# osudrl/cassie-mujoco-sim

Hardware: AMD Instinct MI355X
Metric: env-steps/sec (whole node) at N envs; max |qpos_err| vs CPU ref (higher is better)
Workload: dtype f64

## Files before the change

cassie-mujoco-sim_amd/csrc/env_step_collision.inc:

```
        constexpr int chain_rounds = [] {
            if constexpr (TOPO::is_static) { int r = 0, n = 1; while (n < DofLevels<TOPO>::depth() + 1) { n *= 4; ++r; } return r < 3 ? r : 3; }
            else return 3;
        }();
        int pf_jlim, pf_jtype, pf_jqadr, danc[9], blast, kvin;
        double pf_jmargin, pf_jlo, pf_jhi;
        auto request_behind_collision = [&](int lane_now) {
            const int pf_lj = lane_now < njnt ? lane_now : 0, pf_kd = lane_now < nv ? lane_now : 0, pf_bb = lane_now < nbody ? lane_now : 0;
            pf_jlim = m->jnt_limited[pf_lj]; pf_jtype = m->jnt_type[pf_lj]; pf_jqadr = m->jnt_qposadr[pf_lj];
            pf_jmargin = m->jnt_margin[pf_lj]; pf_jlo = m->jnt_range[pf_lj][0]; pf_jhi = m->jnt_range[pf_lj][1];
#pragma unroll
            for (int r = 0; r < 3 * chain_rounds; ++r) danc[r] = m->dof_anc4[pf_kd][r];
            blast = m->body_lastdof[pf_bb]; kvin = m->dof_vinsrc[pf_kd];
        };
        constexpr bool request_early = (FEAT & FEAT_HFIELD) == 0;
        if constexpr (request_early) request_behind_collision(lane);
        const int pair_bound = m->npair_simple;
        struct PairConst { int g1, g2, tt; double margin, rb1, rb2, s10, s11, s20, s21, s22; };
        auto request_pair = [&](int pp, PairConst &c) {
            const int ps = pp < pair_bound ? pp : 0;
            c.g1 = m->pair_geom1[ps]; c.g2 = m->pair_geom2[ps]; c.tt = m->pair_type[ps];
            c.margin = m->pair_margin[ps]; c.rb1 = m->pair_rbound[ps][0]; c.rb2 = m->pair_rbound[ps][1];
            c.s10 = m->pair_size[ps][0]; c.s11 = m->pair_size[ps][1];
            c.s20 = m->pair_size[ps][3]; c.s21 = m->pair_size[ps][4]; c.s22 = m->pair_size[ps][5];
        };
// ... 145 lines not shown
                const double s10 = pc.s10, s11 = pc.s11, s20 = pc.s20, s21 = pc.s21, s22 = pc.s22;
                double dif[3] = {p2[0] - p1[0], p2[1] - p1[1], p2[2] - p1[2]};
                CK_STAMP(31);
                bool cull = false;
                if (rb1 > 0 && rb2 > 0) {
                    double bound = rb1 + rb2 + margin;
                    cull = dot3(dif, dif) > bound * bound;
                } else if (t1 == CM_GEOM_PLANE && rb2 > 0) {
                    double nn[3] = {m1[2], m1[5], m1[8]};
                    cull = dot3(dif, nn) > margin + rb2;
                }
                if (!cull) {
                    if (t1 == CM_GEOM_PLANE && t2 == CM_GEOM_SPHERE) {
                        n = plane_sphere(rc0, p1, m1, p2, s20, margin);
                    } else if (t1 == CM_GEOM_PLANE && t2 == CM_GEOM_CAPSULE) {
                        double axis[3] = {m2[2], m2[5], m2[8]};
                        RawContact tmp;
                        double e0[3] = {p2[0] + s21 * axis[0], p2[1] + s21 * axis[1], p2[2] + s21 * axis[2]};
                        if (plane_sphere(tmp, p1, m1, e0, s20, margin)) { rc0 = tmp; n = 1; }
                        double e1[3] = {p2[0] - s21 * axis[0], p2[1] - s21 * axis[1], p2[2] - s21 * axis[2]};
                        if (plane_sphere(tmp, p1, m1, e1, s20, margin)) { if (n == 0) rc0 = tmp; else rc1 = tmp; ++n; }
                        for (int i = 0; i < 3; ++i) { rc0.tangent[i] = axis[i]; rc1.tangent[i] = axis[i]; }
                    } else if (t1 == CM_GEOM_SPHERE && t2 == CM_GEOM_SPHERE) {
                        n = sphere_sphere(rc0, p1, s10, p2, s20, margin);
                    } else if (t1 == CM_GEOM_SPHERE && t2 == CM_GEOM_CAPSULE) {
                        double a2[3] = {m2[2], m2[5], m2[8]};
                        double d12[3] = {-dif[0], -dif[1], -dif[2]};
                        double x = clampd(dot3(a2, d12), -s21, s21);
                        double q2[3] = {p2[0] + a2[0] * x, p2[1] + a2[1] * x, p2[2] + a2[2] * x};
                        n = sphere_sphere(rc0, p1, s10, q2, s20, margin);
                    } else if (t1 == CM_GEOM_CAPSULE && t2 == CM_GEOM_CAPSULE) {
                        double a1[3] = {m1[2], m1[5], m1[8]}, a2[3] = {m2[2], m2[5], m2[8]};
                        double x1, x2;
                        segment_closest(p1, a1, s11, p2, a2, s21, x1, x2);
                        double q1[3] = {p1[0] + a1[0] * x1, p1[1] + a1[1] * x1, p1[2] + a1[2] * x1};
                        double q2[3] = {p2[0] + a2[0] * x2, p2[1] + a2[1] * x2, p2[2] + a2[2] * x2};
                        n = sphere_sphere(rc0, q1, s10, q2, s20, margin);
                    } else if (t1 == CM_GEOM_SPHERE && t2 == CM_GEOM_BOX) {
                        double sb[3] = {s20, s21, s22};
                        n = sphere_box(rc0, p1, s10, p2, m2, sb, margin);
                    } else if (t1 == CM_GEOM_CAPSULE && t2 == CM_GEOM_BOX) {
                        double sb[3] = {s20, s21, s22};
                        n = capsule_box(rc0, rc1, p1, m1, s10, s11, p2, m2, sb, margin);
                    } else {
                        warn |= WARN_UNSUPPORTED_PAIR;
                    }
                }
            }
            CK_STAMP(32);
            if (p0 + WV_WAVE < npass) request_pair(p + WV_WAVE, pc);
            const unsigned long long m1b = wv::ballot(n >= 1), m2b = wv::ballot(n >= 2);
            const unsigned long long below = (lane == 0) ? 0ull : (~0ull >> (64 - lane));
            int slot = ncon + wv::popc64(m1b & below) + wv::popc64(m2b & below);
            int more = 0;
            if constexpr ((FEAT & FEAT_HFIELD) != 0) {
                const unsigned long long m3b = wv::ballot(n >= 3), m4b = wv::ballot(n >= 4);
                slot += wv::popc64(m3b & below) + wv::popc64(m4b & below);
                more = wv::popc64(m3b) + wv::popc64(m4b);
                for (int extra = 2; extra < CM_HF_MAXC; ++extra)
                    if (n > extra && slot + extra < MAXC) {
                        const double *c = hfres + (size_t)hfs * HF_REC + 1 + 10 * extra;
                        RawContact rx;
                        rx.dist = c[0];
                        for (int i = 0; i < 3; ++i) { rx.pos[i] = c[1 + i]; rx.normal[i] = c[4 + i]; rx.tangent[i] = c[7 + i]; }
                        write_raw_contact(S, slot + extra, p, rx);
                    }
            }
            if (n >= 1 && slot < MAXC) write_raw_contact(S, slot, p, rc0);
            if (n >= 2 && slot + 1 < MAXC) write_raw_contact(S, slot + 1, p, rc1);
            ncon += wv::popc64(m1b) + wv::popc64(m2b) + more;
        }
        CK_STAMP(22);
        if constexpr (!request_early) request_behind_collision(lane);
        if constexpr ((FEAT & FEAT_WAVEPAIRS) != 0) for (int p = m->npair_simple; p < m->npair; ++p) {
            const int g1 = m->pair_geom1[p], g2 = m->pair_geom2[p], tt = m->pair_type[p];
            const int t1 = tt & 255, t2 = tt >> 8;
            const double margin = m->pair_margin[p];
            const double *p1 = S.x.s.geom_xpos[g1], *p2 = S.x.s.geom_xpos[g2];
            const double *m1 = S.x.s.geom_xmat[g1], *m2 = S.x.s.geom_xmat[g2];
            const double rb1 = m->pair_rbound[p][0], rb2 = m->pair_rbound[p][1];
            {
                double dif[3] = {p2[0] - p1[0], p2[1] - p1[1], p2[2] - p1[2]};
                bool cull = false;
                if (rb1 > 0 && rb2 > 0) { const double bound = rb1 + rb2 + margin; cull = dot3(dif, dif) > bound * bound; }
                else if (t1 == CM_GEOM_PLANE && rb2 > 0) { double nn[3] = {m1[2], m1[5], m1[8]}; cull = dot3(dif, nn) > margin + rb2; }
                if (cull) continue;
            }
            bool hit = false;
            int pairmax = 4;
            RawContact rc;
            if (t1 == CM_GEOM_PLANE && t2 == CM_GEOM_BOX) {
                if (lane < 8) {
                    const double sb0 = m->pair_size[p][3], sb1 = m->pair_size[p][4], sb2 = m->pair_size[p][5];
                    double nrm[3] = {m1[2], m1[5], m1[8]}, dif[3] = {p2[0] - p1[0], p2[1] - p1[1], p2[2] - p1[2]};
                    const double dist = dot3(dif, nrm);
                    double v[3] = {(lane & 1) ? sb0 : -sb0, (lane & 2) ? sb1 : -sb1, (lane & 4) ? sb2 : -sb2}, corner[3];
                    mulmatvec3(corner, m2, v);
                    const double ld = dot3(nrm, corner);
                    if (!(dist + ld > margin || ld > 0)) {
                        hit = true;
                        rc.dist = dist + ld;
                        for (int k = 0; k < 3; ++k) { rc.normal[k] = nrm[k]; rc.tangent[k] = 0; rc.pos[k] = corner[k] + p2[k] - nrm[k] * 0.5 * rc.dist; }
                    }
                }
            } else if (t1 == CM_GEOM_BOX && t2 == CM_GEOM_BOX) {
                double s1[3] = {m->pair_size[p][0], m->pair_size[p][1], m->pair_size[p][2]};
                double s2[3] = {m->pair_size[p][3], m->pair_size[p][4], m->pair_size[p][5]};
                pairmax = (m->flags & CM_FLAG_BOX8) ? 8 : 4;
                hit = box_box_lane(rc, lane, p1, m1, s1, p2, m2, s2, margin, pairmax);
            } else {
                warn |= WARN_UNSUPPORTED_PAIR;
            }
            const unsigned long long hb = wv::ballot(hit);
            const unsigned long long below = (lane == 0) ? 0ull : (~0ull >> (64 - lane));
            const int rank = wv::popc64(hb & below);
            if (hit && rank < pairmax && ncon + rank < MAXC) write_raw_contact(S, ncon + rank, p, rc);
            const int nh = wv::popc64(hb);
            ncon += nh < pairmax ? nh : pairmax;
        }
        const int ncon_found = ncon;
        if (ncon > capc) ncon = capc;
        wv::sync();
        finish_contacts(S, m, P, lane, ncon);
        unsigned long long lob, hib;
        {
            bool lo = false, hi = false;
            wv::keep(pf_jlim); wv::keep(pf_jtype);
            if (lane < njnt && pf_jlim && (pf_jtype == CM_JNT_HINGE || pf_jtype == CM_JNT_SLIDE)) {
                const double q = S.qpos[pf_jqadr];
                lo = q - pf_jlo < pf_jmargin;
                hi = pf_jhi - q < pf_jmargin;
            }
            lob = wv::ballot(lo); hib = wv::ballot(hi);
        }
        if constexpr (MAXR < WIDE_ROWS) {
            const bool may_go_down = io.down_rows > 0 && sub > sub_start;
            if (can_hand_over || may_go_down) {
                const int neq = m->neq;
                const bool eact = lane < neq && m->eq_active[lane < neq ? lane : 0] != 0;
                wv::sync();
                const int nfrictionless = wv::popc64(wv::ballot(lane < ncon && S.c_dim[lane < MAXC ? lane : 0] == 1));
                const int need = 3 * wv::popc64(wv::ballot(eact)) + wv::popc64(lob) + wv::popc64(hib) + 4 * ncon - 3 * nfrictionless;
                const bool up = can_hand_over && (need > capr || (ncon_found > capc && MAXC < m->maxcon));
                const bool down = !up && may_go_down && need <= io.down_rows;
                if (up || down) {
                    bailed = true; bailed_down = down;
                    if constexpr (NW == 2) { if (lane == 0) S.cmd[0] = 1; wv::publish(&S.cmd[4], sub + 1); }
                    break;
                }
            }
        }
        if (ncon_found > capc) warn |= WARN_CONTACT_FULL;
        if constexpr (NW == 1) if (io.drive_mode) {
            if (io.integrate) drive_level_io(io, S, m, env, lane, lastsub);
            wv::sync();
        }
        if constexpr (NW == 2) { CK_STAMP(33); wv::publish(&S.cmd[4], sub + 1); wv::wait_for(&S.cmd[3], sub + 1); }
        CK_STAMP(5);
```

cassie-mujoco-sim_amd/csrc/env_step_rows.inc:

```
        int r_ = lane;
        int rtype = -1, rid = 0, rsub = 0;
        int nefc = 0, nefc_before_contacts = 0;
        double rpos = 0, rmargin = 0, rR = 1.0, rK = 0, rB = 0, rimp = 1.0;
        const bool need_imu = lastsub || io.all_outputs_every_substep || (io.drive_mode && sub + 2 == nsub);
        const bool need_pos = lastsub || io.drive_mode || io.all_outputs_every_substep;
        const bool issens = lane < m->nsensor && need_pos;
        const int ls = issens ? lane : 0;
        SensorConsts sens_c;
        double ycol[NVP];
        double jvel = 0, jws = 0;
        const bool lastcol = !WIDE && lane == NROW - 1;
        for (int pass = 0; pass < (WIDE ? 2 : 1); ++pass) {
        if constexpr (WIDE) {
            if (pass == 1 && nefc <= NROW) break;
            r_ = NROW * pass + lane; rtype = -1; rid = 0; rsub = 0; nefc = 0; jvel = 0; jws = 0;
            rpos = 0; rmargin = 0; rR = 1.0; rK = 0; rB = 0; rimp = 1.0;
        }
        {
            const int neq = m->neq;
            const bool eact = lane < neq && m->eq_active[lane < neq ? lane : 0] != 0;
            const unsigned long long eall = neq >= 64 ? ~0ull : (1ull << neq) - 1;
            if (wv::ballot(eact) == eall && 3 * neq <= capr) {
                if (r_ < 3 * neq) { rtype = CM_CNSTR_EQUALITY; rid = r_ / 3; rsub = r_ - 3 * rid; }
                nefc = 3 * neq;
// ... 10 lines not shown
                const int j = wv::popc64((any & (0ull - any)) - 1);
                for (int side = 0; side < 2; ++side) {
                    if (!(((side == 0 ? lob : hib) >> j) & 1ull)) continue;
                    if (nefc >= capr) { warn |= WARN_CONSTRAINT_FULL; continue; }
                    if (r_ == nefc) { rtype = CM_CNSTR_LIMIT_JOINT; rid = j; rsub = side; }
                    ++nefc;
                }
            }
        }
        nefc_before_contacts = nefc;
        const bool cpyr = lane < ncon && S.c_dim[lane < ncon ? lane : 0] == 3;
        if (wv::ballot(cpyr) == (ncon >= 64 ? ~0ull : (1ull << ncon) - 1) && nefc + 4 * ncon <= capr) {
            if (r_ >= nefc && r_ < nefc + 4 * ncon) { rtype = CM_CNSTR_CONTACT_PYRAMIDAL; rid = (r_ - nefc) >> 2; rsub = (r_ - nefc) & 3; }
            nefc += 4 * ncon;
        } else
        for (int c = 0; c < ncon; ++c) {
            const int dim = S.c_dim[c];
            if (dim != 1 && dim != 3) { warn |= WARN_UNSUPPORTED_PAIR; continue; }
            const int nrow = dim == 1 ? 1 : 2 * (dim - 1);
            if (nefc + nrow > capr) { warn |= WARN_CONSTRAINT_FULL; continue; }
            if (r_ >= nefc && r_ < nefc + nrow) {
                rtype = dim == 1 ? CM_CNSTR_CONTACT_FRICTIONLESS : CM_CNSTR_CONTACT_PYRAMIDAL;
                rid = c; rsub = r_ - nefc;
            }
            nefc += nrow;
        }

        CK_STAMP(25);
        double u3[3] = {0, 0, 0}, wp[3] = {0, 0, 0}, wm[3] = {0, 0, 0};
        unsigned long long maskp = 0, maskm = 0;
        int limdof = -1;
        double limsgn = 0, rdiag = 0, imp_pos = 0, rRscale = 1.0;
        double solref0 = 0.02, solref1 = 1, solimp[5] = {0.9, 0.95, 0.001, 0.5, 2};
        if (rtype == CM_CNSTR_EQUALITY) {
            if (rid != pf_eq) {
                pf_eb1 = m->eq_body1[rid]; pf_eb2 = m->eq_body2[rid]; pf_er1 = m->eq_root[rid][0]; pf_er2 = m->eq_root[rid][1];
            }
            maskp = m->eq_dofmask[rid][0]; maskm = m->eq_dofmask[rid][1];
            rdiag = P->eq_invweight[rid];
            solref0 = m->eq_solref[rid][0]; solref1 = m->eq_solref[rid][1];
            for (int i = 0; i < 5; ++i) solimp[i] = m->eq_solimp[rid][i];
            const int b1 = pf_eb1, b2 = pf_eb2;
            double l1[3] = {m->eq_data[rid][0], m->eq_data[rid][1], m->eq_data[rid][2]};
            double l2[3] = {m->eq_data[rid][3], m->eq_data[rid][4], m->eq_data[rid][5]};
            double a1[3], a2[3];
            mulmatvec3(a1, S.x.s.xmat[b1], l1);
            mulmatvec3(a2, S.x.s.xmat[b2], l2);
            for (int i = 0; i < 3; ++i) { a1[i] += S.x.s.xpos[b1][i]; a2[i] += S.x.s.xpos[b2][i]; }
            u3[0] = rsub == 0 ? 1.0 : 0.0; u3[1] = rsub == 1 ? 1.0 : 0.0; u3[2] = rsub == 2 ? 1.0 : 0.0;
            const double *c1 = S.com[pf_er1], *c2 = S.com[pf_er2];
            double o1[3] = {a1[0] - c1[0], a1[1] - c1[1], a1[2] - c1[2]};
            double o2[3] = {a2[0] - c2[0], a2[1] - c2[1], a2[2] - c2[2]};
            cross3(wp, o1, u3);
            cross3(wm, o2, u3);

            double res[3] = {a1[0] - a2[0], a1[1] - a2[1], a1[2] - a2[2]};
            rpos = rsub == 0 ? res[0] : (rsub == 1 ? res[1] : res[2]); rmargin = 0;
            imp_pos = sqrt(dot3(res, res));

        } else if (rtype == CM_CNSTR_LIMIT_JOINT) {
            const double q = S.qpos[m->jnt_qposadr[rid]];
            rpos = rsub == 0 ? q - m->jnt_range[rid][0] : m->jnt_range[rid][1] - q;
            rmargin = m->jnt_margin[rid];
            imp_pos = rpos;
            limdof = m->jnt_dofadr[rid];
            limsgn = rsub == 0 ? 1.0 : -1.0;
            rdiag = P->jnt_liminvweight[rid];
            solref0 = m->jnt_solref[rid][0]; solref1 = m->jnt_solref[rid][1];
            for (int i = 0; i < 5; ++i) solimp[i] = m->jnt_solimp[rid][i];
        } else if (rtype >= 0) {
            const int c = rid;
            const double *fr = S.c_frame[c];
            if (rtype == CM_CNSTR_CONTACT_PYRAMIDAL) {
                const int a = 1 + rsub / 2;
                const double mu = a <= 2 ? S.c_fri[c][0] : (a == 3 ? S.c_fri[c][1] : S.c_fri[c][2]);
                const double sg = (rsub & 1) ? -mu : mu;
                for (int i = 0; i < 3; ++i) u3[i] = fr[i] + sg * fr[3 * a + i];
                const double mu0 = S.c_fri[c][0];
                rRscale = 2 * mu0 * mu0;
            } else {
                for (int i = 0; i < 3; ++i) u3[i] = fr[i];
            }
            const double *c1 = S.com[S.c_root[c][0]], *c2 = S.com[S.c_root[c][1]];
            double o1[3] = {S.c_pos[c][0] - c1[0], S.c_pos[c][1] - c1[1], S.c_pos[c][2] - c1[2]};
            double o2[3] = {S.c_pos[c][0] - c2[0], S.c_pos[c][1] - c2[1], S.c_pos[c][2] - c2[2]};
            cross3(wp, o2, u3);
            cross3(wm, o1, u3);
            maskp = S.c_dofmask[c][1];
            maskm = S.c_dofmask[c][0];
            rpos = S.c_dist[c]; rmargin = S.c_margin[c]; imp_pos = rpos;
            const double tran = S.c_tran[c];
            const double mu_first = S.c_fri[c][0];
            rdiag = rtype == CM_CNSTR_CONTACT_PYRAMIDAL ? tran + mu_first * mu_first * tran : tran;
            solref0 = S.c_solref[c][0]; solref1 = S.c_solref[c][1];
            for (int i = 0; i < 5; ++i) solimp[i] = S.c_solimp[c][i];
        }
        CK_STAMP(26);
        if (rtype >= 0) {
            rimp = impedance(solimp, imp_pos, rmargin);
            rR = fmax(CM_MINVAL, (1 - rimp) * rdiag / rimp);
            if (rtype == CM_CNSTR_CONTACT_PYRAMIDAL) rR = fmax(CM_MINVAL, rRscale * rR);
            const double dmax = solimp[1];
            if (solref0 > 0) {
                double tc = solref0;
                if ((m->flags & CM_FLAG_REFSAFE) && tc < 2 * h) tc = 2 * h;
                rK = 1.0 / fmax(CM_MINVAL, dmax * dmax * tc * tc * solref1 * solref1);
                rB = 2.0 / fmax(CM_MINVAL, dmax * tc);
            } else {
                rK = -solref0 / fmax(CM_MINVAL, dmax * dmax);
                rB = -solref1 / fmax(CM_MINVAL, dmax);
            }
        }
        CK_STAMP(27);
        if constexpr (NW == 1) sens_c = request_sensor_consts(m, ls);
#pragma unroll
        for (int k0 = 0; k0 < NVP; k0 += 4) {
            double cc[4][6], qv[4], qw[4], qs[4];
#pragma unroll
            for (int kk = 0; kk < 4; ++kk) {
#pragma unroll
                for (int t = 0; t < 6; ++t) cc[kk][t] = S.cdof[k0 + kk][t];
                qv[kk] = S.qvel[k0 + kk]; qw[kk] = S.qacc_ws[k0 + kk];
                if constexpr (NW == 1) qs[kk] = S.qfrc_smooth[k0 + kk]; else qs[kk] = 0.0;
            }
            wv::sched_fence();
#pragma unroll
            for (int kk = 0; kk < 4; ++kk) {
                const int k = k0 + kk;
                double v = 0;
                if (TOPO::is_static ? k < TOPO::nv : k < nv) {
                    if (rtype >= 0) {
                        const double ul = u3[0] * cc[kk][3] + u3[1] * cc[kk][4] + u3[2] * cc[kk][5];
                        const double sp = bitf(maskp, k), sm = bitf(maskm, k);
                        v = sp * (ul + wp[0] * cc[kk][0] + wp[1] * cc[kk][1] + wp[2] * cc[kk][2]) -
                            sm * (ul + wm[0] * cc[kk][0] + wm[1] * cc[kk][1] + wm[2] * cc[kk][2]);
                        if (k == limdof) v = limsgn;
                        jvel += v * qv[kk];
                        jws += v * qw[kk];
                    } else if (lastcol) {
                        v = qs[kk];
                    }
                }
                ycol[k] = v;
            }
        }
        if constexpr (WIDE) {
            if (r_ < MAXR) {
#pragma unroll
                for (int k = 0; k < NVP; ++k) S.x.Yr[r_][k] = ycol[k];
                double *rt = S.x.rowt[r_];
                rt[0] = rR; rt[1] = rtype >= 0 ? -rB * jvel - rK * rimp * (rpos - rmargin) : 0.0; rt[2] = jws;
                rt[3] = rtype < 0 ? -1.0 : (rtype == CM_CNSTR_EQUALITY ? 0.0 : 1.0);
            }
            if (io.ext && pass == 0 && rtype == CM_CNSTR_EQUALITY && r_ < CM_MAXEQROW) {
                cm_ext_t *ex = io.ext + env;
                ex->eq_pos[r_] = rpos; ex->eq_id[r_] = rid;
#pragma unroll
                for (int k = 0; k < NVP; ++k) if (k < nv) ex->eq_J[r_][k] = ycol[k];
            }
        }
        }
        const int sb = NW == 1 ? sens_c.sb : 0;
        CK_STAMP(28);
        if constexpr (NW == 2) {
            if constexpr (WIDE) { if (lane == 0) S.x.turn[0] = nefc; }
            CK_STAMP(34); wv::block_barrier();
            if (lastcol) {
#pragma unroll
                for (int k = 0; k < NVP; ++k) ycol[k] = (TOPO::is_static ? k < TOPO::nv : k < nv) ? S.qfrc_smooth[k] : 0.0;
            }
        }
        const double raref = rtype >= 0 ? -rB * jvel - rK * rimp * (rpos - rmargin) : 0.0;

        int aslot = -1;
        if constexpr (NW == 1) aslot = sensors_before_solve(io, S, m, env, issens, ls, sens_c, need_imu, lastsub);
        CK_STAMP(29);
        if (io.xpos_out && isbody && lastsub) {
            for (int i = 0; i < 3; ++i) io.xpos_out[((size_t)env * io.sb + b) * 3 + i] = S.x.s.xpos[b][i];
            if (io.xquat_out) for (int i = 0; i < 4; ++i) io.xquat_out[((size_t)env * io.sb + b) * 4 + i] = S.x.s.xquat[b][i];
        }
        if (io.ext) {
            cm_ext_t *ex = io.ext + env;
            if (isbody) for (int i = 0; i < 6; ++i) ex->cvel[b][i] = S.x.s.cvel[b][i];
            if (isbody) for (int i = 0; i < 3; ++i) { ex->subtree_com[b][i] = S.com[broot > 0 ? broot : 0][i]; ex->xipos[b][i] = S.x.s.xipos[b][i]; }
            if (lane < m->nsite) {
                const int sb = m->site_bodyid[lane];
                double sp[3] = {m->site_pos[lane][0], m->site_pos[lane][1], m->site_pos[lane][2]};
                double sq[4] = {m->site_quat[lane][0], m->site_quat[lane][1], m->site_quat[lane][2], m->site_quat[lane][3]};
                double t[3], q[4], mm[9];
                mulmatvec3(t, S.x.s.xmat[sb], sp);
                for (int i = 0; i < 3; ++i) ex->site_xpos[lane][i] = t[i] + S.x.s.xpos[sb][i];
                mulquat(q, S.x.s.xquat[sb], sq);
                quat2mat(mm, q);
                for (int i = 0; i < 9; ++i) ex->site_xmat[lane][i] = mm[i];
            }
            if (isdof) for (int i = 0; i < 6; ++i) { ex->cdof[k_][i] = S.cdof[k_][i]; ex->cdof_dot[k_][i] = S.x.s.cdof_dot[k_][i]; }
            if (!WIDE && rtype == CM_CNSTR_EQUALITY && r_ < CM_MAXEQROW) {
                ex->eq_pos[r_] = rpos; ex->eq_id[r_] = rid;
#pragma unroll
                for (int k = 0; k < NVP; ++k) if (k < nv) ex->eq_J[r_][k] = ycol[k];
            }
            if (lane == 0) { int ne = 0; for (int e = 0; e < m->neq; ++e) if (m->eq_active[e] && ne + 3 <= capr) ne += 3; ex->ne = ne; }
            if (lane < ncon) {
                ex->con_geom1[lane] = m->geom_fullid[S.c_g1[lane]]; ex->con_geom2[lane] = m->geom_fullid[S.c_g2[lane]];
                ex->con_body1[lane] = m->geom_bodyid[S.c_g1[lane]]; ex->con_body2[lane] = m->geom_bodyid[S.c_g2[lane]];
                ex->con_dim[lane] = S.c_dim[lane]; ex->con_dist[lane] = S.c_dist[lane];
                for (int i = 0; i < 3; ++i) ex->con_pos[lane][i] = S.c_pos[lane][i];
                for (int i = 0; i < 9; ++i) ex->con_frame[lane][i] = S.c_frame[lane][i];
            }
        }
        int caddr = -1;
        const bool want_cfrc = io.body_cfrc && (sub == nsub - 1 || !io.integrate);
        if (io.ext || want_cfrc) {
            int acc = nefc_before_contacts;
            for (int c = 0; c < ncon; ++c) {
                const int dim = S.c_dim[c];
                if (dim != 1 && dim != 3) continue;
                const int nrow = dim == 1 ? 1 : 2 * (dim - 1);
                if (acc + nrow > capr) continue;
                if (c == lane) caddr = acc;
                acc += nrow;
            }
        }
        wv::sync();
        CK_STAMP(8);
```

cassie-mujoco-sim_amd/csrc/env_step_solve.inc:

```
        if constexpr (WIDE) {
            int iters = 0, nguarded = 0;
            const double f = wide_solve<NVP, TOPO>(S, m, P, 0, nefc, sub, iters, nguarded);
            CK_STAMP(11);

            static_assert(sizeof(S.c_solimp) >= (2 * NROW + 4) * sizeof(double), "the row forces are handed over through the contacts' solimp slots");
            double *const fbuf = &S.c_solimp[0][0];
            fbuf[lane] = f;
            if (lane == 0) { fbuf[2 * NROW] = (double)ncon; fbuf[2 * NROW + 1] = (double)nefc; fbuf[2 * NROW + 2] = (double)iters; fbuf[2 * NROW + 3] = (double)nguarded; }
            wv::block_barrier();
#ifdef CK_WIDE_PROFILE
            if (io.prof && lane < 12) io.prof[(size_t)env * NSTAMP + (lane < 6 ? 16 + lane : 22 + lane)] = (long long)S.x.stepv[lane / 6][lane % 6];
#endif
            if (io.ext || want_cfrc) {
                const int a0 = caddr >= 0 ? caddr : 0;
                double fn = 0, ft1 = 0, ft2 = 0;
                if (lane < ncon && caddr >= 0) {
                    const double f0 = fbuf[a0];
                    if (S.c_dim[lane] == 1) fn = f0;
                    else { const double f1 = fbuf[a0 + 1], f2 = fbuf[a0 + 2], f3 = fbuf[a0 + 3], mu = S.c_fri[lane][0]; fn = f0 + f1 + f2 + f3; ft1 = mu * (f0 - f1); ft2 = mu * (f2 - f3); }
                }
                if (io.ext) {
                    cm_ext_t *ex = io.ext + env;
                    if (lane < ncon) { ex->con_force[lane][0] = fn; ex->con_force[lane][1] = ft1; ex->con_force[lane][2] = ft2; }
                    if (lane == 0) { ex->ncon = ncon; ex->nefc = nefc; ex->solver_iter = iters; }
                }
                if (want_cfrc) {
                    if (lane < ncon) {
                        const double *fr = S.c_frame[lane];
                        double fw[3];
                        for (int j = 0; j < 3; ++j) fw[j] = fr[j] * fn + fr[3 + j] * ft1 + fr[6 + j] * ft2;
                        for (int j = 0; j < 3; ++j) S.c_pos[lane][j] = fw[j];
                    }
                    wv::sync();
                    if (isbody) {
                        double acc[3] = {0, 0, 0};
                        for (int c = 0; c < ncon; ++c) {
                            const int b1 = m->geom_bodyid[S.c_g1[c]], b2 = m->geom_bodyid[S.c_g2[c]];
                            const double sg = (b2 == b ? 1.0 : 0.0) - (b1 == b ? 1.0 : 0.0);
                            for (int j = 0; j < 3; ++j) acc[j] += sg * S.c_pos[c][j];
                        }
                        for (int j = 0; j < 3; ++j) io.body_cfrc[((size_t)env * io.sb + b) * 3 + j] = acc[j];
                    }
                    wv::sync();
                }
            }
            wv::block_barrier();
            CK_STAMP(37);
            if (wv::opaque(S.cmd[0])) { warn |= WARN_DIVERGED; break; }
            if (!io.integrate) break;
            time += h;
            continue;
        }
        if constexpr (TOPO::is_static) {
            double ta[NVP], tb[NVP], ra = 0, rb = 0;
            auto fetch = [&](int k, double (&t)[NVP], double &rs) {
#pragma unroll
                for (int i = k - 1; i >= 0; --i) if ((TOPO::table[k] >> i) & 1ull) t[i] = S.Lp[LPack<TOPO, NVP>::idx(k, i)];
                rs = S.rsd[k];
            };
            fetch(TOPO::nv - 1, ((TOPO::nv - 1) & 1) ? ta : tb, ((TOPO::nv - 1) & 1) ? ra : rb);
#pragma unroll
            for (int k = NVP - 1; k >= 0; --k) {
                if (k >= TOPO::nv) continue;
                if (k > 0) fetch(k - 1, ((k - 1) & 1) ? ta : tb, ((k - 1) & 1) ? ra : rb);
                wv::sched_fence();
                const double (&t)[NVP] = (k & 1) ? ta : tb;
                const double xk = ycol[k];
#pragma unroll
                for (int i = k - 1; i >= 0; --i) if ((TOPO::table[k] >> i) & 1ull) ycol[i] -= t[i] * xk;
                ycol[k] = xk * ((k & 1) ? ra : rb);
                wv::sched_fence();
            }
        } else {
#pragma unroll
            for (int k = NVP - 1; k >= 0; --k) {
                if (k >= nv) continue;
                const unsigned long long anc = m->dof_ancmask[k];
                const double xk = ycol[k];
#pragma unroll
                for (int i = k - 1; i >= 0; --i) {
                    if (!((anc >> i) & 1ull)) continue;
                    ycol[i] -= S.Lp[CK_TRI(k, i)] * xk;
                }
                ycol[k] = xk * S.rsd[k];
            }
        }
        if (r_ < MAXR || lastcol) {
            const int yrow = lastcol ? MAXR : r_;
#pragma unroll
            for (int k = 0; k < NVP; ++k) S.x.Yr[yrow][k] = ycol[k];
        }
        wv::sync();
        if constexpr (NW == 2) wv::publish(&S.cmd[2], sub + 1);
        CK_STAMP(9);

        double arow[MAXR];
        double diag_yy = 0;
        double rb = 0;
        constexpr bool gram_on_matrix_core = MAXR == 31 && NVP % 4 == 0;
        constexpr bool gram_in_place = MAXR == 47 && NVP == 40;
        if constexpr (gram_on_matrix_core) {
            constexpr int YP = EnvShared<NVP, LPack<TOPO, NVP>::count, MAXR>::YP;
            static_assert(2 * (MAXR + 1) * YP * sizeof(double) <= sizeof(S.x), "the Gram matrix is parked behind the staged tile");
            double (*Am)[YP] = (double (*)[YP])(&S.x.Yr[0][0] + (MAXR + 1) * YP);
            const int mi = lane & 15, mk = lane >> 4;
            double y0[NVP / 4], y1[NVP / 4];
#pragma unroll
            for (int kb = 0; kb < NVP / 4; ++kb) { y0[kb] = S.x.Yr[mi][4 * kb + mk]; y1[kb] = S.x.Yr[16 + mi][4 * kb + mk]; }
            wv::mfma_acc t00 = {{0, 0, 0, 0}}, t01 = {{0, 0, 0, 0}}, t11 = {{0, 0, 0, 0}};
#pragma unroll
            for (int kb = 0; kb < NVP / 4; ++kb) wv::mfma_f64_16x16x4_x3(y0[kb], y0[kb], t00, y0[kb], y1[kb], t01, y1[kb], y1[kb], t11);
            wv::mfma_f64_drain(t00, t01, t11);
#pragma unroll
            for (int v = 0; v < 4; ++v) {
                const int row = mk + 4 * v;
                Am[row][mi] = t00.c[v];
                Am[row][16 + mi] = t01.c[v];
                Am[16 + mi][row] = t01.c[v];
                Am[16 + row][16 + mi] = t11.c[v];
            }
            wv::sync();
            const int myrow = lane & 31;
#pragma unroll
            for (int t = 0; t < MAXR; ++t) arow[t] = Am[myrow][t];
            rb = Am[myrow][MAXR] - raref;
#pragma unroll
            for (int k = 0; k < NVP; ++k) wv::touch(ycol[k]);
            diag_yy = Am[myrow][myrow];
        } else if constexpr (gram_in_place) {
            constexpr int AP = 49, AR = MAXR + 1;
            static_assert(AR == 48, "three blocks of sixteen staged rows");
            static_assert(AR * AP * sizeof(double) <= sizeof(S.x), "the matrix fits the region of the staged tile");
            double (*Am)[AP] = (double (*)[AP])&S.x.Yr[0][0];
            const int mi = lane & 15, mk = lane >> 4;
            double y0[NVP / 4], y1[NVP / 4], y2[NVP / 4];
#pragma unroll
            for (int kb = 0; kb < NVP / 4; ++kb) { y0[kb] = S.x.Yr[mi][4 * kb + mk]; y1[kb] = S.x.Yr[16 + mi][4 * kb + mk]; y2[kb] = S.x.Yr[32 + mi][4 * kb + mk]; }
            wv::mfma_acc t00 = {{0, 0, 0, 0}}, t01 = {{0, 0, 0, 0}}, t11 = {{0, 0, 0, 0}}, t02 = {{0, 0, 0, 0}}, t12 = {{0, 0, 0, 0}}, t22 = {{0, 0, 0, 0}};
#pragma unroll
            for (int kb = 0; kb < NVP / 4; ++kb) wv::mfma_f64_16x16x4_x3(y0[kb], y2[kb], t02, y1[kb], y2[kb], t12, y2[kb], y2[kb], t22);
#pragma unroll
            for (int kb = 0; kb < NVP / 4; ++kb) wv::mfma_f64_16x16x4_x3(y0[kb], y0[kb], t00, y0[kb], y1[kb], t01, y1[kb], y1[kb], t11);
            wv::mfma_f64_drain(t00, t01, t11);
            wv::mfma_f64_drain(t02, t12, t22);
            wv::sync();
#pragma unroll
            for (int v = 0; v < 4; ++v) {
                const int row = mk + 4 * v;
                Am[row][mi] = t00.c[v];
                Am[row][16 + mi] = t01.c[v]; Am[16 + mi][row] = t01.c[v];
                Am[16 + row][16 + mi] = t11.c[v];
                Am[row][32 + mi] = t02.c[v]; Am[32 + mi][row] = t02.c[v];
                Am[16 + row][32 + mi] = t12.c[v]; Am[32 + mi][16 + row] = t12.c[v];
                Am[32 + row][32 + mi] = t22.c[v];
            }
            wv::sync();
            const int myrow = lane < AR ? lane : AR - 1;
            rb = Am[myrow][MAXR] - raref;
            diag_yy = Am[myrow][myrow];
#pragma unroll
            for (int t = 0; t < MAXR; ++t) arow[t] = Am[myrow][t];
            wv::sync();
            if (r_ < MAXR || lastcol) {
                const int yrow = lastcol ? MAXR : r_;
#pragma unroll
                for (int k = 0; k < NVP; ++k) S.x.Yr[yrow][k] = ycol[k];
            }
            wv::sync();
        }
        else if constexpr (NW == 2 && NVP > 32) {
#pragma unroll
            for (int r = 0; r < MAXR; ++r) {
                double acc = 0;
                if (r < nefc) {
#pragma unroll
                    for (int k0 = 0; k0 < NVP; k0 += NVP / 2) {
                        double ya[NVP / 2];
#pragma unroll
                        for (int k = 0; k < NVP / 2; ++k) ya[k] = S.x.Yr[r][k0 + k];
#pragma unroll
                        for (int k = 0; k < NVP / 2; ++k) acc = fma(ya[k], ycol[k0 + k], acc);
                    }
                }
                arow[r] = acc;
            }
            {
                double acc = 0;
#pragma unroll
                for (int k = 0; k < NVP; ++k) acc = fma(S.x.Yr[MAXR][k], ycol[k], acc);
                rb = acc - raref;
            }
        } else {
#pragma unroll
        for (int r = 0; r < MAXR; r += 2) {
            double acc0 = 0, acc1 = 0;
            if (r < nefc) {
                constexpr int YB1 = NVP > 32 ? NVP / 2 : NVP;
                double ya[NVP], yb[NVP];
#pragma unroll
                for (int k = 0; k < NVP; ++k) ya[k] = S.x.Yr[r][k];
#pragma unroll
                for (int k = 0; k < YB1; ++k) yb[k] = S.x.Yr[r + 1 < MAXR ? r + 1 : r][k];
                wv::sched_fence();
                if constexpr (NVP == 32) {
#pragma unroll
                    for (int k = 0; k < NVP; ++k) { acc0 = fma(ya[k], ycol[k], acc0); if (r + 1 < MAXR) acc1 = fma(yb[k], ycol[k], acc1); }
                } else if constexpr (NVP == 40) {
#pragma unroll
                    for (int k = 0; k < YB1; ++k) { acc0 = fma(ya[k], ycol[k], acc0); if (r + 1 < MAXR) acc1 = fma(yb[k], ycol[k], acc1); }
                    wv::sched_fence();
#pragma unroll
                    for (int k = YB1; k < NVP; ++k) yb[k] = S.x.Yr[r + 1 < MAXR ? r + 1 : r][k];
#pragma unroll
                    for (int k = YB1; k < NVP; ++k) { acc0 = fma(ya[k], ycol[k], acc0); if (r + 1 < MAXR) acc1 = fma(yb[k], ycol[k], acc1); }
                } else {
                double a0 = 0, a1 = 0, a2 = 0, a3 = 0;
#pragma unroll
                for (int k = 0; k < NVP; k += 4) {
                    a0 += ya[k] * ycol[k]; a1 += ya[k + 1] * ycol[k + 1];
                    a2 += ya[k + 2] * ycol[k + 2]; a3 += ya[k + 3] * ycol[k + 3];
                }
                acc0 = (a0 + a1) + (a2 + a3);
                if constexpr (YB1 < NVP) {
                    wv::sched_fence();
#pragma unroll
                    for (int k = YB1; k < NVP; ++k) yb[k] = S.x.Yr[r + 1 < MAXR ? r + 1 : r][k];
                }
                if (r + 1 < MAXR) {
                    double b0 = 0, b1 = 0, b2 = 0, b3 = 0;
#pragma unroll
                    for (int k = 0; k < NVP; k += 4) {
                        b0 += yb[k] * ycol[k]; b1 += yb[k + 1] * ycol[k + 1];
                        b2 += yb[k + 2] * ycol[k + 2]; b3 += yb[k + 3] * ycol[k + 3];
                    }
                    acc1 = (b0 + b1) + (b2 + b3);
                }
                }
            }
            arow[r] = acc0;
            if (r + 1 < MAXR) arow[r + 1] = acc1;
        }
        {
            double acc = 0;
#pragma unroll
            for (int k = 0; k < NVP; ++k) acc = fma(S.x.Yr[MAXR][k], ycol[k], acc);
            rb = acc - raref;
        }
        }
        CK_STAMP(10);

        const bool isrow = rtype >= 0;
        const bool clampf = isrow && rtype != CM_CNSTR_EQUALITY;
        double Aii = 1.0;
        if constexpr (gram_on_matrix_core || gram_in_place) { if (isrow) Aii = diag_yy + rR; }
        else if (isrow) {
            if constexpr (NVP == 32 || NVP == 40) {
                double d = 0;
#pragma unroll
                for (int k = 0; k < NVP; ++k) d = fma(ycol[k], ycol[k], d);
                Aii = d + rR;
            } else {
                double d0 = 0, d1 = 0, d2 = 0, d3 = 0;
#pragma unroll
                for (int k = 0; k < NVP; k += 4) {
                    d0 += ycol[k] * ycol[k]; d1 += ycol[k + 1] * ycol[k + 1];
                    d2 += ycol[k + 2] * ycol[k + 2]; d3 += ycol[k + 3] * ycol[k + 3];
                }
                Aii = ((d0 + d1) + (d2 + d3)) + rR;
            }
        }
        const double invAii = 1.0 / Aii;
        double f = 0, res = isrow ? rb : 0.0;
        int iters = 0, nguarded = 0;
        if (nefc > 0) {
            if (m->flags & CM_FLAG_WARMSTART) {
                if (isrow) {
                    f = -(jws - raref) / rR;
                    if (clampf && f < 0) f = 0;
                }
                double af0 = 0, af1 = 0, af2 = 0, af3 = 0;
#pragma unroll
                for (int t = 0; t < MAXR; t += 4) {
                    if (t < nefc) {
                        af0 += arow[t] * wv::readlane(f, t);
                        if (t + 1 < MAXR) af1 += arow[t + 1] * wv::readlane(f, t + 1);
                        if (t + 2 < MAXR) af2 += arow[t + 2] * wv::readlane(f, t + 2);
                        if (t + 3 < MAXR) af3 += arow[t + 3] * wv::readlane(f, t + 3);
                    }
                }
                const double af = ((af0 + af1) + (af2 + af3)) + (isrow ? rR * f : 0.0);
                double cost = wv::wave_sum(isrow ? f * (rb + 0.5 * af) : 0.0);
                if (cost > 0) f = 0;
                else if (isrow) res = rb + af;
            }
        CK_STAMP(30);
            const double scale = 1.0 / (P->meaninertia * (nv > 1 ? nv : 1));
            const double halfAii = 0.5 * Aii;
            const double flo = clampf ? 0.0 : -1e300;
            const double ninvAii = -invAii;
            double sres = res * ninvAii;
#pragma unroll
            for (int t = 0; t < MAXR; ++t) arow[t] *= ninvAii;
            const double cdiag = isrow ? rR * ninvAii : 0.0;
            const int maxiter = m->iterations;
            const double tolerance = m->tolerance;
            const bool shortcut_ok = 0.5 * tolerance > (double)MAXR * 1e-10 * scale;
            if constexpr (NW == 2 && CK_PRIO_W0_PGS != CK_PRIO_W0) wv::set_priority<CK_PRIO_W0_PGS>();
            while (iters < maxiter) {
                const int nrows = wv::opaque(nefc);
                bool converged;
                {
                    const double f0 = f, s0 = sres;
                    double mys = 0;
                    const double lo_f = flo - f;
                    pgs_rows_fast<0, MAXR>(arow, nrows, r_, lo_f, sres, mys);
                    const double mydelta = wv::max_raw(mys, lo_f);
                    const double change = (r_ < nrows) ? mydelta * (halfAii * mydelta - Aii * mys) : 0.0;
                    const float tol = (float)tolerance;
                    const bool one_row_decides = shortcut_ok && wv::ballot(-(float)change * (float)scale > 2.5f * tol) != 0ull;
                    const float est = one_row_decides ? 4.0f * tol : -wv::wave_sum_f32((float)change) * (float)scale;
                    if (wv::ballot(change > 1e-10) != 0ull || wv::debug_force_guarded()) {
                        double improvement = 0;
                        f = f0; sres = s0; ++nguarded;
                        pgs_rows<0, MAXR>(arow, nrows, r_, Aii, halfAii, flo, f, sres, improvement);
                        sres = fma(cdiag, f - f0, sres);
                        converged = improvement * scale < tolerance;
                    } else {
                        if (r_ < nrows) { f += mydelta; sres = fma(cdiag, mydelta, sres); }
                        if (est < 0.5f * tol) converged = true;
                        else if (est > 2.0f * tol) converged = false;
                        else {
                            const double tree = -wv::wave_sum(change) * scale, tolv = tolerance;
                            if (fabs(tree - tolv) > 1e-9 * tolv) converged = tree < tolv;
                            else
                            {
                                double improvement = 0;
                                for (int t = 0; t < nrows; ++t) improvement -= wv::readlane(change, t);
                                converged = improvement * scale < tolerance;
                            }
                        }
                    }
                }
                ++iters;
                if (converged) break;
            }
        }
        if constexpr (NW == 2 && CK_PRIO_W0_PGS != CK_PRIO_W0) wv::set_priority<CK_PRIO_W0>();
        CK_STAMP(11);
        if (io.ext || want_cfrc) {
            const int a0 = caddr >= 0 ? caddr : 0;
            const double f0 = wv::shfl(f, a0), f1 = wv::shfl(f, (a0 + 1) & 63), f2 = wv::shfl(f, (a0 + 2) & 63), f3 = wv::shfl(f, (a0 + 3) & 63);
            double fn = 0, ft1 = 0, ft2 = 0;
            if (lane < ncon && caddr >= 0) {
                if (S.c_dim[lane] == 1) fn = f0;
                else { const double mu = S.c_fri[lane][0]; fn = f0 + f1 + f2 + f3; ft1 = mu * (f0 - f1); ft2 = mu * (f2 - f3); }
            }
            if (io.ext) {
                cm_ext_t *ex = io.ext + env;
                if (lane < ncon) { ex->con_force[lane][0] = fn; ex->con_force[lane][1] = ft1; ex->con_force[lane][2] = ft2; }
                if (lane == 0) { ex->ncon = ncon; ex->nefc = nefc; ex->solver_iter = iters; }
            }
            if (want_cfrc) {
                if (lane < ncon) {
                    const double *fr = S.c_frame[lane];
                    double fw[3];
                    for (int j = 0; j < 3; ++j) fw[j] = fr[j] * fn + fr[3 + j] * ft1 + fr[6 + j] * ft2;
                    for (int j = 0; j < 3; ++j) S.c_pos[lane][j] = fw[j];
                }
                wv::sync();
                if (isbody) {
                    double acc[3] = {0, 0, 0};
                    for (int c = 0; c < ncon; ++c) {
                        const int b1 = m->geom_bodyid[S.c_g1[c]], b2 = m->geom_bodyid[S.c_g2[c]];
                        const double sg = (b2 == b ? 1.0 : 0.0) - (b1 == b ? 1.0 : 0.0);
                        for (int j = 0; j < 3; ++j) acc[j] += sg * S.c_pos[c][j];
                    }
                    for (int j = 0; j < 3; ++j) io.body_cfrc[((size_t)env * io.sb + b) * 3 + j] = acc[j];
                }
                wv::sync();
            }
        }

        if constexpr (NW == 2) {
            static_assert(sizeof(S.c_solimp) >= 68 * sizeof(double), "the row forces are handed over through the contacts' solimp slots");
            double *const fbuf = &S.c_solimp[0][0];
            fbuf[lane] = f;
            if (lane == 0) { fbuf[64] = (double)ncon; fbuf[65] = (double)nefc; fbuf[66] = (double)iters; fbuf[67] = (double)nguarded; }
            wv::block_barrier();
            wv::block_barrier();
            CK_STAMP(37);
            if (wv::opaque(S.cmd[0])) { warn |= WARN_DIVERGED; break; }
            if (!io.integrate) break;
            time += h;
            continue;
        }
        const int pf_u = lane < nu ? lane : 0, pf_ej = lane < njnt ? lane : 0;
        const double pf_agear = m->act_gear[pf_u], pf_kdamp = P->dof_damping[isdof ? k_ : 0];
        const int pf_adof = m->act_dofid[pf_u], pf_ejt = m->jnt_type[pf_ej], pf_eqa = m->jnt_qposadr[pf_ej], pf_eda = m->jnt_dofadr[pf_ej];
        double qacc;
        {
            double z = isdof ? S.x.Yr[MAXR][k_] : 0.0;
            {
                double z1 = 0, z2 = 0, z3 = 0;
                const int kk = isdof ? k_ : 0;
                int r = 0;
                for (; r + 4 <= nefc; r += 4) {
                    const double y0 = S.x.Yr[r][kk], y1 = S.x.Yr[r + 1][kk], y2 = S.x.Yr[r + 2][kk], y3 = S.x.Yr[r + 3][kk];
                    z += y0 * wv::readlane(f, r); z1 += y1 * wv::readlane(f, r + 1);
                    z2 += y2 * wv::readlane(f, r + 2); z3 += y3 * wv::readlane(f, r + 3);
                }
                for (; r < nefc; ++r) z += S.x.Yr[r][kk] * wv::readlane(f, r);
                z = (z + z1) + (z2 + z3);
                if (!isdof) z = 0.0;
            }
            if (isdof) z *= S.rsd[k_];
            double lrow[NVP];
            stage_factor_row<NVP, TOPO>(S, k_, isdof, lrow);
            qacc = solve_forward<NVP, TOPO>(z, lrow, lane, nv);
        }
        {
            const bool badv = isdof && (!(qacc == qacc) || fabs(qacc) > 1e10);
            if (wv::ballot(badv) != 0ull) { warn |= WARN_DIVERGED; break; }
        }
        if (isdof) S.qacc[k_] = qacc;
        wv::sync();
        CK_STAMP(12);

        outputs_after_qacc(io, S, m, env, lane, isdof, k_, nu, qacc, aslot, sb, need_imu, lastsub, pf_agear * S.qvel[pf_adof], ncon, nefc, iters, nguarded);
        if (!io.integrate) break;
        CK_STAMP(13);

        {
            double lcol[NVP], lrowh[NVP];
            stage_factor_h<NVP, TOPO>(S, k_, isdof, nv, lcol, lrowh);
            const double dih = isdof ? S.dinvH[k_] : 0.0;
            euler_step<NVP, TOPO>(S, m, lane, isdof, k_, nv, njnt, h, qacc, lcol, lrowh, dih, pf_kdamp, pf_ejt, pf_eqa, pf_eda);
        }
        time += h;
        CK_STAMP(14);
    }
```

cassie-mujoco-sim_amd/csrc/env_step_wave1.inc:

```
    if constexpr (NW == 2) {
        if (wid == 1) {
            for (int sub1 = sub_start;;) {
                const int pb = isbody ? b : 0;
                const double mass = P->body_mass[pb];
                double iner[3], imat[9];
                for (int i = 0; i < 3; ++i) iner[i] = P->body_inertia[pb][i];
                for (int i = 0; i < 9; ++i) imat[i] = m->body_imat[pb][i];
                CK_STAMP(35);
                wv::block_barrier();
                if (wv::opaque(S.cmd[0])) return -1;
                wv::set_priority<(FEAT & FEAT_HFIELD) != 0 ? CK_PRIO_W1_FJ_HFIELD : CK_PRIO_W1_FJ>();
                CK_STAMP(36);
                double ximat[9] = {1, 0, 0, 0, 1, 0, 0, 0, 1};
                if (isbody && b > 0) {
                    double xm[9];
                    for (int i = 0; i < 9; ++i) xm[i] = S.x.s.xmat[b][i];
                    for (int i = 0; i < 3; ++i)
                        for (int c = 0; c < 3; ++c) ximat[3 * i + c] = xm[3 * i] * imat[c] + xm[3 * i + 1] * imat[3 + c] + xm[3 * i + 2] * imat[6 + c];
                }
                double col[NVP], colh[NVP];
                mass_matrix_columns<NVP, TOPO, FEAT, NW>(io, S, m, env, ids, mass, iner, ximat, col, colh);
                wv::publish(&S.cmd[3], sub1 + 1);
                CK_STAMP(38);
                factor_pair_by_height<NVP, TOPO, 0>(m, P, h, S, col, colh, lane);
                constexpr bool park_colh = NVP > 32;
                if constexpr (park_colh) {
                    if (isdof) {
#pragma unroll
                        for (int i = 0; i < NVP; ++i) {
                            if (i >= TOPO::nv) continue;
                            if (i == k_) S.dinvH[k_] = colh[i];
                            else if (i > k_ && LP::col_has(i, k_)) S.LHp[LP::col_idx(i, k_)] = colh[i];
                        }
                    }
                    wv::sync();
                }
                wv::wait_for(&S.cmd[4], sub1 + 1);
                if (wv::opaque(S.cmd[0])) return -1;
                if (io.drive_mode) {
                    if (io.integrate) drive_level_io(io, S, m, env, lane, sub1 == nsub - 1);
                    wv::sync();
                }
                CK_STAMP(4);
                {
                    const int kd = isdof ? k_ : 0;
                    const double kdamp = P->dof_damping[kd], kstiff = PS->dof_stiffness[kd], kref = PS->dof_springref[kd];
                    const double kgear = m->dof_gear[kd], klo = m->dof_ctrl_lo[kd], khi = m->dof_ctrl_hi[kd];
                    const int kq = m->dof_qadr[kd], ka = m->dof_act[kd];
                    wv::wait_for(&S.cmd[1], sub1 + 1);
                    bias_forces_and_qfrc_smooth<NVP, (NVP > 32)>(io, S, m, env, ids, kdamp, kstiff, kref, kgear, klo, khi, kq, ka);
                }
                const bool lastsub1 = sub1 == nsub - 1 || !io.integrate;
                const bool need_imu1 = lastsub1 || io.all_outputs_every_substep || (io.drive_mode && sub1 + 2 == nsub);
                const bool issens1 = lane < m->nsensor && (lastsub1 || io.drive_mode || io.all_outputs_every_substep);
                const int ls1 = issens1 ? lane : 0;
                const SensorConsts sens_c1 = request_sensor_consts(m, ls1);
                const int aslot1 = sensors_before_solve(io, S, m, env, issens1, ls1, sens_c1, need_imu1, lastsub1);
                CK_STAMP(47);
                wv::block_barrier();
                wv::set_priority<CK_PRIO_W1_JP>();
                CK_STAMP(39);
                if constexpr (WIDE) {
                    int it1 = 0, ng1 = 0;
                    const double f1 = wide_solve<NVP, TOPO>(S, m, P, 1, wv::opaque(S.x.turn[0]), sub1, it1, ng1);
                    (&S.c_solimp[0][0])[NROW + lane] = f1;
                }
                if constexpr (park_colh) {
#pragma unroll
                    for (int i = 0; i < NVP; ++i) {
                        double v = 0.0;
                        if (i < TOPO::nv && isdof) {
                            if (i == k_) v = S.dinvH[k_];
                            else if (i > k_ && LP::col_has(i, k_)) v = S.LHp[LP::col_idx(i, k_)];
                        }
                        colh[i] = v;
                    }
                    wv::sync();
                }
                factor_pair_by_height<NVP, TOPO, 1>(m, P, h, S, col, colh, lane);
                {
                    const bool lastsub = lastsub1, need_imu = need_imu1;
                    const int sb = sens_c1.sb, aslot = aslot1;
                    const int pf_u = lane < nu ? lane : 0, pf_ej = lane < njnt ? lane : 0;
                    const double pf_agear = m->act_gear[pf_u], pf_kdamp = P->dof_damping[isdof ? k_ : 0];
                    const int pf_adof = m->act_dofid[pf_u], pf_ejt = m->jnt_type[pf_ej], pf_eqa = m->jnt_qposadr[pf_ej], pf_eda = m->jnt_dofadr[pf_ej];
                    const double *const fbuf = &S.c_solimp[0][0];
                    double lrow[NVP];
                    constexpr bool stage_h_early = NVP <= 32;
                    if constexpr (stage_h_early) stage_factor_row<NVP, TOPO>(S, k_, isdof, lrow);
                    double lcol[NVP], lrowh[NVP];
                    if constexpr (stage_h_early) stage_factor_h<NVP, TOPO, 0>(S, k_, isdof, nv, lcol, lrowh);
                    const double rsdk = isdof ? S.rsd[k_] : 0.0;
                    const int kk = isdof ? k_ : 0;
                    constexpr bool stage_y = MAXR <= 31;
                    double ycolk[stage_y ? MAXR + 1 : 1];
                    if constexpr (stage_y) {
                        wv::wait_for(&S.cmd[2], sub1 + 1);
#pragma unroll
                        for (int r = 0; r <= MAXR; ++r) ycolk[r] = S.x.Yr[r][kk];
                    }
                    wv::block_barrier();
                    wv::set_priority<CK_PRIO_W1_PE>();
                    const double f = fbuf[lane], f_hi = WIDE ? fbuf[NROW + lane] : 0.0;
                    constexpr int FB = WIDE ? 2 * NROW : NROW;
                    const int ncon = (int)fbuf[FB], nefc = (int)fbuf[FB + 1], iters = (int)fbuf[FB + 2], nguarded = (int)fbuf[FB + 3];
                    double z, z1 = 0, z2 = 0, z3 = 0;
                    if constexpr (stage_y) {
                        z = isdof ? ycolk[MAXR] : 0.0;
#pragma unroll
                        for (int r = 0; r < MAXR; r += 4) {
                            if (r + 4 <= nefc) {
                                z += ycolk[r] * wv::readlane(f, r); z1 += ycolk[r + 1 < MAXR ? r + 1 : r] * wv::readlane(f, r + 1);
                                z2 += ycolk[r + 2 < MAXR ? r + 2 : r] * wv::readlane(f, r + 2); z3 += ycolk[r + 3 < MAXR ? r + 3 : r] * wv::readlane(f, r + 3);
                            } else {
#pragma unroll
                                for (int j = 0; j < 4; ++j) if (r + j < nefc && r + j < MAXR) z += ycolk[r + j < MAXR ? r + j : r] * wv::readlane(f, r + j);
                            }
                        }
                    } else {
                        z = isdof ? S.x.Yr[MAXR][k_] : 0.0;
                        auto frow = [&](int r) { if constexpr (WIDE) return r < NROW ? wv::readlane(f, r) : wv::readlane(f_hi, r - NROW); else return wv::readlane(f, r); };
                        int r = 0;
                        for (; r + 4 <= nefc; r += 4) {
                            const double y0 = S.x.Yr[r][kk], y1 = S.x.Yr[r + 1][kk], y2 = S.x.Yr[r + 2][kk], y3 = S.x.Yr[r + 3][kk];
                            z += y0 * frow(r); z1 += y1 * frow(r + 1);
                            z2 += y2 * frow(r + 2); z3 += y3 * frow(r + 3);
                        }
                        for (; r < nefc; ++r) z += S.x.Yr[r][kk] * frow(r);
                    }
                    z = (z + z1) + (z2 + z3);
                    if (!isdof) z = 0.0;
                    if (isdof) z *= rsdk;
                    if constexpr (stage_h_early) stage_factor_h<NVP, TOPO, 1>(S, k_, isdof, nv, lcol, lrowh);
                    const double dih = isdof ? S.dinvH[k_] : 0.0;
                    if constexpr (!stage_h_early) stage_factor_row<NVP, TOPO>(S, k_, isdof, lrow);
                    wv::sched_fence();
                    const double qacc = solve_forward<NVP, TOPO>(z, lrow, lane, nv);
                    {
                        const bool badv = isdof && (!(qacc == qacc) || fabs(qacc) > 1e10);
                        if (wv::ballot(badv) != 0ull) {
                            if (lane == 0) S.cmd[0] = 2;
                            wv::block_barrier();
                            return -1;
                        }
                    }
                    if (isdof) S.qacc[k_] = qacc;
                    const double av = pf_agear * S.qvel[pf_adof];
                    wv::sync();
                    CK_STAMP(12);
                    if (io.integrate) {
                        if constexpr (!stage_h_early) stage_factor_h<NVP, TOPO>(S, k_, isdof, nv, lcol, lrowh);
                        euler_step<NVP, TOPO>(S, m, lane, isdof, k_, nv, njnt, h, qacc, lcol, lrowh, dih, pf_kdamp, pf_ejt, pf_eqa, pf_eda);
                    }
                    CK_STAMP(13);
                    wv::block_barrier();
                    wv::set_priority<CK_PRIO_W1_EF>();
                    outputs_after_qacc(io, S, m, env, lane, isdof, k_, nu, qacc, aslot, sb, need_imu, lastsub, av, ncon, nefc, iters, nguarded);
                    CK_STAMP(14);
                }
                if (!io.integrate || ++sub1 >= nsub) return -1;
            }
        }
    }
```

cassie-mujoco-sim_amd/csrc/kernels_cassie.hip:

```cpp
#include "step_kernels.h"
namespace ck {
template void launch_step<32, TopoCassie32, 0>(unsigned, hipStream_t, const PhysIO &);
template void launch_step<32, TopoCassie32, 0, FAST_ROWS>(unsigned, hipStream_t, const PhysIO &);
}
```

cassie-mujoco-sim_amd/csrc/kernels_cassie_2w.hip:

```cpp
#include "step_kernels.h"
namespace ck {
template void launch_step<32, TopoCassie32, 0, FAST_ROWS, 2>(unsigned, hipStream_t, const PhysIO &);
}
```

cassie-mujoco-sim_amd/csrc/kernels_cassie_2w_inplace.hip:

```cpp
#include "step_kernels.h"
namespace ck {
template void launch_step<32, TopoCassie32, 0, FAST_ROWS, 2, false, 2, MID_ROWS>(unsigned, hipStream_t, const PhysIO &);
}
```

cassie-mujoco-sim_amd/csrc/kernels_hfield.hip:

```cpp
#include "step_kernels.h"
namespace ck {
template void launch_step<32, TopoCassie32, FEAT_HFIELD>(unsigned, hipStream_t, const PhysIO &);
template void launch_step<32, TopoCassie32, FEAT_HFIELD, FAST_ROWS>(unsigned, hipStream_t, const PhysIO &);
}
```

cassie-mujoco-sim_amd/csrc/kernels_hfield_2w.hip:

```cpp
#include "step_kernels.h"
namespace ck {
template void launch_step<32, TopoCassie32, FEAT_HFIELD, FAST_ROWS, 2>(unsigned, hipStream_t, const PhysIO &);
}
```

cassie-mujoco-sim_amd/csrc/kernels_hfield_2w_inplace.hip:

```cpp
#include "step_kernels.h"
namespace ck {
template void launch_step<32, TopoCassie32, FEAT_HFIELD, FAST_ROWS, 2, false, 2, MID_ROWS>(unsigned, hipStream_t, const PhysIO &);
}
```

cassie-mujoco-sim_amd/csrc/kernels_tray_2w.hip:

```cpp
#include "step_kernels.h"
namespace ck {
template void launch_step<40, TopoCassieTray38, FEAT_WAVEPAIRS, FAST_ROWS_TRAY, 2>(unsigned, hipStream_t, const PhysIO &);
}
```

cassie-mujoco-sim_amd/csrc/kernels_tray_fast.hip:

```cpp
#include "step_kernels.h"
namespace ck {
template void launch_step<40, TopoCassieTray38, FEAT_WAVEPAIRS, FAST_ROWS_TRAY>(unsigned, hipStream_t, const PhysIO &);
template void launch_step<40, TopoCassieTray38, FEAT_WAVEPAIRS, MID_ROWS, 1, true>(unsigned, hipStream_t, const PhysIO &);
}
```

cassie-mujoco-sim_amd/csrc/phys_batch.hip:

```cpp
#include <hip/hip_runtime.h>

#include <cstddef>
#include <cstdio>
#include <cstdlib>
#include <cstring>
#include <string>
#include <utility>
#include <vector>

#include "cassie_phys.h"
#include "device_mem.h"
#include "small_launch.h"
#include "step_launch.h"
#include "step_policy.h"

void phys_set_last_error(const char *s);

constexpr int DEFAULT_TRAY_WAVES = 2;

struct phys_batch {
    int nenv = 0, device = 0;
    cm_model_t host_model;
    DevBuf<cm_model_t> d_models;
    DevBuf<cm_envparams_t> d_envparams;
// ... 9 lines not shown
    DevBuf<int> d_terrain_index;
    ck::ScanCfg scan = {};
    DevBuf<double> d_scan_offsets;
    ck::DepthCfg depth = {};
    long long depth_launches[2] = {0, 0};
    ck::RayCfg rays = {};
    DevBuf<ck::RayDef> d_rays;
    long long ray_launches = 0;
    hipStream_t stream = nullptr;
    hipStream_t recent_streams[4] = {nullptr, nullptr, nullptr, nullptr};
    int recent_next = 0;
    hipEvent_t ev0 = nullptr, ev1 = nullptr, ev_mark = nullptr;
    bool use_applied = false;
    bool pd_mode = false;
    int drive_mode = CM_DRIVE_OFF;
    DevBuf<cm_drive_state_t> d_drive;
    bool use_pd_dtarget = false, use_pd_torque = false;
    DevBuf<long long> d_prof;
    bool all_outputs = false;
    DevBuf<cm_ext_t> d_ext;

    bool fast_rows = true;
    int waves_per_env = 2;
    int waves_per_env_tray = DEFAULT_TRAY_WAVES;
    int inplace_mode = 2;
    long long form_launches[2] = {0, 0};
    bool balance = true;
    DevBuf<unsigned> d_cost, d_cost_wall;
    DevBuf<int> d_order;
    std::vector<int> order_ident;
    ck::RangeTable ranges;
    DevBuf<int> d_progress;
    int chunks = ck::DEFAULT_CHUNKS_WHOLE, chunks_range = ck::DEFAULT_CHUNKS_RANGE;
    bool chunks_default = true;
    DevBuf<int> d_chunk_flag;
    int chunk_seq = 0;
    bool chunks_allowed = true;
    std::vector<std::pair<hipStream_t, bool>> probed_streams;
    HostWords chunk_fault;
    bool chunk_fault_reported = false;
    DevBuf<int> d_handover_list, d_handover_count, d_handover_list2, d_handover_count2;
    HostWords handover_seen, handover_seen2;
    bool timing = false;
    std::vector<std::pair<hipEvent_t, hipEvent_t>> ev_pool;
    size_t ev_used = 0;

    DevBuf<double> d_scratch_out;
    bool episodes = false;
    ck::EpisodeCfg ep = {};
    DevBuf<char> d_ep[PHYS_EP_ARRAYS];
    DevBuf<const double> d_ep_bank;
    ck::PlaceCfg place = {};
    DevBuf<ck::PlaceTable> d_place_table;
    DevBuf<double> d_place_offsets, d_place_pose, d_place_ground;
};

static bool hip_ok(hipError_t e, const char *what) {
    if (e == hipSuccess) return true;
    std::string msg = std::string("HIP error in ") + what + ": " + hipGetErrorString(e);
    phys_set_last_error(msg.c_str());
    fprintf(stderr, "cassie_phys: %s\n", msg.c_str());
    return false;
}

static ck::PhysIO make_io(phys_batch *b, int nsub, int integrate) {
    ck::PhysIO io;
    memset(&io, 0, sizeof io);
    io.models = b->d_models;
    io.model_stride = b->model_stride;
    io.envparams = b->d_envparams;
    io.nenv = b->nenv; io.nsub = nsub; io.integrate = integrate;
    io.sq = b->stride[PHYS_F_QPOS]; io.sqv = b->stride[PHYS_F_QVEL]; io.sv = b->host_model.nv; io.su = b->host_model.nu;
    io.ssd = b->stride[PHYS_F_SENSORDATA]; io.sb = b->host_model.nbody;
    io.qpos = b->d_field[PHYS_F_QPOS]; io.qvel = b->d_field[PHYS_F_QVEL];
    io.qacc_warmstart = b->d_field[PHYS_F_QACC_WARMSTART]; io.time = b->d_field[PHYS_F_TIME];
    io.ctrl = b->d_field[PHYS_F_CTRL];
    io.qfrc_applied = b->use_applied ? b->d_field[PHYS_F_QFRC_APPLIED] : nullptr;
    io.xfrc_applied = b->use_applied ? b->d_field[PHYS_F_XFRC_APPLIED] : nullptr;
    io.qacc = b->d_field[PHYS_F_QACC]; io.sensordata = b->d_field[PHYS_F_SENSORDATA];
    io.actuator_velocity = b->d_field[PHYS_F_ACTUATOR_VELOCITY];
    io.warn = b->d_warn; io.info = b->d_info;
    io.xpos_out = b->d_field[PHYS_F_XPOS]; io.xquat_out = b->d_field[PHYS_F_XQUAT];
    io.body_cfrc = b->d_field[PHYS_F_BODY_CFRC];
    io.hfield = b->d_hfield;
    io.hfield_stride = b->hfield_stride;
    if (b->nterrain > 0) { io.hfield_index = b->d_terrain_index; io.hfield_nterrain = b->nterrain; }
    if (b->pd_mode) {
        io.pd_ptarget = b->d_field[PHYS_F_PD_PTARGET]; io.pd_kp = b->d_field[PHYS_F_PD_KP]; io.pd_kd = b->d_field[PHYS_F_PD_KD];
    }
    io.drive_mode = b->d_drive ? b->drive_mode : CM_DRIVE_OFF;
    if (io.drive_mode != CM_DRIVE_OFF) {
        io.drive_state = b->d_drive;
        io.drive_cmd = b->d_field[PHYS_F_DRIVE_CMD];
        io.meas = b->d_field[PHYS_F_MEAS];
        if (io.drive_mode == CM_DRIVE_PD || io.drive_mode == CM_DRIVE_PD_SAFE) {
            io.pd_ptarget = b->d_field[PHYS_F_PD_PTARGET]; io.pd_kp = b->d_field[PHYS_F_PD_KP]; io.pd_kd = b->d_field[PHYS_F_PD_KD];
            io.pd_dtarget = b->use_pd_dtarget ? b->d_field[PHYS_F_PD_DTARGET] : nullptr;
            io.pd_torque = b->use_pd_torque ? b->d_field[PHYS_F_PD_TORQUE] : nullptr;
        }
    }
    io.all_outputs_every_substep = b->all_outputs ? 1 : 0;
    io.prof = b->d_prof;
    io.ext = b->d_ext;
    if (b->balance && b->d_order) { io.order = b->d_order; io.cost = b->d_cost; io.cost_wall = b->d_cost_wall; }
    return io;
}

static bool quiesce(phys_batch *b) {
    bool ok = hip_ok(hipStreamSynchronize(b->stream), "hipStreamSynchronize");
    for (hipStream_t r : b->recent_streams)
        if (r && r != b->stream) ok = hip_ok(hipStreamSynchronize(r), "hipStreamSynchronize(caller stream)") && ok;
    return ok;
}

static void note_stream(phys_batch *b, hipStream_t s) {
    for (hipStream_t r : b->recent_streams) if (r == s) return;
    b->recent_streams[b->recent_next] = s;
    b->recent_next = (b->recent_next + 1) % 4;
}

static hipStream_t launch_stream(phys_batch *b, void *stream) {
    const hipStream_t s = stream ? (hipStream_t)stream : b->stream;
    note_stream(b, s);
    return s;
}

static bool range_ok(const phys_batch *b, int env0, int n) {
    return env0 >= 0 && n >= 0 && (size_t)env0 + (size_t)n <= (size_t)b->nenv;
}
static bool strided_ok(const phys_batch *b, int first, int stride, int count) {
    return first >= 0 && stride >= 1 && count >= 0 && (count == 0 || (size_t)first + (size_t)(count - 1) * (size_t)stride < (size_t)b->nenv);
}

static ck::BatchView view_of(const phys_batch *b) {
    ck::BatchView v = {b->d_models, b->model_stride, b->d_envparams, b->d_hfield, b->hfield_stride, b->d_terrain_index, b->nterrain};
    ck::view_sizes(v, b->host_model);
    v.sq = b->stride[PHYS_F_QPOS]; v.sqv = b->stride[PHYS_F_QVEL]; v.ssd = b->stride[PHYS_F_SENSORDATA];
    v.qpos = b->d_field[PHYS_F_QPOS]; v.qvel = b->d_field[PHYS_F_QVEL]; v.warm = b->d_field[PHYS_F_QACC_WARMSTART];
    v.ctrl = b->d_field[PHYS_F_CTRL]; v.qacc = b->d_field[PHYS_F_QACC]; v.time = b->d_field[PHYS_F_TIME];
    v.sens = b->d_field[PHYS_F_SENSORDATA]; v.actvel = b->d_field[PHYS_F_ACTUATOR_VELOCITY];
    v.meas = b->d_drive ? b->d_field[PHYS_F_MEAS].get() : nullptr;
    v.drive = b->d_drive; v.warn = b->d_warn;
    v.xpos = b->d_field[PHYS_F_XPOS]; v.xquat = b->d_field[PHYS_F_XQUAT];
    return v;
}
static int refuse(const char *entry, const char *why) {
    phys_set_last_error((std::string(entry) + ": " + why).c_str());
    return -1;
}

using ck::launch_step;
using ck::FAST_ROWS; using ck::FAST_ROWS_TRAY; using ck::MID_ROWS; using ck::WIDE_ROWS;
using ck::TopoCassie32; using ck::TopoCassieTray38; using ck::TopoRuntime;
template <int FEAT>
static const ck::StepLauncher CASSIE_FORMS[ck::FORM_COUNT] = {
    launch_step<32, TopoCassie32, FEAT>,
    launch_step<32, TopoCassie32, FEAT, MID_ROWS, 2, false, 1>,
    launch_step<32, TopoCassie32, FEAT, WIDE_ROWS, 2, false, 1>,
    launch_step<32, TopoCassie32, FEAT, FAST_ROWS>,
    launch_step<32, TopoCassie32, FEAT, FAST_ROWS, 2>,
    launch_step<32, TopoCassie32, FEAT, FAST_ROWS, 2, false, 2, MID_ROWS>,
    nullptr,
    launch_step<32, TopoCassie32, FEAT, MID_ROWS, 2, true>,
    launch_step<32, TopoCassie32, FEAT, WIDE_ROWS, 2, true, 1>,
};
static const ck::StepLauncher TRAY_FORMS[ck::FORM_COUNT] = {
    launch_step<40, TopoCassieTray38, ck::FEAT_WAVEPAIRS>,
    launch_step<40, TopoCassieTray38, ck::FEAT_WAVEPAIRS, MID_ROWS, 2>,
    nullptr,
    launch_step<40, TopoCassieTray38, ck::FEAT_WAVEPAIRS, FAST_ROWS_TRAY>,
    launch_step<40, TopoCassieTray38, ck::FEAT_WAVEPAIRS, FAST_ROWS_TRAY, 2>,
    nullptr,
    launch_step<40, TopoCassieTray38, ck::FEAT_WAVEPAIRS, MID_ROWS, 1, true>,
    launch_step<40, TopoCassieTray38, ck::FEAT_WAVEPAIRS, MID_ROWS, 2, true>,
    nullptr,
};
static const ck::StepLauncher CASSIE_ALL_FORMS[ck::FORM_COUNT] = {launch_step<32, TopoCassie32, ck::FEAT_ALL>};
static const ck::StepLauncher TRAY_HFIELD_FORMS[ck::FORM_COUNT] = {launch_step<40, TopoCassieTray38, ck::FEAT_ALL>};
static const ck::StepLauncher GENERIC32_FORMS[ck::FORM_COUNT] = {launch_step<32, TopoRuntime, ck::FEAT_ALL>};
static const ck::StepLauncher GENERIC40_FORMS[ck::FORM_COUNT] = {launch_step<40, TopoRuntime, ck::FEAT_ALL>};
static const ck::StepLauncher *const FAMILY_FORMS[ck::FAMILY_COUNT] = {
    CASSIE_FORMS<0>, CASSIE_FORMS<ck::FEAT_HFIELD>, CASSIE_ALL_FORMS, TRAY_FORMS, TRAY_HFIELD_FORMS, GENERIC32_FORMS, GENERIC40_FORMS,
};

extern "C" __global__ void __launch_bounds__(128) cassie_xcd_probe_kernel(int *xcc) {
    if (threadIdx.x == 0) xcc[blockIdx.x] = (int)(wv::hw_id() >> 32) & 7;
}
static bool workgroups_go_round_the_xcds(hipStream_t s) {
    constexpr int NWG = 1024;
    DevBuf<int> d;
    int h[NWG];
    bool ok = d.alloc(NWG, false, "XCD probe");
    if (ok) {
        hipLaunchKernelGGL(cassie_xcd_probe_kernel, dim3(NWG), dim3(128), 0, s, d.get());
        ok = hipGetLastError() == hipSuccess && hipMemcpyAsync(h, d, sizeof h, hipMemcpyDeviceToHost, s) == hipSuccess && hipStreamSynchronize(s) == hipSuccess;
        for (int w = 8; ok && w < NWG; ++w) ok = h[w] == h[w % 8];
    }
    return ok;
}
static bool stream_may_chunk(phys_batch *b, hipStream_t s) {
    if (!b->chunks_allowed) return false;
    if (b->chunk_fault.host() && *(volatile int *)b->chunk_fault.host()) {
        b->chunks_allowed = false;
        if (!b->chunk_fault_reported) {
            b->chunk_fault_reported = true;
            fprintf(stderr, "cassie_phys: a chunk of a stepping launch ran on another XCD than the chunk before it (a CU-masked stream or a partition mode that "
                            "breaks the round-robin placement): the envs concerned carry warning bit 16, launches go in one piece from now on\n");
        }
        return false;
    }
    for (const auto &ps : b->probed_streams) if (ps.first == s) return ps.second;
    const bool ok = workgroups_go_round_the_xcds(s);
    if (b->probed_streams.size() < 64) b->probed_streams.emplace_back(s, ok);
    return ok;
}

static void set_chunks(phys_batch *b, ck::PhysIO &io, int n, int nsub, hipStream_t s) {
    const int nchunk = b->chunks_allowed ? ck::launch_chunks(n, b->nenv, nsub, b->chunks, b->chunks_range, b->chunks_default) : 1;
    io.nchunk = 1;
    if (nchunk <= 1 || !stream_may_chunk(b, s)) return;
    io.nchunk = nchunk;
    if (b->chunk_seq >= (1 << 24)) {
        (void)hipDeviceSynchronize();
        (void)hipMemsetAsync(b->d_chunk_flag, 0, sizeof(int) * (size_t)b->nenv, s);
        (void)hipStreamSynchronize(s);
        b->chunk_seq = 0;
    }
    io.chunk_seq = ++b->chunk_seq;
    io.chunk_flag = b->d_chunk_flag;
    io.chunk_fault = b->chunk_fault.dev();
}

static void reset_range_words(phys_batch *b, int env0, hipStream_t s) {
    (void)hipMemsetAsync(b->d_handover_count + 2 * (size_t)env0, 0, 2 * sizeof(int), s);
    b->handover_seen.host()[env0] = 0;
}

static ck::LaunchRange *claim_range(phys_batch *b, int env0, int n, hipStream_t s) {
    std::vector<ck::LaunchRange> retired;
    ck::LaunchRange *range = b->ranges.claim(env0, n, retired);
    for (const ck::LaunchRange &g : retired) {
        if (b->d_order && !hip_ok(hipMemcpyAsync(b->d_order + g.env0, b->order_ident.data() + g.env0, sizeof(int) * (size_t)g.n, hipMemcpyHostToDevice, s), "hipMemcpy(order reset)")) return nullptr;
        if (g.inplace) reset_range_words(b, g.env0, s);
    }
    return range;
}

static hipEvent_t timing_begin(phys_batch *b, hipStream_t s) {
    if (b->ev_used == b->ev_pool.size() && b->ev_pool.size() < 65536) {
        hipEvent_t a = nullptr, c = nullptr;
        if (hipEventCreate(&a) == hipSuccess && hipEventCreate(&c) == hipSuccess) b->ev_pool.emplace_back(a, c);
    }
    if (b->ev_used == b->ev_pool.size()) return nullptr;
    (void)hipEventRecord(b->ev_pool[b->ev_used].first, s);
    return b->ev_pool[b->ev_used++].second;
}

static int launch(phys_batch *b, int nsub, int integrate, hipStream_t s, bool scratch_outputs = false, int env0 = 0, int n = -1) {
    ck::PhysIO io = make_io(b, nsub, integrate);
    if (n < 0) n = b->nenv;
    io.env0 = env0; io.nenv = n;
    if (!integrate) { io.order = nullptr; io.cost = nullptr; io.cost_wall = nullptr; }
    if (scratch_outputs) {
        const cm_model_t &m = b->host_model;
        io.qacc = b->d_scratch_out; io.sv = m.nv;
        io.sensordata = b->d_scratch_out + (size_t)b->nenv * m.nv; io.ssd = m.nsensordata;
        io.actuator_velocity = io.sensordata + (size_t)b->nenv * m.nsensordata;
    }
    note_stream(b, s);
    const cm_model_t &hm = b->host_model;
    const ck::StepFamily fam = ck::pick_family(hm, b->generic_kernel);
    const ck::StepLauncher *family = FAMILY_FORMS[fam];
    const bool has_inplace = family[ck::FORM_FAST_INPLACE] != nullptr;
    auto forms_if = [&](bool inplace) {
        return ck::launch_forms(fam, has_inplace, hm.maxefc, integrate, io.ext != nullptr, n, nsub, b->fast_rows, b->waves_per_env, b->waves_per_env_tray, inplace);
    };
    ck::StepForms forms = forms_if(false);
    const bool fast = ck::is_fast_form(forms.first);
    ck::LaunchRange *range = nullptr;
    if (integrate && (io.order || fast) && !(range = claim_range(b, env0, n, s))) return -1;
    const hipEvent_t ev_after = b->timing && integrate ? timing_begin(b, s) : nullptr;
    ck::HandoverLists hl = {nullptr, nullptr, nullptr, nullptr, nullptr, nullptr};
    ck::StepGrids grids = {(unsigned)n, (unsigned)n, (unsigned)n};
    if (fast) {
        io.progress = b->d_progress;
        set_chunks(b, io, n, nsub, s);
        hl.list1 = b->d_handover_list; hl.count1 = b->d_handover_count + 2 * (size_t)env0; hl.seen1 = b->handover_seen.dev() + env0;
        if (forms.wide) { hl.list2 = b->d_handover_list2; hl.count2 = b->d_handover_count2 + 2 * (size_t)env0; hl.seen2 = b->handover_seen2.dev() + env0; }
        const int seen = *(volatile int *)(b->handover_seen.host() + env0);
        grids = ck::pass_grids(n, seen, forms.wide ? b->handover_seen2.host()[env0] : 0, forms.wide);
        if (forms.first == ck::FORM_FAST_2W && has_inplace) {
            const bool was = range->inplace;
            range->inplace = ck::next_inplace(was, seen, b->inplace_mode, io.order != nullptr);
            if (was != range->inplace) reset_range_words(b, env0, s);
            ++b->form_launches[range->inplace ? 1 : 0];
            forms = forms_if(range->inplace);
        }
    }
    const ck::StepPlan plan = ck::plan_step(io, forms, hl, grids);
    for (int i = 0; i < plan.n; ++i) {
        const ck::StepPass &p = plan.pass[i];
        if (!family[p.form]) { (void)hip_ok(hipErrorInvalidDeviceFunction, "cassie_step_kernel launch (no instantiation of this form)"); return -1; }
        family[p.form](p.grid, s, p.io);
        if (!hip_ok(hipGetLastError(), "cassie_step_kernel launch")) return -1;
        if (i == 0 && ev_after) (void)hipEventRecord(ev_after, s);
    }
    if (io.order && ck::order_kernel_due(nsub, ++range->launches_since_sort)) {
        range->launches_since_sort = 0;
        const bool inplace = forms.first == ck::FORM_FAST_INPLACE;
        hipLaunchKernelGGL(ck::cassie_order_kernel, dim3(1), dim3(ck::ORDER_THREADS), 0, s, b->d_cost, b->d_order, n, env0,
                           inplace ? hl.count1 : (int *)nullptr, inplace ? hl.seen1 : (volatile int *)nullptr);
        if (!hip_ok(hipGetLastError(), "cassie_order_kernel launch")) return -1;
    }
    return 0;
}

static void note_field_in_use(phys_batch *b, int field) {
    if (field == PHYS_F_QFRC_APPLIED || field == PHYS_F_XFRC_APPLIED) b->use_applied = true;
    if (field == PHYS_F_PD_DTARGET) b->use_pd_dtarget = true;
    if (field == PHYS_F_PD_TORQUE) b->use_pd_torque = true;
}

static bool copy_rows(phys_batch *b, int field, void *host, int env0, int n, bool to_device, const char *what) {
    if (!b->d_field[field]) { phys_set_last_error("this field is allocated by phys_batch_derive (PHYS_F_HEIGHT_SCAN: phys_batch_scan_configure, PHYS_F_DEPTH: phys_batch_depth_configure, PHYS_F_RAYS: phys_batch_rays_configure); call it first"); return false; }
    const size_t row = (size_t)b->dim[field], st = (size_t)b->stride[field];
    double *dev = b->d_field[field] + st * env0;
    if (n == 0) return true;
    if (st == row)
        return hip_ok(to_device ? hipMemcpyAsync(dev, host, sizeof(double) * row * n, hipMemcpyHostToDevice, b->stream)
                                : hipMemcpyAsync(host, dev, sizeof(double) * row * n, hipMemcpyDeviceToHost, b->stream), what);
    return hip_ok(to_device ? hipMemcpy2DAsync(dev, sizeof(double) * st, host, sizeof(double) * row, sizeof(double) * row, n, hipMemcpyHostToDevice, b->stream)
                            : hipMemcpy2DAsync(host, sizeof(double) * row, dev, sizeof(double) * st, sizeof(double) * row, n, hipMemcpyDeviceToHost, b->stream), what);
}

extern "C" {

phys_batch_t *phys_batch_create(const cm_model_t *model, int nenv, int device) {
    if (!model || nenv <= 0) { phys_set_last_error("phys_batch_create: bad arguments"); return nullptr; }
    int ndev = 0;
    if (hipGetDeviceCount(&ndev) != hipSuccess || ndev <= 0) {
        const char *msg = "phys_batch_create: no HIP device available -- this library has no CPU fallback";
        phys_set_last_error(msg);
        fprintf(stderr, "cassie_phys: %s\n", msg);
        return nullptr;
    }
    if (device < 0 || device >= ndev) { phys_set_last_error("phys_batch_create: bad device index"); return nullptr; }
    if (!hip_ok(hipSetDevice(device), "hipSetDevice")) return nullptr;
    phys_batch *b = new phys_batch;
    b->nenv = nenv; b->device = device;
    if (const char *tw = getenv("CASSIE_TRAY_TWO_WAVES")) b->waves_per_env_tray = atoi(tw) ? 2 : 1;
    b->host_model = *model;
    cm_model_sync_params(&b->host_model);
    b->host_model.env_geom = 0; b->host_model.env_springs = 0;
    model = &b->host_model;
    const int d[PHYS_F_COUNT] = {model->nq, model->nv, model->nv, 1, model->nu, model->nv, model->nbody * 6,
                                 model->nv, model->nsensordata, model->nu, model->nbody * 3, model->nbody * 4,
                                 model->nu, model->nu, model->nu, model->nbody * 3,
                                 model->nu + 1, CM_MEAS_DIM, model->nu, model->nu, CM_DRV_DIM, model->nv * model->nv, 0, 0, 0};
    const size_t n = (size_t)nenv;
    bool ok = true;
    for (int f = 0; f < PHYS_F_COUNT; ++f) {
        b->dim[f] = d[f]; b->stride[f] = d[f];
        if (f == PHYS_F_DERIVED || f == PHYS_F_QM) continue;
        if (f == PHYS_F_HEIGHT_SCAN) continue;
        if (f == PHYS_F_DEPTH) continue;
        if (f == PHYS_F_RAYS) continue;
        ok = ok && b->d_field[f].alloc(n * (d[f] > 0 ? d[f] : 1), true, "field");
    }
    ok = ok && b->d_models.alloc(1, false, "model");
    ok = ok && hip_ok(hipMemcpy(b->d_models, model, sizeof(cm_model_t), hipMemcpyHostToDevice), "hipMemcpy(model)");
    ok = ok && b->d_warn.alloc(n, true, "warn") && b->d_info.alloc(4 * n, true, "info");
    if (nenv >= 2048) {
        b->order_ident.resize(n);
        for (int e = 0; e < nenv; ++e) b->order_ident[(size_t)e] = e;
        ok = ok && b->d_order.alloc(n, false, "order");
        ok = ok && hip_ok(hipMemcpy(b->d_order, b->order_ident.data(), sizeof(int) * n, hipMemcpyHostToDevice), "hipMemcpy(order)");
        ok = ok && b->d_cost.alloc(n, true, "cost") && b->d_cost_wall.alloc(n, true, "cost, wall clock");
    }
    ok = ok && b->d_progress.alloc(n, true, "progress") && b->d_chunk_flag.alloc(n, true, "chunk words");
    if (const char *ck = getenv("CASSIE_CHUNKS")) { b->chunks = b->chunks_range = atoi(ck) > 1 ? (atoi(ck) < 7 ? atoi(ck) : 7) : 1; b->chunks_default = false; }
    ok = ok && b->chunk_fault.alloc(1, "chunk fault word");
    ok = ok && b->d_handover_list.alloc(n, false, "hand-over list") && b->d_handover_count.alloc(2 * n, true, "hand-over counts");
    ok = ok && b->handover_seen.alloc(n, "hand-over seen");
    ok = ok && b->d_handover_list2.alloc(n, false, "second hand-over list") && b->d_handover_count2.alloc(2 * n, true, "second hand-over counts");
    ok = ok && b->handover_seen2.alloc(n, "second hand-over seen");
    ok = ok && hip_ok(hipStreamCreateWithFlags(&b->stream, hipStreamNonBlocking), "hipStreamCreate");
    ok = ok && hip_ok(hipEventCreate(&b->ev0), "hipEventCreate") && hip_ok(hipEventCreate(&b->ev1), "hipEventCreate");
    ok = ok && hip_ok(hipEventCreateWithFlags(&b->ev_mark, hipEventDisableTiming), "hipEventCreate");
    if (ok) {
        std::vector<double> q0((size_t)nenv * model->nq);
        for (int e = 0; e < nenv; ++e) memcpy(&q0[(size_t)e * model->nq], model->qpos0, sizeof(double) * model->nq);
        ok = hip_ok(hipMemcpy(b->d_field[PHYS_F_QPOS], q0.data(), q0.size() * sizeof(double), hipMemcpyHostToDevice),
                    "hipMemcpy(qpos0)");
    }
    if (!ok) { phys_batch_free(b); return nullptr; }
    return b;
}

void phys_batch_free(phys_batch_t *b) {
    if (!b) return;
    (void)hipSetDevice(b->device);
    for (auto &e : b->ev_pool) { (void)hipEventDestroy(e.first); (void)hipEventDestroy(e.second); }
    if (b->ev0) (void)hipEventDestroy(b->ev0);
    if (b->ev1) (void)hipEventDestroy(b->ev1);
    if (b->ev_mark) (void)hipEventDestroy(b->ev_mark);
    if (b->stream) (void)hipStreamDestroy(b->stream);
    delete b;
}

int phys_batch_nenv(const phys_batch_t *b) { return b ? b->nenv : 0; }
int phys_batch_field_dim(const phys_batch_t *b, int field) {
    return (b && field >= 0 && field < PHYS_F_COUNT) ? b->dim[field] : 0;
}

int phys_batch_set_model(phys_batch_t *b, const cm_model_t *model, int env) {
    if (!b || !model) return -1;
    if (model->nq != b->host_model.nq || model->nv != b->host_model.nv || model->nbody != b->host_model.nbody ||
        model->nu != b->host_model.nu || model->nsensordata != b->host_model.nsensordata) {
        phys_set_last_error("phys_batch_set_model: model dimensions differ from the batch's");
        return -1;
    }
    (void)hipSetDevice(b->device);
    if (!quiesce(b)) return -1;
    cm_model_t synced = *model;
    cm_model_sync_params(&synced);
    synced.env_geom = 0; synced.env_springs = 0;
    model = &synced;
    if (env < 0) {
        b->d_envparams.reset();
        if (b->model_stride == 1) {
            if (!b->d_models.alloc(1, false, "model")) return -1;
            b->model_stride = 0;
        }
        b->host_model = *model;
        return hip_ok(hipMemcpy(b->d_models, model, sizeof(cm_model_t), hipMemcpyHostToDevice), "hipMemcpy(model)") ? 0 : -1;
    }
    if (env >= b->nenv) return -1;
    if (b->d_envparams) { phys_set_last_error("phys_batch_set_model: per-env models and per-env parameter blocks (phys_batch_randomize) do not mix"); return -1; }
    if (memcmp(model->dof_ancmask, b->host_model.dof_ancmask, sizeof(model->dof_ancmask[0]) * (size_t)model->nv) != 0 ||
        model->kin_simple != b->host_model.kin_simple || model->maxdepth != b->host_model.maxdepth ||
        (model->nhfpair > 0) != (b->host_model.nhfpair > 0) || (model->hfield_geom >= 0) != (b->host_model.hfield_geom >= 0) ||
        (model->npair > model->npair_simple) != (b->host_model.npair > b->host_model.npair_simple) ||
        model->maxefc != b->host_model.maxefc || model->maxcon != b->host_model.maxcon ||
        ((model->flags ^ b->host_model.flags) & (CM_FLAG_HFPRISM | CM_FLAG_HFMULTI | CM_FLAG_HFDENSE | CM_FLAG_BOX8)) != 0) {
        phys_set_last_error("phys_batch_set_model: a per-env model must keep the shared model's dof tree, collision pair kinds, contact / row caps and height-field contact option");
        return -1;
    }
    if (b->model_stride == 0) {
        DevBuf<cm_model_t> all;
        if (!all.alloc((size_t)b->nenv, false, "models")) return -1;
        std::vector<cm_model_t> tmp((size_t)b->nenv, b->host_model);
        if (!hip_ok(hipMemcpy(all, tmp.data(), sizeof(cm_model_t) * tmp.size(), hipMemcpyHostToDevice), "hipMemcpy(models)")) return -1;
        b->d_models = std::move(all);
        b->model_stride = 1;
    }
// ... 884 lines not shown
```

cassie-mujoco-sim_amd/csrc/physics_kernel.h:

```cpp
#ifndef CASSIE_PHYSICS_KERNEL_H
#define CASSIE_PHYSICS_KERNEL_H

#include <wave.h>

#include "cm_model.h"
#include "topo_static.h"

#include "pk_types.h"
#include "pk_math.h"
#include "pk_safety.h"
#include "pk_collision.h"
#include "pk_factor_solve.h"
#include "pk_stages.h"
#include "pk_wide_solve.h"

namespace ck {


constexpr int ENV_STEP_WENT_DOWN = 1 << 20;

template <int NVP, class TOPO, int FEAT, int MAXR, int NW>
WV_DEVICE int env_step(const PhysIO &io, EnvShared<NVP, LPack<TOPO, NVP>::count, MAXR> &S, int env, int sub_start, int nsub) {
    typedef LPack<TOPO, NVP> LP;
    static_assert(NW == 1 || NW == 2, "one or two wavefronts per env");
    static_assert(NW == 1 || TOPO::is_static, "the two-wave form exists for the compile-time topologies");
    const int wid = NW == 2 ? wv::wave_id() : 0;
    if constexpr (NW == 2) { if (wid == 0) wv::set_priority<CK_PRIO_W0>(); }
    constexpr int prio_kin = (FEAT & FEAT_HFIELD) != 0 ? CK_PRIO_W0 : CK_PRIO_W0_KIN;

    static_assert(LP::covers() && LP::distinct(), "packed factor rows must hold every ancestor pair, each in its own slot");
    typedef EnvShared<NVP, LPack<TOPO, NVP>::count, MAXR> SH_T;
    constexpr int MAXC = SH_T::MAXC;
    constexpr bool WIDE = SH_T::WIDE;
    static_assert(!WIDE || (NW == 2 && MAXR == WIDE_ROWS), "the 127-row instantiation spreads its solve over the two wavefronts of an env");
    const ModelPtr m_launch = (ModelPtr)(io.models + (size_t)env * io.model_stride);
    ModelPtr m = m_launch;
    const ParamPtr P = io.envparams ? (ParamPtr)(io.envparams + (size_t)env) : (ParamPtr)&m_launch->params;
    const ParamPtr PG = m_launch->env_geom ? P : (ParamPtr)&m_launch->params, PS = m_launch->env_springs ? P : (ParamPtr)&m_launch->params;
    int lane = wv::lane();
    const int nq = m->nq, nv = m->nv, nu = m->nu, nbody = m->nbody, njnt = m->njnt;
    const int capr = m->maxefc < MAXR ? m->maxefc : MAXR, capc = m->maxcon < MAXC ? m->maxcon : MAXC;
    const bool can_hand_over = MAXR < WIDE_ROWS && io.has_next != 0 && io.progress != nullptr && (MAXR < m->maxefc || MAXC < m->maxcon);
    const double h = m->timestep;
    int warn = 0;

    if (NW == 1 || wid == 0) {
    if (lane == 0) { S.cmd[0] = 0; S.cmd[1] = 0; S.cmd[2] = 0; S.cmd[3] = 0; S.cmd[4] = 0; }
    if constexpr (WIDE) { if (lane == 0) { S.x.turn[0] = 0; S.x.turn[1] = 0; S.x.turn[2] = 0; S.x.turn[3] = 0; } }
    if (lane < nq) S.qpos[lane] = io.qpos[(size_t)env * io.sq + lane];
    if (lane < nv) {
        S.qvel[lane] = io.qvel[(size_t)env * io.sqv + lane];
        S.qacc_ws[lane] = io.qacc_warmstart[(size_t)env * io.sv + lane];
    }
    if (lane < nu) S.ctrl[lane] = io.ctrl[(size_t)env * io.su + lane];
    if (lane < NB && !wv::test_skip_com_init()) { S.com[lane][0] = 0.0; S.com[lane][1] = 0.0; S.com[lane][2] = 0.0; }
    if (io.drive_mode) {
        if (lane < m->nsensordata) S.sens[lane] = io.sensordata[(size_t)env * io.ssd + lane];
        if (lane < nu) S.actvel[lane] = io.actuator_velocity[(size_t)env * io.su + lane];
        drive_state_load(io, S, env, lane);
        drive_consts_load(io, S, m, env, lane);
    }
    }
    double time = io.time[env];

    int b = lane;
    bool isbody = b < nbody;
    const int depth = isbody ? m->body_depth[b] : -1;
    const int bparent = isbody ? m->body_parentid[b] : 0;
    const int broot = isbody ? m->body_rootid[b] : -1;
    const int bjn = isbody ? m->body_jntnum[b] : 0;
    const int bj0 = (isbody && bjn > 0) ? m->body_jntadr[b] : 0;
    const int bend = isbody ? m->body_subtreeend[b] : 0;
    const unsigned long long bdofmask = isbody ? m->body_dofmask[b] : 0ull;
    const int bjt = (isbody && bjn > 0) ? m->jnt_type[bj0] : -1;
    const int bjq = (isbody && bjn > 0) ? m->jnt_qposadr[bj0] : 0;
    int k_ = lane;
    bool isdof = k_ < nv;
    const int kjnt = isdof ? m->dof_jntid[k_] : 0;
    const int kbody = isdof ? m->dof_bodyid[k_] : 0;
    const int kjt = isdof ? m->jnt_type[kjnt] : -1;
    const int kda = isdof ? m->jnt_dofadr[kjnt] : 0;
    const int kqa = isdof ? m->jnt_qposadr[kjnt] : 0;
    const int kroot = isdof ? m->body_rootid[kbody] : 0;
    const int kbend = isdof ? m->body_subtreeend[kbody] : 0;
    const unsigned long long kdesc = isdof ? m->dof_descmask[k_] : 0ull;
    const unsigned long long kvelmask = isdof ? m->dof_velmask[k_] : 0ull;
    int kact = -1;
    for (int u = 0; u < nu; ++u) if (isdof && m->act_dofid[u] == k_) kact = u;
    const LaneIds ids = {nbody, nv, broot, bend, kjnt, kbody, kjt, kda, kroot, kbend, kdesc};
    wv::sync();

#include "env_step_wave1.inc"

    const float *env_hfield = nullptr;
    if constexpr ((FEAT & FEAT_HFIELD) != 0) {
        bool clamped;
        env_hfield = terrain_grid(io.hfield, io.hfield_stride, io.hfield_index, io.hfield_nterrain, env, &clamped);
        if (clamped && lane == 0 && wid == 0) wv::atomic_or(io.warn + env, WARN_TERRAIN_INDEX);
    }

    bool bailed = false, bailed_down = false;
    int sub = sub_start;
    for (; sub < nsub; ++sub) {
        const bool lastsub = sub == nsub - 1 || !io.integrate;
        const bool need_quat = lastsub || io.ext != nullptr || io.all_outputs_every_substep || (io.drive_mode && sub + 2 == nsub);
        {
            bool badv = false;
            if (lane < nq) { double v = S.qpos[lane]; badv |= !(v == v) || fabs(v) > 1e10; }
            if (lane < nv) { double v = S.qvel[lane]; badv |= !(v == v) || fabs(v) > 1e10; }
            if (wv::ballot(badv) != 0ull) {
                warn |= WARN_DIVERGED;
                if constexpr (NW == 2) { if (lane == 0) S.cmd[0] = 1; wv::block_barrier(); }
                break;
            }
        }
        if (io.drive_mode) {
        } else if (io.pd_ptarget) {
            if (lane < nu) {
                const size_t o = (size_t)env * io.su + lane;
                const double ratio = m->act_gear[lane], tmax = m->act_ctrlrange[lane][1];
                const double q = S.qpos[m->act_qposadr[lane]], qd = S.qvel[m->act_dofid[lane]];
                const double tau = io.pd_kp[o] * (io.pd_ptarget[o] - q) - io.pd_kd[o] * qd;
                const double wmax = m->act_maxrpm[lane] * (2.0 * 3.14159265358979323846 / 60.0);
                const double tlim = clampd(2 * tmax * (1 - fabs(ratio * qd) / wmax), 0.0, tmax);
                S.ctrl[lane] = copysign(fmin(fabs(tau / ratio), tlim), tau);
            }
            wv::sync();
        }
        CK_STAMP(0);
        if constexpr (NW == 2 && prio_kin != CK_PRIO_W0) wv::set_priority<prio_kin>();

        double Rl[9] = {1, 0, 0, 0, 1, 0, 0, 0, 1}, pl[3] = {0, 0, 0}, qlq[4] = {1, 0, 0, 0};
        constexpr int kin_rounds = [] {
            if constexpr (TOPO::is_static) { int r = 0, n = 1; while (n < TOPO::body_levels) { n *= 3; ++r; } return r < 1 ? 1 : r; }
            else return 3;
        }();
        int kanc[2 * kin_rounds];
#pragma unroll
        for (int r = 0; r < 2 * kin_rounds; ++r) kanc[r] = isbody ? m->body_anc3[b][r] : 0;
        const bool isfree = bjt == CM_JNT_FREE;
        if constexpr (TOPO::is_static) {
            {
                const auto *kr = &m->body_kin[isbody ? b : 0];
                const int nsl = kr->nslide, j0 = kr->jnt0, jr = kr->rot_jnt, jt = kr->rot_type, qa = kr->rot_qadr;
                int sqa[CM_MAXSLIDE];
                double sref[CM_MAXSLIDE], sax[CM_MAXSLIDE][3], spo[CM_MAXSLIDE][3];
#pragma unroll
                for (int sl = 0; sl < CM_MAXSLIDE; ++sl) {
                    sqa[sl] = kr->slide_qadr[sl]; sref[sl] = kr->slide_ref[sl];
                    for (int i = 0; i < 3; ++i) { sax[sl][i] = kr->slide_axis_p[sl][i]; spo[sl][i] = kr->slide_pos_p[sl][i]; }
                }
                const double jref = kr->rot_ref;
                double jp[3], ja[3], jpp[3], xl[3], q0[4];
                for (int i = 0; i < 3; ++i) { jp[i] = kr->rot_pos[i]; ja[i] = kr->rot_axis[i]; jpp[i] = kr->rot_pos_p[i]; xl[i] = kr->rot_axis_p[i]; }
                for (int i = 0; i < 9; ++i) Rl[i] = kr->mat[i];
                for (int i = 0; i < 3; ++i) pl[i] = kr->pos[i];
                for (int i = 0; i < 4; ++i) q0[i] = kr->quat[i];
#pragma unroll
                for (int sl = 0; sl < CM_MAXSLIDE; ++sl) {
                    const double d = S.qpos[sqa[sl]] - sref[sl];
                    if (sl < nsl) for (int i = 0; i < 3; ++i) { S.x.s.xanchor[j0 + sl][i] = pl[i] + spo[sl][i]; S.x.s.xaxis[j0 + sl][i] = sax[sl][i]; }
                    for (int i = 0; i < 3; ++i) pl[i] += sax[sl][i] * d;
                }
                for (int i = 0; i < 4; ++i) qlq[i] = q0[i];
                double sn, cs;
                sincos_bounded(jt == CM_JNT_HINGE ? 0.5 * (S.qpos[qa] - jref) : 0.0, sn, cs);
                if (jr >= 0) {
                    double qj[4];
                    if (jt == CM_JNT_HINGE) {
                        qj[0] = cs; qj[1] = ja[0] * sn; qj[2] = ja[1] * sn; qj[3] = ja[2] * sn;
                    } else {
                        const int qo = jt == CM_JNT_FREE ? qa + 3 : qa;
                        for (int i = 0; i < 4; ++i) qj[i] = S.qpos[qo + i];
                        normalize4_fast(qj);
                        if (jt == CM_JNT_FREE) for (int i = 0; i < 3; ++i) pl[i] = S.qpos[qa + i];
                    }
                    double al[3], Rq[9], Rn[9], r[3];
                    for (int i = 0; i < 3; ++i) { al[i] = pl[i] + jpp[i]; S.x.s.xanchor[jr][i] = al[i]; S.x.s.xaxis[jr][i] = xl[i]; }
                    quat2mat(Rq, qj);
                    for (int i = 0; i < 3; ++i)
                        for (int c = 0; c < 3; ++c) Rn[3 * i + c] = Rl[3 * i] * Rq[c] + Rl[3 * i + 1] * Rq[3 + c] + Rl[3 * i + 2] * Rq[6 + c];
                    for (int i = 0; i < 9; ++i) Rl[i] = Rn[i];
                    if (need_quat) mulquat(qlq, q0, qj);
                    mulmatvec3(r, Rl, jp);
                    for (int i = 0; i < 3; ++i) pl[i] = al[i] - r[i];
                }
            }
        } else
        if (isbody && b > 0) {
            double bpos[3], bq[4];
            for (int i = 0; i < 3; ++i) bpos[i] = m->body_pos[b][i];
            for (int i = 0; i < 4; ++i) bq[i] = m->body_quat[b][i];
            if (isfree) {
                for (int i = 0; i < 3; ++i) pl[i] = S.qpos[bjq + i];
                for (int i = 0; i < 4; ++i) qlq[i] = S.qpos[bjq + 3 + i];
                normalize4(qlq);
                quat2mat(Rl, qlq);
                for (int i = 0; i < 3; ++i) { S.x.s.xanchor[bj0][i] = pl[i]; S.x.s.xaxis[bj0][i] = (i == 2) ? 1.0 : 0.0; }
            } else {
                for (int i = 0; i < 9; ++i) Rl[i] = m->body_mat[b][i];
                for (int i = 0; i < 3; ++i) pl[i] = bpos[i];
                for (int i = 0; i < 4; ++i) qlq[i] = bq[i];
                int jt_n = 0, qa_n = 0;
                double jp_n[3] = {0, 0, 0}, ja_n[3] = {0, 0, 0}, ref_n = 0;
                if (bjn > 0) {
                    jt_n = m->jnt_type[bj0]; qa_n = m->jnt_qposadr[bj0]; ref_n = m->jnt_ref[bj0];
                    for (int i = 0; i < 3; ++i) { jp_n[i] = m->jnt_pos[bj0][i]; ja_n[i] = m->jnt_axis[bj0][i]; }
                }
                for (int jj = 0; jj < bjn; ++jj) {
                    const int j = bj0 + jj, jt = jt_n, qa = qa_n;
                    const double jref = ref_n;
                    double jp[3] = {jp_n[0], jp_n[1], jp_n[2]}, ja[3] = {ja_n[0], ja_n[1], ja_n[2]};
                    if (jj + 1 < bjn) {
                        jt_n = m->jnt_type[j + 1]; qa_n = m->jnt_qposadr[j + 1]; ref_n = m->jnt_ref[j + 1];
                        for (int i = 0; i < 3; ++i) { jp_n[i] = m->jnt_pos[j + 1][i]; ja_n[i] = m->jnt_axis[j + 1][i]; }
                    }
                    double al[3], xl[3];
                    mulmatvec3(al, Rl, jp);
                    for (int i = 0; i < 3; ++i) al[i] += pl[i];
                    mulmatvec3(xl, Rl, ja);
                    for (int i = 0; i < 3; ++i) { S.x.s.xanchor[j][i] = al[i]; S.x.s.xaxis[j][i] = xl[i]; }
                    if (jt == CM_JNT_SLIDE) {
                        const double sl = S.qpos[qa] - jref;
                        for (int i = 0; i < 3; ++i) pl[i] += xl[i] * sl;
                    } else {
                        double qj[4];
                        if (jt == CM_JNT_BALL) { for (int i = 0; i < 4; ++i) qj[i] = S.qpos[qa + i]; normalize4(qj); }
                        else {
                            const double ang = S.qpos[qa] - jref;
                            const double sn = sin(0.5 * ang);
                            qj[0] = cos(0.5 * ang); qj[1] = ja[0] * sn; qj[2] = ja[1] * sn; qj[3] = ja[2] * sn;
                        }
                        double Rq[9], Rn[9], r[3];
                        quat2mat(Rq, qj);
                        for (int i = 0; i < 3; ++i)
                            for (int c = 0; c < 3; ++c) Rn[3 * i + c] = Rl[3 * i] * Rq[c] + Rl[3 * i + 1] * Rq[3 + c] + Rl[3 * i + 2] * Rq[6 + c];
                        for (int i = 0; i < 9; ++i) Rl[i] = Rn[i];
                        if (need_quat) mulquat(qlq, qlq, qj);
                        mulmatvec3(r, Rl, jp);
                        for (int i = 0; i < 3; ++i) pl[i] = al[i] - r[i];
                    }
                }
            }
        }
        CK_STAMP(16);
        const int pf_b = isbody ? b : 0, pf_g = lane < m->ngeom ? lane : -1, pf_gs = pf_g >= 0 ? pf_g : 0;
        const int pf_jpb = lane < njnt ? m->jnt_parentbody[lane] : -1, pf_gb = m->geom_bodyid[pf_gs];
        const double pf_mass = P->body_mass[pf_b];
        double pf_ipos[3], pf_imat[9], pf_iner[3], pf_gpos[3], pf_gmat[9];
        for (int i = 0; i < 3; ++i) { pf_ipos[i] = P->body_ipos[pf_b][i]; pf_iner[i] = P->body_inertia[pf_b][i]; pf_gpos[i] = PG->geom_pos[pf_gs][i]; }
        for (int i = 0; i < 9; ++i) { pf_imat[i] = m->body_imat[pf_b][i]; pf_gmat[i] = PG->geom_mat[pf_gs][i]; }
        double xm[9], xp[3], xq[4];
        for (int i = 0; i < 9; ++i) xm[i] = Rl[i];
        for (int i = 0; i < 3; ++i) xp[i] = pl[i];
        for (int i = 0; i < 4; ++i) xq[i] = qlq[i];
        {
            double *bufB = &S.x.s.cinert[0][0];
            auto park = [&](bool in_pose_tiles) {
// ... 20 lines not shown
                for (int i = 0; i < 3; ++i) xp[i] = pn[i];
                if (need_quat) mulquat(xq, qa, xq);
            };
            constexpr bool first_in_pose_tiles = (kin_rounds & 1) == 0;
            park(first_in_pose_tiles);
#pragma unroll
            for (int r = 0; r < kin_rounds; ++r) {
                const bool from_pose_tiles = first_in_pose_tiles == ((r & 1) == 0);
                const int a1 = kanc[2 * r], a2 = kanc[2 * r + 1];
                double R1[9], p1[3], q1[4] = {1, 0, 0, 0}, R2[9], p2[3], q2[4] = {1, 0, 0, 0};
                if (from_pose_tiles) {
                    for (int i = 0; i < 9; ++i) { R1[i] = S.x.s.xmat[a1][i]; R2[i] = S.x.s.xmat[a2][i]; }
                    for (int i = 0; i < 3; ++i) { p1[i] = S.x.s.xpos[a1][i]; p2[i] = S.x.s.xpos[a2][i]; }
                    if (need_quat) for (int i = 0; i < 4; ++i) { q1[i] = S.x.s.xquat[a1][i]; q2[i] = S.x.s.xquat[a2][i]; }
                } else {
                    for (int i = 0; i < 9; ++i) { R1[i] = bufB[a1 * 17 + i]; R2[i] = bufB[a2 * 17 + i]; }
                    for (int i = 0; i < 3; ++i) { p1[i] = bufB[a1 * 17 + 9 + i]; p2[i] = bufB[a2 * 17 + 9 + i]; }
                    if (need_quat) for (int i = 0; i < 4; ++i) { q1[i] = bufB[a1 * 17 + 12 + i]; q2[i] = bufB[a2 * 17 + 12 + i]; }
                }
                if (a1 > 0) compose(R1, p1, q1);
                if (a2 > 0) compose(R2, p2, q2);
                park(!from_pose_tiles);
            }
        }
        if (b == 0) for (int i = 0; i < 3; ++i) S.x.s.xipos[0][i] = 0;
        double ximat[9] = {1, 0, 0, 0, 1, 0, 0, 0, 1};
        if (isbody && b > 0) {
            double xi[3];
            const double *ip = pf_ipos, *im = pf_imat;
            mulmatvec3(xi, xm, ip);
            for (int i = 0; i < 3; ++i) S.x.s.xipos[b][i] = xp[i] + xi[i];
            for (int i = 0; i < 3; ++i)
                for (int c = 0; c < 3; ++c) ximat[3 * i + c] = xm[3 * i] * im[c] + xm[3 * i + 1] * im[3 + c] + xm[3 * i + 2] * im[6 + c];
        }
        const int jpb = pf_jpb;
        if (jpb >= 0) {
            const int pb = jpb;
            double al[3] = {S.x.s.xanchor[lane][0], S.x.s.xanchor[lane][1], S.x.s.xanchor[lane][2]};
            double xl[3] = {S.x.s.xaxis[lane][0], S.x.s.xaxis[lane][1], S.x.s.xaxis[lane][2]}, aw[3], xw[3];
            mulmatvec3(aw, S.x.s.xmat[pb], al);
            mulmatvec3(xw, S.x.s.xmat[pb], xl);
            for (int i = 0; i < 3; ++i) { S.x.s.xanchor[lane][i] = aw[i] + S.x.s.xpos[pb][i]; S.x.s.xaxis[lane][i] = xw[i]; }
        }
        if constexpr (NW == 2) wv::block_barrier();
        if constexpr (NW == 2 && prio_kin != CK_PRIO_W0) wv::set_priority<CK_PRIO_W0>();
        CK_STAMP(1);

        if (pf_g >= 0) {
            const int g = pf_g, gb = pf_gb;
            const double *gp = pf_gpos, *gm = pf_gmat;
            double t[3];
            const double *R = S.x.s.xmat[gb];
            mulmatvec3(t, R, gp);
            for (int i = 0; i < 3; ++i) S.x.s.geom_xpos[g][i] = t[i] + S.x.s.xpos[gb][i];
            for (int i = 0; i < 3; ++i)
                for (int c = 0; c < 3; ++c) S.x.s.geom_xmat[g][3 * i + c] = R[3 * i] * gm[c] + R[3 * i + 1] * gm[3 + c] + R[3 * i + 2] * gm[6 + c];
        }
        if constexpr (NW == 2) wv::sync();

        CK_STAMP(17);
        double col[NVP], colh[NVP];
        if constexpr (NW == 1) mass_matrix_columns<NVP, TOPO, FEAT, NW>(io, S, m, env, ids, pf_mass, pf_iner, ximat, col, colh);

        constexpr bool by_height = TOPO::is_static;
        if constexpr (NW == 2) {
        } else if constexpr (by_height) {
            factor_pair_by_height<NVP, TOPO>(m, P, h, S, col, colh, lane);
        } else {
            factor_pair_in_registers<NVP, TOPO>(m, P, h, col, colh, lane, nv, S.dinv, S.rsd, S.dinvH);
            if (isdof) {
#pragma unroll
                for (int k = 1; k < NVP; ++k) {
                    if (TOPO::is_static ? k >= TOPO::nv : k >= nv) continue;
                    if (k > k_) { S.Lp[CK_TRI(k, k_)] = col[k]; S.LHp[CK_TRI(k, k_)] = colh[k]; }
                }
            }
        }
        if constexpr (NW == 1) CK_STAMP(4);

#include "env_step_collision.inc"

        double mycvel[6], mycacc[6];
#pragma unroll
        for (int r = 0; r < 3 * chain_rounds; ++r) { wv::keep(danc[r]); if (!isdof) danc[r] = -1; }
        wv::keep(blast); wv::keep(kvin);
        if (!isbody) blast = -1;
        if (!isdof) kvin = -1;
        const int kd = isdof ? k_ : 0;
        const double kdamp = P->dof_damping[kd], kstiff = PS->dof_stiffness[kd], kref = PS->dof_springref[kd];
        const double kgear = m->dof_gear[kd], klo = m->dof_ctrl_lo[kd], khi = m->dof_ctrl_hi[kd];
        const int kq = m->dof_qadr[kd], ka = m->dof_act[kd];
        auto chain_sums = [&](double (&acc)[6]) {
            if (lane < NVP) for (int t = 0; t < 6; ++t) S.x.s.buf[lane][t] = acc[t];
            wv::sync();
#pragma unroll
            for (int r = 0; r < chain_rounds; ++r) {
                double up[3][6];
#pragma unroll
                for (int i = 0; i < 3; ++i) {
                    const int a = danc[3 * r + i] >= 0 ? danc[3 * r + i] : 0;
                    for (int t = 0; t < 6; ++t) up[i][t] = S.x.s.buf[a][t];
                }
                wv::sync();
#pragma unroll
                for (int i = 0; i < 3; ++i)
                    if (danc[3 * r + i] >= 0) for (int t = 0; t < 6; ++t) acc[t] += up[i][t];
                if (lane < NVP) for (int t = 0; t < 6; ++t) S.x.s.buf[lane][t] = acc[t];
                wv::sync();
            }
        };
        {
            double term[6];
            const double qd = isdof ? S.qvel[lane < NVP ? lane : 0] : 0.0;
            for (int t = 0; t < 6; ++t) term[t] = (lane < NVP ? S.cdof[lane < NVP ? lane : 0][t] : 0.0) * qd;
            chain_sums(term);
            for (int t = 0; t < 6; ++t) mycvel[t] = blast >= 0 ? S.x.s.buf[blast >= 0 ? blast : 0][t] : 0.0;
            double vin[6];
            for (int t = 0; t < 6; ++t) vin[t] = kvin >= 0 ? S.x.s.buf[kvin >= 0 ? kvin : 0][t] : 0.0;
            if (lane < NB) for (int t = 0; t < 6; ++t) S.x.s.cvel[lane][t] = mycvel[t];
            if (lane < NVP) {
                double cdd[6] = {0, 0, 0, 0, 0, 0}, cd[6];
                for (int i = 0; i < 6; ++i) cd[i] = S.cdof[lane][i];
                if (isdof && !(kjt == CM_JNT_FREE && k_ - kda < 3)) cross_motion(cdd, vin, cd);
                for (int i = 0; i < 6; ++i) S.x.s.cdof_dot[lane][i] = cdd[i];
                for (int t = 0; t < 6; ++t) term[t] = cdd[t] * qd;
            } else {
                for (int t = 0; t < 6; ++t) term[t] = 0;
            }
            wv::sync();
            CK_STAMP(23);
            chain_sums(term);
            for (int t = 0; t < 6; ++t) mycacc[t] = blast >= 0 ? S.x.s.buf[blast >= 0 ? blast : 0][t] : 0.0;
            mycacc[3] -= m->gravity[0]; mycacc[4] -= m->gravity[1]; mycacc[5] -= m->gravity[2];
            wv::sync();
            if (lane < NB) for (int t = 0; t < 6; ++t) S.x.s.buf[lane][t] = mycacc[t];
            wv::sync();
        }
        if (lane < NB) {
            double f6[6] = {0, 0, 0, 0, 0, 0};
            if (isbody && b > 0) {
                double t1[6], t2[6], t3[6], ci[10];
                for (int i = 0; i < 10; ++i) ci[i] = S.x.s.cinert[b][i];
                mul_inert_vec(t1, ci, mycacc);
                mul_inert_vec(t2, ci, mycvel);
                cross_force(t3, mycvel, t2);
                for (int i = 0; i < 6; ++i) f6[i] = t1[i] + t3[i];
            }
            for (int i = 0; i < 6; ++i) S.x.s.cfrc[lane][i] = f6[i];
        }
        wv::sync();
        CK_STAMP(24);
        if constexpr (NW == 2) {
            wv::publish(&S.cmd[1], sub + 1);
        } else bias_forces_and_qfrc_smooth<NVP>(io, S, m, env, ids, kdamp, kstiff, kref, kgear, klo, khi, kq, ka);
        const int pf_eq = lane < 3 * m->neq ? lane / 3 : 0;
        int pf_eb1 = m->eq_body1[pf_eq], pf_eb2 = m->eq_body2[pf_eq], pf_er1 = m->eq_root[pf_eq][0], pf_er2 = m->eq_root[pf_eq][1];

#include "env_step_rows.inc"

#include "env_step_solve.inc"

    if (io.progress && lane == 0 && (!io.resume || bailed)) {
        io.progress[env] = bailed ? sub : nsub;
        if (bailed && !bailed_down && io.handover_out_list) io.handover_out_list[io.env0 + wv::atomic_add(io.handover_out_count, 1)] = env;
    }
    if (io.integrate && io.drive_mode) {
        drive_state_store(io, S, env, lane);
        if (lane < nu) io.ctrl[(size_t)env * io.su + lane] = S.ctrl[lane];
        if (bailed) {
            if (lane < m->nsensordata) io.sensordata[(size_t)env * io.ssd + lane] = S.sens[lane];
            if (lane < nu) io.actuator_velocity[(size_t)env * io.su + lane] = S.actvel[lane];
            if (lane < CM_NUM_DRIVES) {
                double *meas = io.meas + (size_t)env * CM_MEAS_DIM;
                meas[CM_MEAS_DRIVE_POS + lane] = S.drv_pos[lane]; meas[CM_MEAS_DRIVE_VEL + lane] = S.drv_vel[lane];
            }
        }
    }
    if (io.integrate) {
        if (lane < nq) io.qpos[(size_t)env * io.sq + lane] = S.qpos[lane];
        if (lane < nv) {
            io.qvel[(size_t)env * io.sqv + lane] = S.qvel[lane];
            io.qacc_warmstart[(size_t)env * io.sv + lane] = S.qacc_ws[lane];
        }
        if (lane == 0) io.time[env] = time;
    }
    {
        int w = 0;
        for (int bit = 1; bit <= 8; bit <<= 1)
            if (wv::ballot((warn & bit) != 0) != 0ull) w |= bit;
        if (lane == 0 && w) io.warn[env] |= w;
    }
    return (warn & WARN_DIVERGED) ? -2 : (bailed ? (bailed_down ? sub | ENV_STEP_WENT_DOWN : sub) : nsub);
}

template <int NVP, class TOPO, int FEAT = FEAT_ALL, int MAXR = MID_ROWS, int NW = 1, bool WALK = false, int WPS = NW, int INROWS = 0>
WV_GLOBAL void __launch_bounds__(WV_WAVE * NW) WV_OCC WV_WAVES_PER_SIMD(WPS) cassie_step_kernel(PhysIO io) {
    WV_SHARED EnvShared<NVP, LPack<TOPO, NVP>::count, MAXR> S;
    const int slot = wv::env_id();
    if constexpr (WALK) {
        wv::test_launch_hook(&S, sizeof S);
        const int count = wv::opaque(wv::shfl_i(wv::lane() == 0 ? wv::atomic_add(io.handover_count, 0) : 0, 0));
        for (int idx = slot; idx < count; idx += wv::grid_size()) {
            const int env = io.handover_list[io.env0 + idx];
            const long long t0 = io.cost ? wv::clock() : 0, t0w = io.cost_wall ? wv::wall_clock() : 0;
            env_step<NVP, TOPO, FEAT, MAXR, NW>(io, S, env, io.progress[env], io.nsub);
            if (io.cost && wv::lane() == 0 && (NW == 1 || wv::wave_id() == 0)) {
                io.cost[env] += (unsigned)((wv::clock() - t0) >> 6);
                if (io.cost_wall) io.cost_wall[env] += (unsigned)(wv::wall_clock() - t0w);
            }
            if constexpr (NW == 2) wv::block_barrier();
            else wv::sync();
        }
        if (wv::lane() == 0 && (NW == 1 || wv::wave_id() == 0) && wv::atomic_add(io.handover_count + 1, 1) == wv::grid_size() - 1) {
            io.handover_count[0] = 0; io.handover_count[1] = 0;
            if (io.handover_seen) *io.handover_seen = count;
        }
    } else {
    const int chunk = io.nchunk > 1 ? wv::env_id() / io.nenv : 0;
    const int eslot = slot - chunk * io.nenv;
    if (chunk >= (io.nchunk > 1 ? io.nchunk : 1)) return;
    wv::test_launch_hook(&S, sizeof S);
    const int env = io.order ? io.order[io.env0 + eslot] : io.env0 + eslot;
    int sub_start = io.resume ? io.progress[env] : 0, sub_end = io.nsub;
    if (io.nchunk > 1) {
        const int per = (io.nsub + io.nchunk - 1) / io.nchunk;
        sub_start = chunk * per;
        sub_end = sub_start + per < io.nsub ? sub_start + per : io.nsub;
    }
    if (sub_start >= io.nsub) return;
    if (chunk > 0) {
        if (!wv::wait_global<NW>(io.chunk_flag + env, io.chunk_seq, chunk)) {
            if (wv::lane() == 0) { wv::atomic_or(io.warn + env, WARN_CHUNK_PLACEMENT); if (io.chunk_fault) *io.chunk_fault = 1; }
        }
        if (io.progress[env] != sub_start) {
            if (sub_end < io.nsub) wv::publish_global<NW>(io.chunk_flag + env, io.chunk_seq, chunk + 1);
            return;
        }
    }
    const long long t0 = io.cost ? wv::clock() : 0, t0w = io.cost_wall ? wv::wall_clock() : 0;
    if constexpr (INROWS > 0) {
        static_assert(NW == 2 && INROWS > MAXR && INROWS <= MID_ROWS, "the in-place form: a two-wave fast instantiation with the 63-row code behind it");
        static_assert(sizeof(EnvShared<NVP, LPack<TOPO, NVP>::count, MAXR>) == sizeof(EnvShared<NVP, LPack<TOPO, NVP>::count, INROWS>), "both instantiations use the env's LDS block alike");
        auto &S2 = reinterpret_cast<EnvShared<NVP, LPack<TOPO, NVP>::count, INROWS> &>(S);
        PhysIO io2 = io;
        io2.has_next = io.inplace_has_next; io2.handover_out_list = io.inplace_out_list; io2.handover_out_count = io.inplace_out_count;
        io2.down_rows = io.inplace_stay_rows;
        const bool stay = io.inplace_stay_rows > 0;
        bool did = false;
        for (int s = sub_start;;) {
            int at = env_step<NVP, TOPO, FEAT, MAXR, NW>(io, S, env, s, sub_end);
            if (wv::lane() == 0 && wv::wave_id() == 0) S.cmd[5] = at;
            wv::drain_vmem(); wv::block_barrier();
            at = wv::opaque(S.cmd[5]);
            if (at < 0 || at >= sub_end) break;
            did = true;
            int at2 = env_step<NVP, TOPO, FEAT, INROWS, NW>(io2, S2, env, at, stay ? sub_end : at + 1);
            if (wv::lane() == 0 && wv::wave_id() == 0) S.cmd[5] = at2;
            wv::drain_vmem(); wv::block_barrier();
            at2 = wv::opaque(S.cmd[5]);
            if (at2 < 0) break;
            const bool down = (at2 & ENV_STEP_WENT_DOWN) != 0;
            at2 &= ENV_STEP_WENT_DOWN - 1;
            if (at2 >= sub_end) break;
            if (stay ? !down : at2 != at + 1) break;
            s = at2;
        }
        if (did && io.inplace_count && wv::lane() == 0 && wv::wave_id() == 0) wv::atomic_add(io.inplace_count, 1);
    } else env_step<NVP, TOPO, FEAT, MAXR, NW>(io, S, env, sub_start, sub_end);
    if (sub_end < io.nsub) wv::publish_global<NW>(io.chunk_flag + env, io.chunk_seq, chunk + 1);
    if (io.prof && wv::lane() == 0) io.prof[(size_t)env * NSTAMP + 40 + (NW == 2 ? wv::wave_id() : 0)] = wv::hw_id();
    if (io.prof && wv::lane() == 0 && (NW == 1 || wv::wave_id() == 0)) {
        io.prof[(size_t)env * NSTAMP + 42] = wv::clock(); io.prof[(size_t)env * NSTAMP + 43] = wv::wall_clock();
    }
    if (io.cost && wv::lane() == 0 && (NW == 1 || wv::wave_id() == 0)) {
        const unsigned c = (unsigned)((wv::clock() - t0) >> 6);
        io.cost[env] = io.resume || chunk > 0 ? io.cost[env] + c : c;
        if (io.cost_wall) { const unsigned cw = (unsigned)(wv::wall_clock() - t0w); io.cost_wall[env] = io.resume || chunk > 0 ? io.cost_wall[env] + cw : cw; }
    }
    }
}

}
#endif
```

cassie-mujoco-sim_amd/csrc/pk_stages.h:

```cpp
#ifndef CASSIE_PK_STAGES_H
#define CASSIE_PK_STAGES_H

namespace ck {

WV_DEVICE int drive_sensor_slot(int i) { return i < 5 ? i : i + 3; }
WV_DEVICE int joint_sensor_slot(int j) { return j < 3 ? j + 5 : j + 10; }

#define WV_DRIVE_FN WV_DEVICE
template <class SH>
WV_DEVICE void drive_state_load(const PhysIO &io, SH &S, int env, int lane) {
    const cm_drive_state_t *ds = io.drive_state + env;
    const double *meas = io.meas + (size_t)env * CM_MEAS_DIM;
    if (lane < CM_NUM_DRIVES) {
        for (int k = 0; k < CM_DRIVE_FILTER_NB; ++k) S.drv_x[lane][k] = ds->drive_x[lane][k];
        for (int k = 0; k < CM_TORQUE_DELAY_CYCLES; ++k) S.drv_delay[lane][k] = ds->torque_delay[lane][k];
        S.drv_pos[lane] = meas[CM_MEAS_DRIVE_POS + lane]; S.drv_vel[lane] = meas[CM_MEAS_DRIVE_VEL + lane];
        if (lane == 0) S.drv_msg[0] = ds->safety_msg;
    } else if (lane < CM_NUM_DRIVES + CM_NUM_JOINTS) {
        const int j = lane - CM_NUM_DRIVES;
        for (int k = 0; k < CM_JOINT_FILTER_NB; ++k) S.drv_jx[j][k] = ds->joint_x[j][k];
        for (int k = 0; k < CM_JOINT_FILTER_NA; ++k) S.drv_jy[j][k] = ds->joint_y[j][k];
    }
}
template <class SH>
WV_DEVICE void drive_state_store(const PhysIO &io, SH &S, int env, int lane) {
    cm_drive_state_t *ds = io.drive_state + env;
    if (lane < CM_NUM_DRIVES) {
        for (int k = 0; k < CM_DRIVE_FILTER_NB; ++k) ds->drive_x[lane][k] = S.drv_x[lane][k];
        for (int k = 0; k < CM_TORQUE_DELAY_CYCLES; ++k) ds->torque_delay[lane][k] = S.drv_delay[lane][k];
        if (lane == 0) ds->safety_msg = S.drv_msg[0];
    } else if (lane < CM_NUM_DRIVES + CM_NUM_JOINTS) {
        const int j = lane - CM_NUM_DRIVES;
        for (int k = 0; k < CM_JOINT_FILTER_NB; ++k) ds->joint_x[j][k] = S.drv_jx[j][k];
        for (int k = 0; k < CM_JOINT_FILTER_NA; ++k) ds->joint_y[j][k] = S.drv_jy[j][k];
    }
}

enum { DRVC_RATIO = 0, DRVC_TMAX, DRVC_WMAX, DRVC_COUNTS, DRVC_SCALE, DRVC_U_OR_PT, DRVC_STO_OR_DT, DRVC_FF, DRVC_KP, DRVC_KD };
template <class SH>
WV_DEVICE void drive_consts_load(const PhysIO &io, SH &S, ModelPtr m, int env, int lane) {
    const double TWO_PI = 2 * 3.14159265358979323846, PI = 3.14159265358979323846;
    const int nu = m->nu;
    if (lane < CM_NUM_DRIVES) {
        const int i = lane, bits = m->sensor_bits[drive_sensor_slot(i)];
        const double ratio = m->act_gear[i], counts = (double)(1 << bits);
        double *c = S.drv_c[i];
        c[DRVC_RATIO] = ratio; c[DRVC_TMAX] = m->act_ctrlrange[i][1];
        c[DRVC_WMAX] = wv::div_rn(wv::mul_rn(wv::mul_rn(m->act_maxrpm[i], 2.0), PI), 60.0);
        c[DRVC_COUNTS] = counts; c[DRVC_SCALE] = wv::div_rn(wv::div_rn(TWO_PI, counts), ratio);
        if (io.drive_mode == CM_DRIVE_TORQUE) {
            c[DRVC_U_OR_PT] = io.drive_cmd[(size_t)env * (nu + 1) + i];
            c[DRVC_STO_OR_DT] = io.drive_cmd[(size_t)env * (nu + 1) + nu] != 0.0 ? 1.0 : 0.0;
            c[DRVC_FF] = 0.0; c[DRVC_KP] = 0.0; c[DRVC_KD] = 0.0;
        } else {
            const size_t o = (size_t)env * nu + i;
            c[DRVC_U_OR_PT] = io.pd_ptarget[o]; c[DRVC_STO_OR_DT] = io.pd_dtarget ? io.pd_dtarget[o] : 0.0;
            c[DRVC_FF] = io.pd_torque ? io.pd_torque[o] : 0.0; c[DRVC_KP] = io.pd_kp[o]; c[DRVC_KD] = io.pd_kd[o];
            if (i == 0) S.drv_msg[1] = (io.drive_mode == CM_DRIVE_PD_SAFE && io.drive_cmd && io.drive_cmd[(size_t)env * (nu + 1) + nu] != 0.0) ? 1 : 0;
        }
    } else if (lane < CM_NUM_DRIVES + CM_NUM_JOINTS) {
        const int j = lane - CM_NUM_DRIVES, bits = m->sensor_bits[joint_sensor_slot(j)];
        const double counts = (double)(1 << bits);
        S.drv_jc[j][0] = counts; S.drv_jc[j][1] = wv::div_rn(TWO_PI, counts);
    }
}

template <class SH>
WV_DRIVE_FN void drive_level_io(const PhysIO &io, SH &S, ModelPtr m, int env, int lane, bool write_meas) {
    const double TWO_PI = 2 * 3.14159265358979323846, PI = 3.14159265358979323846;
    double *meas = io.meas + (size_t)env * CM_MEAS_DIM;
    double u_safe = 0.0;
    if (io.drive_mode == CM_DRIVE_PD_SAFE) {
        int msg = 0;
        const bool sto = S.drv_msg[1] != 0;
        if (lane < CM_NUM_DRIVES) {
            double qq[CM_NUM_DRIVES];
            for (int k = 0; k < CM_NUM_DRIVES; ++k) qq[k] = S.drv_pos[k];
            const double *c = S.drv_c[lane];
            const double wk = S.drv_vel[lane];
            const double uk = wv::add_rn(wv::add_rn(c[DRVC_FF], wv::mul_rn(c[DRVC_KP], wv::sub_rn(c[DRVC_U_OR_PT], S.drv_pos[lane]))), wv::mul_rn(c[DRVC_KD], wv::sub_rn(c[DRVC_STO_OR_DT], wk)));
            u_safe = safety::drive_torque(lane, uk, qq, wk, safety::torque_limit(lane), sto, &msg);
        }
        const bool lim = wv::ballot((msg & safety::MSG_LIMIT) != 0) != 0ull, trq = wv::ballot((msg & safety::MSG_TORQUE) != 0) != 0ull;
        wv::sync();
        if (lane == 0 && io.integrate) S.drv_msg[0] |= (lim ? safety::MSG_LIMIT : 0) | (trq ? safety::MSG_TORQUE : 0);
    }
    if (lane < CM_NUM_DRIVES) {
        const int i = lane;
        double cst[10];
        for (int k = 0; k < 10; ++k) cst[k] = S.drv_c[i][k];
        const double ratio = cst[DRVC_RATIO], tmax = cst[DRVC_TMAX], wmax = cst[DRVC_WMAX];
        double u;
        bool sto = false;
        if (io.drive_mode == CM_DRIVE_TORQUE) {
            u = cst[DRVC_U_OR_PT];
            sto = cst[DRVC_STO_OR_DT] != 0.0;
        } else if (io.drive_mode == CM_DRIVE_PD_SAFE) {
            u = u_safe;
            sto = S.drv_msg[1] != 0;
        } else {
            const double p = S.drv_pos[i], v = S.drv_vel[i];
            const double pt = cst[DRVC_U_OR_PT], dt = cst[DRVC_STO_OR_DT], ff = cst[DRVC_FF];
            u = wv::add_rn(wv::add_rn(ff, wv::mul_rn(cst[DRVC_KP], wv::sub_rn(pt, p))), wv::mul_rn(cst[DRVC_KD], wv::sub_rn(dt, v)));
        }
        const double w = S.actvel[i];
        double tlim = wv::mul_rn(wv::mul_rn(2.0, tmax), wv::sub_rn(1.0, wv::div_rn(fabs(w), wmax)));
        tlim = fmax(fmin(tlim, tmax), 0.0);
        if (sto) u = 0.0;
        const double tau = copysign(fmin(fabs(wv::div_rn(u, ratio)), tlim), u);
        double dl[CM_TORQUE_DELAY_CYCLES];
        for (int k = 0; k < CM_TORQUE_DELAY_CYCLES; ++k) dl[k] = S.drv_delay[i][k];
        const double ctrl_i = dl[CM_TORQUE_DELAY_CYCLES - 1];
        for (int k = CM_TORQUE_DELAY_CYCLES - 1; k > 0; --k) S.drv_delay[i][k] = dl[k - 1];
        S.drv_delay[i][0] = tau;
        S.ctrl[i] = ctrl_i;
        const int slot = drive_sensor_slot(i);
        const double counts = cst[DRVC_COUNTS], scale = cst[DRVC_SCALE];
        const int ev = (int)wv::mul_rn(wv::div_rn(S.sens[slot], TWO_PI), counts);
        const double pos = wv::mul_rn((double)ev, scale);
        int x[CM_DRIVE_FILTER_NB];
        bool allzero = true;
        for (int k = 0; k < CM_DRIVE_FILTER_NB; ++k) { x[k] = S.drv_x[i][k]; allzero &= x[k] == 0; }
        if (allzero) for (int k = 0; k < CM_DRIVE_FILTER_NB; ++k) x[k] = ev;
        for (int k = CM_DRIVE_FILTER_NB - 1; k > 0; --k) x[k] = x[k - 1];
        x[0] = ev;
        const int fir[CM_DRIVE_FILTER_NB] = {2727, 534, -2658, -795, 72, 110, 19, -6, -3};
        int y = 0;
        for (int k = 0; k < CM_DRIVE_FILTER_NB; ++k) { y += x[k] * fir[k]; S.drv_x[i][k] = x[k]; }
        const double vel = wv::div_rn(wv::mul_rn((double)y, scale), PI);
        S.drv_pos[i] = pos; S.drv_vel[i] = vel;
        if (write_meas) {
            meas[CM_MEAS_DRIVE_POS + i] = pos; meas[CM_MEAS_DRIVE_VEL + i] = vel;
            meas[CM_MEAS_DRIVE_TORQUE + i] = wv::mul_rn(ctrl_i, ratio);
        }
    } else if (lane < CM_NUM_DRIVES + CM_NUM_JOINTS) {
        const int j = lane - CM_NUM_DRIVES, slot = joint_sensor_slot(j);
        const double counts = S.drv_jc[j][0], scale = S.drv_jc[j][1];
        const int ev = (int)wv::mul_rn(wv::div_rn(S.sens[slot], TWO_PI), counts);
        const double pos = wv::mul_rn((double)ev, scale);
        double x[CM_JOINT_FILTER_NB], yv[CM_JOINT_FILTER_NA];
        bool allzero = true;
        for (int k = 0; k < CM_JOINT_FILTER_NB; ++k) { x[k] = S.drv_jx[j][k]; allzero &= x[k] == 0; }
        for (int k = 0; k < CM_JOINT_FILTER_NA; ++k) yv[k] = S.drv_jy[j][k];
        if (allzero) for (int k = 0; k < CM_JOINT_FILTER_NB; ++k) x[k] = pos;
        for (int k = CM_JOINT_FILTER_NB - 1; k > 0; --k) x[k] = x[k - 1];
        x[0] = pos;
        for (int k = CM_JOINT_FILTER_NA - 1; k > 0; --k) yv[k] = yv[k - 1];
        const double fb[CM_JOINT_FILTER_NB] = {12.348, 12.348, -12.348, -12.348}, fa[CM_JOINT_FILTER_NA] = {1.0, -1.7658, 0.79045};
        double y0 = 0.0;
        for (int k = 0; k < CM_JOINT_FILTER_NB; ++k) y0 = wv::add_rn(y0, wv::mul_rn(x[k], fb[k]));
        for (int k = 1; k < CM_JOINT_FILTER_NA; ++k) y0 = wv::sub_rn(y0, wv::mul_rn(yv[k], fa[k]));
        yv[0] = y0;
        for (int k = 0; k < CM_JOINT_FILTER_NB; ++k) S.drv_jx[j][k] = x[k];
        for (int k = 0; k < CM_JOINT_FILTER_NA; ++k) S.drv_jy[j][k] = yv[k];
        if (write_meas) { meas[CM_MEAS_JOINT_POS + j] = pos; meas[CM_MEAS_JOINT_VEL + j] = y0; }
    } else if (lane < 29) {
        if (write_meas) meas[CM_MEAS_ORIENTATION + (lane - 16)] = S.sens[lane];
    }
}

enum { FEAT_HFIELD = 1, FEAT_WAVEPAIRS = 2, FEAT_ALL = 3 };

struct LaneIds { int nbody, nv, broot, bend, kjnt, kbody, kjt, kda, kroot, kbend; unsigned long long kdesc; };

template <int NVP, class TOPO, int FEAT, int NW, class SH>
WV_DEVICE void mass_matrix_columns(const PhysIO &io, SH &S, ModelPtr m, int env, const LaneIds &ids, const double pf_mass, const double (&pf_iner)[3],
                                   const double (&ximat)[9], double (&col)[NVP], double (&colh)[NVP]) {
    const int nbody = ids.nbody, nv = ids.nv, broot = ids.broot, bend = ids.bend, kjnt = ids.kjnt, kbody = ids.kbody, kjt = ids.kjt, kda = ids.kda, kroot = ids.kroot;
    const unsigned long long kdesc = ids.kdesc;
    int lane = wv::fresh_lane(), b = lane, k_ = lane;
    bool isbody = b < nbody, isdof = k_ < nv;
    constexpr bool cbuf_over_anchors = NW == 2 && (FEAT & FEAT_HFIELD) != 0;
    static_assert(!cbuf_over_anchors || NVP <= CM_MAXJNT, "crb . cdof (NVP x 6) must fit the xanchor + xaxis tiles");
    static_assert(offsetof(decltype(S.x.s), xaxis) - offsetof(decltype(S.x.s), xanchor) == sizeof(double) * CM_MAXJNT * 3, "xanchor and xaxis are contiguous");
    double (*const cbuf)[6] = cbuf_over_anchors ? reinterpret_cast<double (*)[6]>(&S.x.s.xanchor[0][0]) : S.x.s.buf;
    const double bmass = (isbody && b > 0) ? pf_mass : 0.0;
    {
        const double px = isbody ? S.x.s.xipos[b < NB ? b : 0][0] : 0.0, py = isbody ? S.x.s.xipos[b < NB ? b : 0][1] : 0.0,
                     pz = isbody ? S.x.s.xipos[b < NB ? b : 0][2] : 0.0;
        for (int ri = 0; ri < m->nroot; ++ri) {
            const int r = m->root_body[ri], e = m->body_subtreeend[r];
            const double w = (isbody && b >= r && b < e) ? bmass : 0.0;
            const double sm = wv::wave_sum(w), sx = wv::wave_sum(w * px), sy = wv::wave_sum(w * py), sz = wv::wave_sum(w * pz);
            if (lane == 0) {
                if (sm < CM_MINVAL) { S.com[r][0] = S.x.s.xipos[r][0]; S.com[r][1] = S.x.s.xipos[r][1]; S.com[r][2] = S.x.s.xipos[r][2]; }
                else { const double inv = 1.0 / sm; S.com[r][0] = sx * inv; S.com[r][1] = sy * inv; S.com[r][2] = sz * inv; }
            }
        }
    }
    wv::sync();
    CK_STAMP(18);
    if (lane < NB) {
        double ci[10] = {0, 0, 0, 0, 0, 0, 0, 0, 0, 0};
        if (isbody && b > 0) {
            const double I0 = pf_iner[0], I1 = pf_iner[1], I2 = pf_iner[2];
            const double *c = S.com[broot];
            double dif[3] = {S.x.s.xipos[b][0] - c[0], S.x.s.xipos[b][1] - c[1], S.x.s.xipos[b][2] - c[2]};
            double d2 = dot3(dif, dif);
            const double *R = ximat;
            double W00 = R[0] * I0 * R[0] + R[1] * I1 * R[1] + R[2] * I2 * R[2];
            double W11 = R[3] * I0 * R[3] + R[4] * I1 * R[4] + R[5] * I2 * R[5];
            double W22 = R[6] * I0 * R[6] + R[7] * I1 * R[7] + R[8] * I2 * R[8];
            double W01 = R[0] * I0 * R[3] + R[1] * I1 * R[4] + R[2] * I2 * R[5];
            double W02 = R[0] * I0 * R[6] + R[1] * I1 * R[7] + R[2] * I2 * R[8];
            double W12 = R[3] * I0 * R[6] + R[4] * I1 * R[7] + R[5] * I2 * R[8];
            ci[0] = W00 + bmass * (d2 - dif[0] * dif[0]);
            ci[1] = W11 + bmass * (d2 - dif[1] * dif[1]);
            ci[2] = W22 + bmass * (d2 - dif[2] * dif[2]);
            ci[3] = W01 - bmass * dif[0] * dif[1];
            ci[4] = W02 - bmass * dif[0] * dif[2];
            ci[5] = W12 - bmass * dif[1] * dif[2];
            ci[6] = bmass * dif[0]; ci[7] = bmass * dif[1]; ci[8] = bmass * dif[2]; ci[9] = bmass;
        }
        for (int i = 0; i < 10; ++i) S.x.s.cinert[lane][i] = ci[i];
    }
    {
    double cd[6] = {0, 0, 0, 0, 0, 0};
    if (isdof) {
        const double *c = S.com[kroot];
        double off[3] = {c[0] - S.x.s.xanchor[kjnt][0], c[1] - S.x.s.xanchor[kjnt][1], c[2] - S.x.s.xanchor[kjnt][2]};
        const int sub_k = k_ - kda;
        if (kjt == CM_JNT_SLIDE) {
            for (int i = 0; i < 3; ++i) cd[3 + i] = S.x.s.xaxis[kjnt][i];
        } else if (kjt == CM_JNT_HINGE) {
            for (int i = 0; i < 3; ++i) cd[i] = S.x.s.xaxis[kjnt][i];
            cross3(cd + 3, cd, off);
        } else if (kjt == CM_JNT_FREE && sub_k < 3) {
            cd[3 + sub_k] = 1.0;
        } else {
            const int a = (kjt == CM_JNT_FREE) ? sub_k - 3 : sub_k;
            cd[0] = S.x.s.xmat[kbody][a]; cd[1] = S.x.s.xmat[kbody][3 + a]; cd[2] = S.x.s.xmat[kbody][6 + a];
            cross3(cd + 3, cd, off);
        }
    }
    if (lane < NVP) for (int i = 0; i < 6; ++i) S.cdof[lane][i] = cd[i];
    }
    wv::sync();
    CK_STAMP(2);

    {
        const int mi = lane & 15, mk = lane >> 4;
        const unsigned mine = (isbody && b > 0) ? (unsigned)(((1ull << bend) - 1ull) ^ ((1ull << b) - 1ull)) : 0u;
        const unsigned w0 = (unsigned)wv::shfl_i((int)mine, mi) >> mk, w1 = (unsigned)wv::shfl_i((int)mine, 16 + mi) >> mk;
        double bv[NB / 4];
#pragma unroll
        for (int kb = 0; kb < NB / 4; ++kb) { const double v = S.x.s.cinert[4 * kb + mk][mi < 10 ? mi : 0]; bv[kb] = mi < 10 ? v : 0.0; }
        wv::mfma_acc d0a = {{0, 0, 0, 0}}, d0b = {{0, 0, 0, 0}}, d1a = {{0, 0, 0, 0}}, d1b = {{0, 0, 0, 0}};
#pragma unroll
        for (int kb = 0; kb < NB / 4; kb += 2)
            wv::mfma_f64_16x16x4_x4((double)((w0 >> (4 * kb)) & 1u), bv[kb], d0a, (double)((w1 >> (4 * kb)) & 1u), bv[kb], d1a,
                                    (double)((w0 >> (4 * kb + 4)) & 1u), bv[kb + 1], d0b, (double)((w1 >> (4 * kb + 4)) & 1u), bv[kb + 1], d1b);
        wv::mfma_f64_drain4(d0a, d0b, d1a, d1b);
        if (mi < 10) {
#pragma unroll
            for (int v = 0; v < 4; ++v) {
                S.x.s.crb[mk + 4 * v][mi] = d0a.c[v] + d0b.c[v];
                S.x.s.crb[16 + mk + 4 * v][mi] = d1a.c[v] + d1b.c[v];
            }
        }
    }
    wv::sync();
    CK_STAMP(19);
    if (lane < NVP) {
        double bf[6] = {0, 0, 0, 0, 0, 0}, cd[6];
        for (int i = 0; i < 6; ++i) cd[i] = S.cdof[lane][i];
        if (isdof) mul_inert_vec(bf, S.x.s.crb[kbody], cd);
        for (int i = 0; i < 6; ++i) cbuf[lane][i] = bf[i];
    }
    wv::sync();
    CK_STAMP(20);
    double cdm[6];
    if constexpr (NVP == 32) {
        const int hk = lane & 31, roff = lane < 32 ? 0 : 16;
        const unsigned hdesc = (unsigned)wv::shfl_i((int)(unsigned)kdesc, hk) >> roff;
        for (int i = 0; i < 6; ++i) cdm[i] = S.cdof[hk][i];
        const double (*bufr)[6] = &cbuf[roff];
        double part[16];
#pragma unroll
        for (int i0 = 0; i0 < 16; i0 += 8) {
            double bb[8][6];
#pragma unroll
            for (int ii = 0; ii < 8; ++ii)
#pragma unroll
                for (int t = 0; t < 6; ++t) bb[ii][t] = bufr[i0 + ii][t];
            wv::sched_fence();
#pragma unroll
            for (int ii = 0; ii < 8; ++ii) {
                const double v = (cdm[0] * bb[ii][0] + cdm[1] * bb[ii][1]) + (cdm[2] * bb[ii][2] + cdm[3] * bb[ii][3]) + (cdm[4] * bb[ii][4] + cdm[5] * bb[ii][5]);
                part[i0 + ii] = ((hdesc >> (i0 + ii)) & 1u) ? v : 0.0;
            }
        }
#pragma unroll
        for (int i = 0; i < 16; ++i) {
            const double up = wv::from_upper_half(part[i]);
            col[i] = part[i]; colh[i] = part[i];
            col[16 + i] = up; colh[16 + i] = up;
        }
    } else {
    for (int i = 0; i < 6; ++i) cdm[i] = S.cdof[lane < NVP ? lane : 0][i];
#pragma unroll
    for (int i0 = 0; i0 < NVP; i0 += 8) {
        double bb[8][6];
#pragma unroll
        for (int ii = 0; ii < 8; ++ii)
#pragma unroll
            for (int t = 0; t < 6; ++t) bb[ii][t] = cbuf[i0 + ii][t];
        wv::sched_fence();
#pragma unroll
        for (int ii = 0; ii < 8; ++ii) {
            const int i = i0 + ii;
            double v = (cdm[0] * bb[ii][0] + cdm[1] * bb[ii][1]) + (cdm[2] * bb[ii][2] + cdm[3] * bb[ii][3]) + (cdm[4] * bb[ii][4] + cdm[5] * bb[ii][5]);
            if (TOPO::is_static ? (i >= TOPO::nv || !((kdesc >> i) & 1ull)) : !(i < nv && ((kdesc >> i) & 1ull))) v = 0;
            col[i] = v;
            colh[i] = v;
        }
    }
    }
    if (io.ext && isdof) {
        cm_ext_t *ex = io.ext + env;
#pragma unroll
        for (int i = 0; i < NVP; ++i) if (i < nv && i >= k_) { const double v = (i == k_) ? col[i] + m->dof_armature[k_] : col[i]; ex->qM[i][k_] = v; ex->qM[k_][i] = v; }
    }
    CK_STAMP(3);
}

template <int NVP, bool ROLLED = false, class SH>
WV_DEVICE void bias_forces_and_qfrc_smooth(const PhysIO &io, SH &S, ModelPtr m, int env, const LaneIds &ids, const double kdamp, const double kstiff,
                                           const double kref, const double kgear, const double klo, const double khi, const int kq, const int ka) {
    const int nbody = ids.nbody, nv = ids.nv, kbody = ids.kbody, kbend = ids.kbend;
    int lane = wv::fresh_lane(), b = lane, k_ = lane;
    bool isbody = b < nbody, isdof = k_ < nv;
    double qfrc_bias = 0;
    if constexpr (NVP == 32) {
        double acc[6] = {0, 0, 0, 0, 0, 0};
        const int hk = lane & 31, hkbody = wv::shfl_i(kbody, hk), hkbend = wv::shfl_i(kbend, hk), coff = lane < 32 ? 0 : NB / 2;
        const unsigned ksub = hk < nv ? (unsigned)(((1ull << hkbend) - 1ull) ^ ((1ull << hkbody) - 1ull)) >> coff : 0u;
        const double (*cfr)[6] = &S.x.s.cfrc[coff];
#pragma unroll
        for (int c0 = 0; c0 < NB / 2; c0 += 4) {
            double ff[4][6];
#pragma unroll
            for (int cc = 0; cc < 4; ++cc)
#pragma unroll
                for (int t = 0; t < 6; ++t) ff[cc][t] = cfr[c0 + cc][t];
            wv::sched_fence();
#pragma unroll
            for (int cc = 0; cc < 4; ++cc) {
                const double w = bitf(ksub, c0 + cc);
#pragma unroll
                for (int t = 0; t < 6; ++t) acc[t] = fma(w, ff[cc][t], acc[t]);
            }
        }
        for (int i = 0; i < 6; ++i) { acc[i] += wv::from_upper_half(acc[i]); qfrc_bias += S.cdof[lane < NVP ? lane : 0][i] * acc[i]; }
    } else {
        double acc[6] = {0, 0, 0, 0, 0, 0};
        const unsigned ksub = isdof ? (unsigned)(((1ull << kbend) - 1ull) ^ ((1ull << kbody) - 1ull)) : 0u;
#pragma unroll(ROLLED ? 1 : NB / 4)
        for (int c0 = 0; c0 < NB; c0 += 4) {
            double ff[4][6];
#pragma unroll
            for (int cc = 0; cc < 4; ++cc)
#pragma unroll
                for (int t = 0; t < 6; ++t) ff[cc][t] = S.x.s.cfrc[c0 + cc][t];
            wv::sched_fence();
#pragma unroll
            for (int cc = 0; cc < 4; ++cc) {
                const double w = bitf(ksub, c0 + cc);
#pragma unroll
                for (int t = 0; t < 6; ++t) acc[t] = fma(w, ff[cc][t], acc[t]);
            }
        }
        for (int i = 0; i < 6; ++i) qfrc_bias += S.cdof[lane < NVP ? lane : 0][i] * acc[i];
    }
    CK_STAMP(6);

    {
        if (isdof) {
            double f = -kdamp * S.qvel[k_];
            f -= kstiff * (S.qpos[kq] - kref);
            f -= qfrc_bias;
            if (io.qfrc_applied) f += io.qfrc_applied[(size_t)env * io.sv + k_];
            f += kgear * clampd(S.ctrl[ka], klo, khi);
            S.qfrc_smooth[k_] = f;
        }
    }
    if (io.xfrc_applied) {
        if (isdof) {
            const double *xfa = io.xfrc_applied + ((size_t)env * io.sb) * 6;
            double f = 0;
            for (int bb = 1; bb < nbody; ++bb) {
                if (!((m->body_dofmask[bb] >> k_) & 1ull)) continue;
                const double xf[6] = {xfa[bb * 6], xfa[bb * 6 + 1], xfa[bb * 6 + 2], xfa[bb * 6 + 3], xfa[bb * 6 + 4], xfa[bb * 6 + 5]};
                if (xf[0] == 0 && xf[1] == 0 && xf[2] == 0 && xf[3] == 0 && xf[4] == 0 && xf[5] == 0) continue;
                const double *c = S.com[m->body_rootid[bb]];
                double off[3] = {S.x.s.xipos[bb][0] - c[0], S.x.s.xipos[bb][1] - c[1], S.x.s.xipos[bb][2] - c[2]};
                double t[3], cdk[6];
                for (int i = 0; i < 6; ++i) cdk[i] = S.cdof[k_][i];
                cross3(t, cdk, off);
                for (int i = 0; i < 3; ++i) f += (cdk[3 + i] + t[i]) * xf[i] + cdk[i] * xf[3 + i];
            }
            S.qfrc_smooth[k_] += f;
        }
    }
    wv::sync();
    CK_STAMP(7);
}

template <int NVP, class TOPO, class SH>
WV_DEVICE void stage_factor_row(const SH &S, int k_, bool isdof, double (&lrow)[NVP]) {
    typedef LPack<TOPO, NVP> LP;
    const typename LP::Row myrow = LP::row_of(k_);
#pragma unroll
    for (int i = 0; i < NVP; ++i) {
        if constexpr (LP::packed) {
            const bool has = isdof && i < k_ && LP::row_has(myrow, i);
            const double v = S.Lp[has ? LP::row_idx(myrow, i) : 0];
            lrow[i] = has ? v : 0.0;
        } else lrow[i] = (isdof && i < k_) ? S.Lp[CK_TRI(k_, i)] : 0.0;
    }
}
template <int NVP, class TOPO, int WHICH = 2, class SH>
WV_DEVICE void stage_factor_h(const SH &S, int k_, bool isdof, int nv, double (&lcol)[NVP], double (&lrowh)[NVP]) {
    typedef LPack<TOPO, NVP> LP;
    const typename LP::Row myrow = LP::row_of(k_);
#pragma unroll
    for (int k = 0; k < NVP; ++k) {
        const bool inrange = TOPO::is_static ? k < TOPO::nv : k < nv;
        if constexpr (LP::packed) {
            if constexpr (WHICH != 1) {
                const bool hasc = inrange && isdof && k > k_ && LP::col_has(k, k_);
                const double vc = S.LHp[hasc ? LP::col_idx(k, k_) : 0];
                lcol[k] = hasc ? vc : 0.0;
            }
            if constexpr (WHICH != 0) {
                const bool hasr = isdof && k < k_ && LP::row_has(myrow, k);
                const double vr = S.LHp[hasr ? LP::row_idx(myrow, k) : 0];
                lrowh[k] = hasr ? vr : 0.0;
            }
        } else {
            if constexpr (WHICH != 1) lcol[k] = (inrange && isdof && k > k_) ? S.LHp[CK_TRI(k, k_)] : 0.0;
            if constexpr (WHICH != 0) lrowh[k] = (isdof && k < k_) ? S.LHp[CK_TRI(k_, k)] : 0.0;
        }
    }
}
struct SensorConsts { int stype, slot, sqadr, sb, sroot, sdim, sadr; double sgain, scut; };
WV_DEVICE SensorConsts request_sensor_consts(ModelPtr m, int ls) {
    SensorConsts c;
    c.stype = m->sensor_type[ls]; c.slot = m->sensor_slot[ls];
    c.sqadr = m->sensor_qadr[ls]; c.sb = m->sensor_body[ls]; c.sroot = m->sensor_root[ls];
    c.sdim = m->sensor_dim[ls]; c.sadr = m->sensor_adr[ls];
    c.sgain = m->sensor_gain[ls]; c.scut = m->sensor_cutoff[ls];
    return c;
}
template <class SH>
WV_DEVICE int sensors_before_solve(const PhysIO &io, SH &S, ModelPtr m, int env, bool issens, int ls, SensorConsts sc, bool need_imu, bool lastsub) {
    int stype = sc.stype, slot_ = sc.slot;
    const int sqadr = sc.sqadr, sb = sc.sb, sroot = sc.sroot, sdim = sc.sdim, sadr = sc.sadr;
    const double sgain = sc.sgain, scut = sc.scut;
    wv::keep(stype); wv::keep(slot_);
    if (!issens) stype = -1;
    const int aslot = (stype == CM_SENS_ACCELEROMETER) ? slot_ : -1;
    if (issens) {
        double sout[4] = {0, 0, 0, 0};
        if (sqadr >= 0) sout[0] = sgain * S.qpos[sqadr];
        else if (need_imu && stype >= CM_SENS_FRAMEQUAT && stype <= CM_SENS_MAGNETOMETER) {
            double sq[4] = {m->sensor_squat[ls][0], m->sensor_squat[ls][1], m->sensor_squat[ls][2], m->sensor_squat[ls][3]};
            double q[4], sxmat[9], scvel[6];
            mulquat(q, S.x.s.xquat[sb], sq);
            quat2mat(sxmat, q);
            for (int i = 0; i < 6; ++i) scvel[i] = S.x.s.cvel[sb][i];
            if (stype == CM_SENS_FRAMEQUAT) { for (int i = 0; i < 4; ++i) sout[i] = q[i]; }
            else if (stype == CM_SENS_GYRO) mulmatTvec3(sout, sxmat, scvel);
            else if (stype == CM_SENS_MAGNETOMETER) {
                double mg[3] = {m->magnetic[0], m->magnetic[1], m->magnetic[2]};
                mulmatTvec3(sout, sxmat, mg);
            } else if (aslot >= 0) {
                double acc_ang[3] = {S.x.s.buf[sb][0], S.x.s.buf[sb][1], S.x.s.buf[sb][2]};
                double acc_lin[3] = {S.x.s.buf[sb][3], S.x.s.buf[sb][4], S.x.s.buf[sb][5]};
                double sp[3] = {m->sensor_spos[ls][0], m->sensor_spos[ls][1], m->sensor_spos[ls][2]}, t[3];
// ... 103 lines not shown
```

cassie-mujoco-sim_amd/csrc/pk_types.h:

```cpp
#ifndef CASSIE_PK_TYPES_H
#define CASSIE_PK_TYPES_H

namespace ck {

constexpr int NB = CM_MAXBODY;
constexpr int NG = CM_MAXGEOM;
constexpr int NROW = 64;
constexpr int MID_ROWS = CM_MAXEFC_NARROW;
constexpr int WIDE_ROWS = CM_MAXEFC;
constexpr int FAST_ROWS = 31;
constexpr int FAST_ROWS_TRAY = 47;
constexpr int NSTAMP = 48;
#define CK_TRI(k, i) ((k) * ((k) + 1) / 2 + (i))
#define CK_STAMP(i) do { if (io.prof && lane == 0) io.prof[(size_t)env * NSTAMP + (i)] = wv::clock(); CK_FRESH(); } while (0)
#define CK_FRESH() do { lane = wv::fresh_lane(); b = lane; k_ = lane; isbody = b < nbody; isdof = k_ < nv; } while (0)

enum { WARN_CONTACT_FULL = 1, WARN_CONSTRAINT_FULL = 2, WARN_UNSUPPORTED_PAIR = 4, WARN_DIVERGED = 8,
       WARN_CHUNK_PLACEMENT = 16 ,
       WARN_TERRAIN_INDEX = 32   ,
       WARN_SCAN_TILTED = 64     ,
       WARN_PLACE_MISS = 128      };

#ifndef WV_OCC
#define WV_OCC
#endif
typedef const WV_CONST_AS cm_model_t *ModelPtr;
typedef const WV_CONST_AS cm_envparams_t *ParamPtr;

struct PhysIO {
    const cm_model_t *models;
    int model_stride;
    const cm_envparams_t *envparams;
    int nenv, nsub;
    int env0;
    int integrate;
    int sq, sqv, sv, su, ssd, sb;
    double *qpos, *qvel, *qacc_warmstart, *time;
    double *ctrl;
    const double *qfrc_applied, *xfrc_applied;
    double *qacc, *sensordata, *actuator_velocity;
    int *warn;
    int *info;
    double *xpos_out;
    double *xquat_out;
    double *body_cfrc;
    const float *hfield;
    size_t hfield_stride;
    const double *pd_ptarget, *pd_kp, *pd_kd;
    int drive_mode;
    cm_drive_state_t *drive_state;
    const double *drive_cmd;
    const double *pd_dtarget, *pd_torque;
    double *meas;
    cm_ext_t *ext;
    long long *prof;
    const int *order;
    unsigned *cost;
    unsigned *cost_wall;
    int all_outputs_every_substep;
    int *progress;
    int resume;
    int nchunk, chunk_seq;
    int *chunk_flag;
    volatile int *chunk_fault;
    int *handover_list, *handover_count;
    volatile int *handover_seen;
    int has_next;
    int *handover_out_list, *handover_out_count;
    int inplace_has_next;
    int *inplace_out_list, *inplace_out_count;
    int inplace_stay_rows;
    int down_rows;
    int *inplace_count;
    const int *hfield_index;
    int hfield_nterrain;
};

WV_DEVICE const float *terrain_grid(const float *hfield, size_t stride, const int *index, int nterrain, int env, bool *clamped) {
    *clamped = false;
    if (!hfield) return nullptr;
    if (!index) return hfield + (size_t)env * stride;
    const int want = index[env], last = nterrain - 1;
    const int t = want > last ? last : (want < 0 ? 0 : want);
    *clamped = t != want;
    return hfield + (size_t)(t < 0 ? 0 : t) * stride;
}

template <int NVP>
struct BodyTiles {
    double xpos[NB][3], xquat[NB][4], xmat[NB][9], xipos[NB][3];
    double xanchor[CM_MAXJNT][3], xaxis[CM_MAXJNT][3];
    double cinert[NB][10], crb[NB][10];
    double cvel[NB][6], cfrc[NB][6];
    double cdof_dot[NVP][6], buf[NVP][6];
    double geom_xpos[NG][3], geom_xmat[NG][9];
};
template <int NVP, int MAXR, bool SEPARATE> struct TilesAndY {
    static constexpr int YP = NVP + 2;
    union { BodyTiles<NVP> s; double Yr[MAXR + 1][YP]; };
};
template <int NVP, int MAXR> struct TilesAndY<NVP, MAXR, true> {
    static constexpr int YP = NVP + 2;
    BodyTiles<NVP> s;
    double Yr[MAXR + 1][YP];
    double rowt[MAXR + 1][4];
    double vx[2][NVP];
    double sums[8];
    int turn[4];
    double stepv[2][NROW];
    double chg[NROW];
};
template <int NVP, int NL = NVP * (NVP + 1) / 2, int MAXR = MID_ROWS>
struct EnvShared {
    static constexpr int YP = NVP + 2;
    static constexpr bool WIDE = MAXR > MID_ROWS;
    static constexpr int MAXC = WIDE ? CM_MAXCON : CM_MAXCON_NARROW;
    TilesAndY<NVP, MAXR, WIDE> x;
    double Lp[NL], LHp[NL];
    double accel[2][28];
    double dinv[NVP], rsd[NVP], dinvH[NVP];
    double cdof[NVP][6];
    double com[NB][3];
    double qpos[CM_MAXQ], qvel[NVP], qacc_ws[NVP], qacc[NVP], ctrl[CM_MAXU];
    double qfrc_smooth[NVP];
    double sens[CM_MAXSENSORDATA], actvel[CM_MAXU];
    int drv_x[CM_NUM_DRIVES][CM_DRIVE_FILTER_NB];
    double drv_jx[CM_NUM_JOINTS][CM_JOINT_FILTER_NB], drv_jy[CM_NUM_JOINTS][CM_JOINT_FILTER_NA];
    double drv_delay[CM_NUM_DRIVES][CM_TORQUE_DELAY_CYCLES];
    double drv_pos[CM_NUM_DRIVES], drv_vel[CM_NUM_DRIVES];
    double drv_c[CM_NUM_DRIVES][10], drv_jc[CM_NUM_JOINTS][2];
    int drv_msg[2];
    double c_dist[MAXC], c_pos[MAXC][3], c_frame[MAXC][9], c_fri[MAXC][3];
    double c_solref[MAXC][2], c_solimp[MAXC][5], c_margin[MAXC];
    int c_dim[MAXC], c_g1[MAXC], c_g2[MAXC], c_pair[MAXC];
    int c_root[MAXC][2];
    unsigned long long c_dofmask[MAXC][2];
    double c_tran[MAXC];
    int cmd[6];
};

}
#endif
```

cassie-mujoco-sim_amd/csrc/step_kernels.h:

```cpp
#ifndef CASSIE_STEP_KERNELS_H
#define CASSIE_STEP_KERNELS_H

#include "step_launch.h"

namespace ck {
template <int NVP, class TOPO, int FEAT, int MAXR, int NW, bool WALK, int WPS, int INROWS>
void launch_step(unsigned grid, hipStream_t s, const PhysIO &io) {
    hipLaunchKernelGGL((cassie_step_kernel<NVP, TOPO, FEAT, MAXR, NW, WALK, WPS, INROWS>), dim3(grid), dim3(NW * WV_WAVE), 0, s, io);
}
}
#endif
```

cassie-mujoco-sim_amd/csrc/step_launch.h:

```cpp
#ifndef CASSIE_STEP_LAUNCH_H
#define CASSIE_STEP_LAUNCH_H

#include <hip/hip_runtime.h>

#include "step_plan.h"

namespace ck {
using StepLauncher = void (*)(unsigned grid, hipStream_t s, const PhysIO &io);

template <int NVP, class TOPO, int FEAT = FEAT_ALL, int MAXR = MID_ROWS, int NW = 1, bool WALK = false, int WPS = NW, int INROWS = 0>
void launch_step(unsigned grid, hipStream_t s, const PhysIO &io);
}
#endif
```

cassie-mujoco-sim_amd/csrc/step_plan.h:

```cpp
#ifndef CASSIE_STEP_PLAN_H
#define CASSIE_STEP_PLAN_H

#include "physics_kernel.h"

namespace ck {

enum StepForm {
    FORM_ALONE,
    FORM_ALONE_2W,
    FORM_WIDE,
    FORM_FAST,
    FORM_FAST_2W,
    FORM_FAST_INPLACE,
    FORM_MID_WALK,
    FORM_MID_WALK_2W,
    FORM_WIDE_WALK,
    FORM_COUNT
};

enum StepFamily {
    CASSIE,
    CASSIE_HFIELD,
    CASSIE_ALL,
    TRAY,
    TRAY_HFIELD,
    GENERIC32,
    GENERIC40,
    FAMILY_COUNT
};

template <class TOPO>
inline bool topo_matches(const cm_model_t &m) {
    if (m.nv != TOPO::nv || !m.kin_simple || m.maxdepth > TOPO::body_levels) return false;
    for (int k = 0; k < TOPO::nv; ++k) if (m.dof_ancmask[k] != TOPO::table[k]) return false;
    return true;
}

inline StepFamily pick_family(const cm_model_t &m, bool generic_only) {
    const bool hf = m.nhfpair > 0 || m.hfield_geom >= 0, wp = m.npair > m.npair_simple;
    if (!generic_only && topo_matches<TopoCassie32>(m)) return wp ? CASSIE_ALL : hf ? CASSIE_HFIELD : CASSIE;
    if (!generic_only && topo_matches<TopoCassieTray38>(m)) return hf ? TRAY_HFIELD : TRAY;
    return m.nv > 32 ? GENERIC40 : GENERIC32;
}

struct StepForms {
    int first;
    int mid;
    bool wide;
    int stay_rows;
};

struct HandoverLists {
    int *list1, *count1; volatile int *seen1;
    int *list2, *count2; volatile int *seen2;
};

struct StepGrids { unsigned envs, mid, wide; };

struct StepPass { int form; unsigned grid; PhysIO io; };
struct StepPlan { int n; StepPass pass[3]; };

inline bool is_fast_form(int form) { return form == FORM_FAST || form == FORM_FAST_2W || form == FORM_FAST_INPLACE; }

inline StepPlan plan_step(const PhysIO &base, const StepForms &f, const HandoverLists &hl, const StepGrids &g) {
    StepPlan p;
    p.n = 0;
    PhysIO io = base;
    io.resume = 0;
    io.handover_list = nullptr; io.handover_count = nullptr; io.handover_seen = nullptr;
    io.handover_out_list = nullptr; io.handover_out_count = nullptr;
    if (!is_fast_form(f.first)) {
        io.progress = nullptr; io.has_next = 0; io.nchunk = 1;
        p.pass[p.n++] = {f.first, g.envs, io};
        return p;
    }
    const unsigned fast_grid = g.envs * (unsigned)(io.nchunk > 1 ? io.nchunk : 1);
    io.has_next = 1;
    if (f.first == FORM_FAST_INPLACE) {
        io.inplace_count = hl.count1;
        io.inplace_stay_rows = f.stay_rows;
        io.inplace_has_next = f.wide ? 1 : 0;
        io.inplace_out_list = f.wide ? hl.list2 : nullptr; io.inplace_out_count = f.wide ? hl.count2 : nullptr;
        p.pass[p.n++] = {f.first, fast_grid, io};
    } else {
        const bool walk1 = f.mid != FORM_ALONE;
        io.handover_out_list = walk1 ? hl.list1 : nullptr; io.handover_out_count = walk1 ? hl.count1 : nullptr;
        p.pass[p.n++] = {f.first, fast_grid, io};
        io.resume = 1; io.nchunk = 1; io.has_next = f.wide ? 1 : 0;
        io.handover_out_list = f.wide ? hl.list2 : nullptr; io.handover_out_count = f.wide ? hl.count2 : nullptr;
        if (walk1) { io.handover_list = hl.list1; io.handover_count = hl.count1; io.handover_seen = hl.seen1; }
        p.pass[p.n++] = {f.mid, walk1 ? g.mid : g.envs, io};
    }
    if (f.wide) {
        io.resume = 1; io.nchunk = 1; io.has_next = 0;
        io.handover_out_list = nullptr; io.handover_out_count = nullptr;
        io.handover_list = hl.list2; io.handover_count = hl.count2; io.handover_seen = hl.seen2;
        p.pass[p.n++] = {FORM_WIDE_WALK, g.wide, io};
    }
    return p;
}

}
#endif
```

cassie-mujoco-sim_amd/csrc/step_policy.h:

```cpp
#ifndef CASSIE_STEP_POLICY_H
#define CASSIE_STEP_POLICY_H

#include <vector>

#include "step_plan.h"

namespace ck {


constexpr int SMALL_BATCH_NSUB = 4;
constexpr int SMALL_BATCH = 512;
constexpr int INPLACE_STAY_ROWS = FAST_ROWS - 4;

inline StepForms launch_forms(int fam, bool has_inplace, int maxefc, int integrate, bool ext, int n, int nsub, bool fast_rows,
                              int waves_per_env, int waves_per_env_tray, bool inplace) {
    StepForms forms = {FORM_ALONE, FORM_ALONE, false, INPLACE_STAY_ROWS};
    if (fam == CASSIE || fam == CASSIE_HFIELD) {
        forms.wide = maxefc > CM_MAXEFC_NARROW;
        if (!fast_rows || !integrate || ext || (n <= SMALL_BATCH && nsub <= SMALL_BATCH_NSUB))
            forms.first = forms.wide ? FORM_WIDE : n > SMALL_BATCH ? FORM_ALONE : FORM_ALONE_2W;
        else if (waves_per_env == 2) { forms.first = inplace && has_inplace ? FORM_FAST_INPLACE : FORM_FAST_2W; forms.mid = FORM_MID_WALK_2W; }
        else forms.first = FORM_FAST;
    } else if (fam == TRAY) {
        const bool plain = integrate && !ext, two = plain && waves_per_env_tray == 2;
        if (plain && fast_rows) { forms.first = two ? FORM_FAST_2W : FORM_FAST; forms.mid = two ? FORM_MID_WALK_2W : FORM_MID_WALK; }
        else forms.first = two ? FORM_ALONE_2W : FORM_ALONE;
    }
    return forms;
}


constexpr int DEFAULT_CHUNKS_WHOLE = 7 , DEFAULT_CHUNKS_RANGE = 2, CHUNK_MIN_ENVS = 2048, CHUNK_MIN_SUBSTEPS = 5;
constexpr int SHORT_RANGE_NSUB = 25, SHORT_RANGE_CHUNKS = 3;

inline int launch_chunks(int n, int nenv, int nsub, int chunks, int chunks_range, bool chunks_default) {
    if ((n == nenv ? chunks : chunks_range) <= 1 || n < CHUNK_MIN_ENVS || n % 8 != 0 || nsub < 2 * CHUNK_MIN_SUBSTEPS) return 1;
    const int range_chunks = chunks_default && nsub <= SHORT_RANGE_NSUB ? SHORT_RANGE_CHUNKS : chunks_range;
    const int most = nsub / CHUNK_MIN_SUBSTEPS, asked = n == nenv ? chunks : range_chunks;
    return asked < most ? asked : most;
}


inline StepGrids pass_grids(int n, int seen1, int seen2, bool wide) {
    if (!wide) seen2 = 0;
    const int seen12 = seen1 > seen2 ? seen1 : seen2;
    const long want = 2L * (seen12 > 0 ? seen12 : 0) + 16, want2 = 2L * (seen2 > 0 ? seen2 : 0) + 8;
    return {(unsigned)n, (unsigned)(want < n ? want : n), (unsigned)(want2 < n ? want2 : n)};
}


constexpr int INPLACE_QUIET = 8;

inline bool next_inplace(bool was, int seen, int mode, bool auto_ok) {
    if (mode != 2 || !auto_ok) return mode == 1;
    return was ? seen > -INPLACE_QUIET : seen > 0;
}


constexpr int ORDER_LONG_NSUB = 25, ORDER_EVERY = 16;

inline bool order_kernel_due(int nsub, int launches_since_sort) { return nsub > ORDER_LONG_NSUB || launches_since_sort >= ORDER_EVERY; }


struct LaunchRange { int env0, n; bool inplace; int launches_since_sort; };

struct RangeTable {
    std::vector<LaunchRange> ranges;
    LaunchRange *claim(int env0, int n, std::vector<LaunchRange> &retired) {
        for (auto &r : ranges) if (r.env0 == env0 && r.n == n) return &r;
        for (size_t i = 0; i < ranges.size();) {
            const LaunchRange r = ranges[i];
            if (r.env0 < env0 + n && env0 < r.env0 + r.n) { retired.push_back(r); ranges.erase(ranges.begin() + (long)i); }
            else ++i;
        }
        ranges.push_back({env0, n, false, 0});
        return &ranges.back();
    }
};

}
#endif
```

Before: 27.56 million.

## Specialize fast step kernels into lean variants without readout and profiling branches

Adds a SERVE template parameter with feature bits for readout and profiling, and compiles the fast-path kernels in a lean form where ext writes, the integrate check and CK_STAMP profiling stores are removed at compile time. Separate profiling kernel forms are added and selected when profiling is requested, and a guard refuses lean forms when ext, non-integrating or prof modes are active. The aim is to cut per-substep branches, global stores and register pressure in the hot kernels, at the cost of more kernel instantiations and more complex form selection.

```diff
diff --git a/cassie-mujoco-sim_amd/csrc/env_step_collision.inc b/cassie-mujoco-sim_amd/csrc/env_step_collision.inc
--- a/cassie-mujoco-sim_amd/csrc/env_step_collision.inc
+++ b/cassie-mujoco-sim_amd/csrc/env_step_collision.inc
@@ -321,7 +321,7 @@
         }
         if (ncon_found > capc) warn |= WARN_CONTACT_FULL;
         if constexpr (NW == 1) if (io.drive_mode) {
-            if (io.integrate) drive_level_io(io, S, m, env, lane, lastsub);
+            if (integrates<FEAT>(io)) drive_level_io(io, S, m, env, lane, lastsub);
             wv::sync();
         }
         if constexpr (NW == 2) { CK_STAMP(33); wv::publish(&S.cmd[4], sub + 1); wv::wait_for(&S.cmd[3], sub + 1); }
diff --git a/cassie-mujoco-sim_amd/csrc/env_step_rows.inc b/cassie-mujoco-sim_amd/csrc/env_step_rows.inc
--- a/cassie-mujoco-sim_amd/csrc/env_step_rows.inc
+++ b/cassie-mujoco-sim_amd/csrc/env_step_rows.inc
@@ -186,8 +186,8 @@
                 rt[0] = rR; rt[1] = rtype >= 0 ? -rB * jvel - rK * rimp * (rpos - rmargin) : 0.0; rt[2] = jws;
                 rt[3] = rtype < 0 ? -1.0 : (rtype == CM_CNSTR_EQUALITY ? 0.0 : 1.0);
             }
-            if (io.ext && pass == 0 && rtype == CM_CNSTR_EQUALITY && r_ < CM_MAXEQROW) {
-                cm_ext_t *ex = io.ext + env;
+            if (readout_ext<FEAT>(io) && pass == 0 && rtype == CM_CNSTR_EQUALITY && r_ < CM_MAXEQROW) {
+                cm_ext_t *ex = readout_ext<FEAT>(io) + env;
                 ex->eq_pos[r_] = rpos; ex->eq_id[r_] = rid;
 #pragma unroll
                 for (int k = 0; k < NVP; ++k) if (k < nv) ex->eq_J[r_][k] = ycol[k];
@@ -213,8 +213,8 @@
             for (int i = 0; i < 3; ++i) io.xpos_out[((size_t)env * io.sb + b) * 3 + i] = S.x.s.xpos[b][i];
             if (io.xquat_out) for (int i = 0; i < 4; ++i) io.xquat_out[((size_t)env * io.sb + b) * 4 + i] = S.x.s.xquat[b][i];
         }
-        if (io.ext) {
-            cm_ext_t *ex = io.ext + env;
+        if (readout_ext<FEAT>(io)) {
+            cm_ext_t *ex = readout_ext<FEAT>(io) + env;
             if (isbody) for (int i = 0; i < 6; ++i) ex->cvel[b][i] = S.x.s.cvel[b][i];
             if (isbody) for (int i = 0; i < 3; ++i) { ex->subtree_com[b][i] = S.com[broot > 0 ? broot : 0][i]; ex->xipos[b][i] = S.x.s.xipos[b][i]; }
             if (lane < m->nsite) {
@@ -244,8 +244,8 @@
             }
         }
         int caddr = -1;
-        const bool want_cfrc = io.body_cfrc && (sub == nsub - 1 || !io.integrate);
-        if (io.ext || want_cfrc) {
+        const bool want_cfrc = io.body_cfrc && (sub == nsub - 1 || !integrates<FEAT>(io));
+        if (readout_ext<FEAT>(io) || want_cfrc) {
             int acc = nefc_before_contacts;
             for (int c = 0; c < ncon; ++c) {
                 const int dim = S.c_dim[c];
diff --git a/cassie-mujoco-sim_amd/csrc/env_step_solve.inc b/cassie-mujoco-sim_amd/csrc/env_step_solve.inc
--- a/cassie-mujoco-sim_amd/csrc/env_step_solve.inc
+++ b/cassie-mujoco-sim_amd/csrc/env_step_solve.inc
@@ -9,9 +9,9 @@
             if (lane == 0) { fbuf[2 * NROW] = (double)ncon; fbuf[2 * NROW + 1] = (double)nefc; fbuf[2 * NROW + 2] = (double)iters; fbuf[2 * NROW + 3] = (double)nguarded; }
             wv::block_barrier();
 #ifdef CK_WIDE_PROFILE
-            if (io.prof && lane < 12) io.prof[(size_t)env * NSTAMP + (lane < 6 ? 16 + lane : 22 + lane)] = (long long)S.x.stepv[lane / 6][lane % 6];
+            if constexpr (feat_prof(FEAT)) if (io.prof && lane < 12) io.prof[(size_t)env * NSTAMP + (lane < 6 ? 16 + lane : 22 + lane)] = (long long)S.x.stepv[lane / 6][lane % 6];
 #endif
-            if (io.ext || want_cfrc) {
+            if (readout_ext<FEAT>(io) || want_cfrc) {
                 const int a0 = caddr >= 0 ? caddr : 0;
                 double fn = 0, ft1 = 0, ft2 = 0;
                 if (lane < ncon && caddr >= 0) {
@@ -19,8 +19,8 @@
                     if (S.c_dim[lane] == 1) fn = f0;
                     else { const double f1 = fbuf[a0 + 1], f2 = fbuf[a0 + 2], f3 = fbuf[a0 + 3], mu = S.c_fri[lane][0]; fn = f0 + f1 + f2 + f3; ft1 = mu * (f0 - f1); ft2 = mu * (f2 - f3); }
                 }
-                if (io.ext) {
-                    cm_ext_t *ex = io.ext + env;
+                if (readout_ext<FEAT>(io)) {
+                    cm_ext_t *ex = readout_ext<FEAT>(io) + env;
                     if (lane < ncon) { ex->con_force[lane][0] = fn; ex->con_force[lane][1] = ft1; ex->con_force[lane][2] = ft2; }
                     if (lane == 0) { ex->ncon = ncon; ex->nefc = nefc; ex->solver_iter = iters; }
                 }
@@ -47,7 +47,7 @@
             wv::block_barrier();
             CK_STAMP(37);
             if (wv::opaque(S.cmd[0])) { warn |= WARN_DIVERGED; break; }
-            if (!io.integrate) break;
+            if (!integrates<FEAT>(io)) break;
             time += h;
             continue;
         }
@@ -347,7 +347,7 @@
         }
         if constexpr (NW == 2 && CK_PRIO_W0_PGS != CK_PRIO_W0) wv::set_priority<CK_PRIO_W0>();
         CK_STAMP(11);
-        if (io.ext || want_cfrc) {
+        if (readout_ext<FEAT>(io) || want_cfrc) {
             const int a0 = caddr >= 0 ? caddr : 0;
             const double f0 = wv::shfl(f, a0), f1 = wv::shfl(f, (a0 + 1) & 63), f2 = wv::shfl(f, (a0 + 2) & 63), f3 = wv::shfl(f, (a0 + 3) & 63);
             double fn = 0, ft1 = 0, ft2 = 0;
@@ -355,8 +355,8 @@
                 if (S.c_dim[lane] == 1) fn = f0;
                 else { const double mu = S.c_fri[lane][0]; fn = f0 + f1 + f2 + f3; ft1 = mu * (f0 - f1); ft2 = mu * (f2 - f3); }
             }
-            if (io.ext) {
-                cm_ext_t *ex = io.ext + env;
+            if (readout_ext<FEAT>(io)) {
+                cm_ext_t *ex = readout_ext<FEAT>(io) + env;
                 if (lane < ncon) { ex->con_force[lane][0] = fn; ex->con_force[lane][1] = ft1; ex->con_force[lane][2] = ft2; }
                 if (lane == 0) { ex->ncon = ncon; ex->nefc = nefc; ex->solver_iter = iters; }
             }
@@ -390,7 +390,7 @@
             wv::block_barrier();
             CK_STAMP(37);
             if (wv::opaque(S.cmd[0])) { warn |= WARN_DIVERGED; break; }
-            if (!io.integrate) break;
+            if (!integrates<FEAT>(io)) break;
             time += h;
             continue;
         }
@@ -427,7 +427,7 @@
         CK_STAMP(12);
 
         outputs_after_qacc(io, S, m, env, lane, isdof, k_, nu, qacc, aslot, sb, need_imu, lastsub, pf_agear * S.qvel[pf_adof], ncon, nefc, iters, nguarded);
-        if (!io.integrate) break;
+        if (!integrates<FEAT>(io)) break;
         CK_STAMP(13);
 
         {
diff --git a/cassie-mujoco-sim_amd/csrc/env_step_wave1.inc b/cassie-mujoco-sim_amd/csrc/env_step_wave1.inc
--- a/cassie-mujoco-sim_amd/csrc/env_step_wave1.inc
+++ b/cassie-mujoco-sim_amd/csrc/env_step_wave1.inc
@@ -38,7 +38,7 @@
                 wv::wait_for(&S.cmd[4], sub1 + 1);
                 if (wv::opaque(S.cmd[0])) return -1;
                 if (io.drive_mode) {
-                    if (io.integrate) drive_level_io(io, S, m, env, lane, sub1 == nsub - 1);
+                    if (integrates<FEAT>(io)) drive_level_io(io, S, m, env, lane, sub1 == nsub - 1);
                     wv::sync();
                 }
                 CK_STAMP(4);
@@ -48,9 +48,9 @@
                     const double kgear = m->dof_gear[kd], klo = m->dof_ctrl_lo[kd], khi = m->dof_ctrl_hi[kd];
                     const int kq = m->dof_qadr[kd], ka = m->dof_act[kd];
                     wv::wait_for(&S.cmd[1], sub1 + 1);
-                    bias_forces_and_qfrc_smooth<NVP, (NVP > 32)>(io, S, m, env, ids, kdamp, kstiff, kref, kgear, klo, khi, kq, ka);
+                    bias_forces_and_qfrc_smooth<NVP, FEAT, (NVP > 32)>(io, S, m, env, ids, kdamp, kstiff, kref, kgear, klo, khi, kq, ka);
                 }
-                const bool lastsub1 = sub1 == nsub - 1 || !io.integrate;
+                const bool lastsub1 = sub1 == nsub - 1 || !integrates<FEAT>(io);
                 const bool need_imu1 = lastsub1 || io.all_outputs_every_substep || (io.drive_mode && sub1 + 2 == nsub);
                 const bool issens1 = lane < m->nsensor && (lastsub1 || io.drive_mode || io.all_outputs_every_substep);
                 const int ls1 = issens1 ? lane : 0;
@@ -148,7 +148,7 @@
                     const double av = pf_agear * S.qvel[pf_adof];
                     wv::sync();
                     CK_STAMP(12);
-                    if (io.integrate) {
+                    if (integrates<FEAT>(io)) {
                         if constexpr (!stage_h_early) stage_factor_h<NVP, TOPO>(S, k_, isdof, nv, lcol, lrowh);
                         euler_step<NVP, TOPO>(S, m, lane, isdof, k_, nv, njnt, h, qacc, lcol, lrowh, dih, pf_kdamp, pf_ejt, pf_eqa, pf_eda);
                     }
@@ -158,7 +158,7 @@
                     outputs_after_qacc(io, S, m, env, lane, isdof, k_, nu, qacc, aslot, sb, need_imu, lastsub, av, ncon, nefc, iters, nguarded);
                     CK_STAMP(14);
                 }
-                if (!io.integrate || ++sub1 >= nsub) return -1;
+                if (!integrates<FEAT>(io) || ++sub1 >= nsub) return -1;
             }
         }
     }
diff --git a/cassie-mujoco-sim_amd/csrc/kernels_cassie.hip b/cassie-mujoco-sim_amd/csrc/kernels_cassie.hip
--- a/cassie-mujoco-sim_amd/csrc/kernels_cassie.hip
+++ b/cassie-mujoco-sim_amd/csrc/kernels_cassie.hip
@@ -1,5 +1,5 @@
 #include "step_kernels.h"
 namespace ck {
 template void launch_step<32, TopoCassie32, 0>(unsigned, hipStream_t, const PhysIO &);
-template void launch_step<32, TopoCassie32, 0, FAST_ROWS>(unsigned, hipStream_t, const PhysIO &);
+template void launch_step<32, TopoCassie32, 0, FAST_ROWS, 1, false, 1, 0, FEAT_LEAN>(unsigned, hipStream_t, const PhysIO &);
 }
diff --git a/cassie-mujoco-sim_amd/csrc/kernels_cassie_2w.hip b/cassie-mujoco-sim_amd/csrc/kernels_cassie_2w.hip
--- a/cassie-mujoco-sim_amd/csrc/kernels_cassie_2w.hip
+++ b/cassie-mujoco-sim_amd/csrc/kernels_cassie_2w.hip
@@ -1,4 +1,4 @@
 #include "step_kernels.h"
 namespace ck {
-template void launch_step<32, TopoCassie32, 0, FAST_ROWS, 2>(unsigned, hipStream_t, const PhysIO &);
+template void launch_step<32, TopoCassie32, 0, FAST_ROWS, 2, false, 2, 0, FEAT_LEAN>(unsigned, hipStream_t, const PhysIO &);
 }
diff --git a/cassie-mujoco-sim_amd/csrc/kernels_cassie_2w_inplace.hip b/cassie-mujoco-sim_amd/csrc/kernels_cassie_2w_inplace.hip
--- a/cassie-mujoco-sim_amd/csrc/kernels_cassie_2w_inplace.hip
+++ b/cassie-mujoco-sim_amd/csrc/kernels_cassie_2w_inplace.hip
@@ -1,4 +1,4 @@
 #include "step_kernels.h"
 namespace ck {
-template void launch_step<32, TopoCassie32, 0, FAST_ROWS, 2, false, 2, MID_ROWS>(unsigned, hipStream_t, const PhysIO &);
+template void launch_step<32, TopoCassie32, 0, FAST_ROWS, 2, false, 2, MID_ROWS, FEAT_LEAN>(unsigned, hipStream_t, const PhysIO &);
 }
diff --git a/cassie-mujoco-sim_amd/csrc/kernels_cassie_prof.hip b/cassie-mujoco-sim_amd/csrc/kernels_cassie_prof.hip
--- /dev/null
+++ b/cassie-mujoco-sim_amd/csrc/kernels_cassie_prof.hip
@@ -0,0 +1,5 @@
+#include "step_kernels.h"
+namespace ck {
+template void launch_step<32, TopoCassie32, 0, FAST_ROWS, 1, false, 1, 0, FEAT_PROF>(unsigned, hipStream_t, const PhysIO &);
+template void launch_step<32, TopoCassie32, 0, FAST_ROWS, 2, false, 2, 0, FEAT_PROF>(unsigned, hipStream_t, const PhysIO &);
+}
diff --git a/cassie-mujoco-sim_amd/csrc/kernels_hfield.hip b/cassie-mujoco-sim_amd/csrc/kernels_hfield.hip
--- a/cassie-mujoco-sim_amd/csrc/kernels_hfield.hip
+++ b/cassie-mujoco-sim_amd/csrc/kernels_hfield.hip
@@ -1,5 +1,5 @@
 #include "step_kernels.h"
 namespace ck {
 template void launch_step<32, TopoCassie32, FEAT_HFIELD>(unsigned, hipStream_t, const PhysIO &);
-template void launch_step<32, TopoCassie32, FEAT_HFIELD, FAST_ROWS>(unsigned, hipStream_t, const PhysIO &);
+template void launch_step<32, TopoCassie32, FEAT_HFIELD, FAST_ROWS, 1, false, 1, 0, FEAT_LEAN>(unsigned, hipStream_t, const PhysIO &);
 }
diff --git a/cassie-mujoco-sim_amd/csrc/kernels_hfield_2w.hip b/cassie-mujoco-sim_amd/csrc/kernels_hfield_2w.hip
--- a/cassie-mujoco-sim_amd/csrc/kernels_hfield_2w.hip
+++ b/cassie-mujoco-sim_amd/csrc/kernels_hfield_2w.hip
@@ -1,4 +1,4 @@
 #include "step_kernels.h"
 namespace ck {
-template void launch_step<32, TopoCassie32, FEAT_HFIELD, FAST_ROWS, 2>(unsigned, hipStream_t, const PhysIO &);
+template void launch_step<32, TopoCassie32, FEAT_HFIELD, FAST_ROWS, 2, false, 2, 0, FEAT_LEAN>(unsigned, hipStream_t, const PhysIO &);
 }
diff --git a/cassie-mujoco-sim_amd/csrc/kernels_hfield_2w_inplace.hip b/cassie-mujoco-sim_amd/csrc/kernels_hfield_2w_inplace.hip
--- a/cassie-mujoco-sim_amd/csrc/kernels_hfield_2w_inplace.hip
+++ b/cassie-mujoco-sim_amd/csrc/kernels_hfield_2w_inplace.hip
@@ -1,4 +1,4 @@
 #include "step_kernels.h"
 namespace ck {
-template void launch_step<32, TopoCassie32, FEAT_HFIELD, FAST_ROWS, 2, false, 2, MID_ROWS>(unsigned, hipStream_t, const PhysIO &);
+template void launch_step<32, TopoCassie32, FEAT_HFIELD, FAST_ROWS, 2, false, 2, MID_ROWS, FEAT_LEAN>(unsigned, hipStream_t, const PhysIO &);
 }
diff --git a/cassie-mujoco-sim_amd/csrc/kernels_hfield_prof.hip b/cassie-mujoco-sim_amd/csrc/kernels_hfield_prof.hip
--- /dev/null
+++ b/cassie-mujoco-sim_amd/csrc/kernels_hfield_prof.hip
@@ -0,0 +1,5 @@
+#include "step_kernels.h"
+namespace ck {
+template void launch_step<32, TopoCassie32, FEAT_HFIELD, FAST_ROWS, 1, false, 1, 0, FEAT_PROF>(unsigned, hipStream_t, const PhysIO &);
+template void launch_step<32, TopoCassie32, FEAT_HFIELD, FAST_ROWS, 2, false, 2, 0, FEAT_PROF>(unsigned, hipStream_t, const PhysIO &);
+}
diff --git a/cassie-mujoco-sim_amd/csrc/kernels_tray_2w.hip b/cassie-mujoco-sim_amd/csrc/kernels_tray_2w.hip
--- a/cassie-mujoco-sim_amd/csrc/kernels_tray_2w.hip
+++ b/cassie-mujoco-sim_amd/csrc/kernels_tray_2w.hip
@@ -1,4 +1,4 @@
 #include "step_kernels.h"
 namespace ck {
-template void launch_step<40, TopoCassieTray38, FEAT_WAVEPAIRS, FAST_ROWS_TRAY, 2>(unsigned, hipStream_t, const PhysIO &);
+template void launch_step<40, TopoCassieTray38, FEAT_WAVEPAIRS, FAST_ROWS_TRAY, 2, false, 2, 0, FEAT_READOUT>(unsigned, hipStream_t, const PhysIO &);
 }
diff --git a/cassie-mujoco-sim_amd/csrc/kernels_tray_fast.hip b/cassie-mujoco-sim_amd/csrc/kernels_tray_fast.hip
--- a/cassie-mujoco-sim_amd/csrc/kernels_tray_fast.hip
+++ b/cassie-mujoco-sim_amd/csrc/kernels_tray_fast.hip
@@ -1,5 +1,5 @@
 #include "step_kernels.h"
 namespace ck {
-template void launch_step<40, TopoCassieTray38, FEAT_WAVEPAIRS, FAST_ROWS_TRAY>(unsigned, hipStream_t, const PhysIO &);
+template void launch_step<40, TopoCassieTray38, FEAT_WAVEPAIRS, FAST_ROWS_TRAY, 1, false, 1, 0, FEAT_LEAN>(unsigned, hipStream_t, const PhysIO &);
 template void launch_step<40, TopoCassieTray38, FEAT_WAVEPAIRS, MID_ROWS, 1, true>(unsigned, hipStream_t, const PhysIO &);
 }
diff --git a/cassie-mujoco-sim_amd/csrc/kernels_tray_prof.hip b/cassie-mujoco-sim_amd/csrc/kernels_tray_prof.hip
--- /dev/null
+++ b/cassie-mujoco-sim_amd/csrc/kernels_tray_prof.hip
@@ -0,0 +1,5 @@
+#include "step_kernels.h"
+namespace ck {
+template void launch_step<40, TopoCassieTray38, FEAT_WAVEPAIRS, FAST_ROWS_TRAY, 1, false, 1, 0, FEAT_PROF>(unsigned, hipStream_t, const PhysIO &);
+template void launch_step<40, TopoCassieTray38, FEAT_WAVEPAIRS, FAST_ROWS_TRAY, 2, false, 2, 0, FEAT_FULL>(unsigned, hipStream_t, const PhysIO &);
+}
diff --git a/cassie-mujoco-sim_amd/csrc/phys_batch.hip b/cassie-mujoco-sim_amd/csrc/phys_batch.hip
--- a/cassie-mujoco-sim_amd/csrc/phys_batch.hip
+++ b/cassie-mujoco-sim_amd/csrc/phys_batch.hip
@@ -185,28 +185,33 @@
 using ck::launch_step;
 using ck::FAST_ROWS; using ck::FAST_ROWS_TRAY; using ck::MID_ROWS; using ck::WIDE_ROWS;
 using ck::TopoCassie32; using ck::TopoCassieTray38; using ck::TopoRuntime;
+using ck::FEAT_LEAN; using ck::FEAT_PROF; using ck::FEAT_READOUT; using ck::FEAT_FULL;
 template <int FEAT>
 static const ck::StepLauncher CASSIE_FORMS[ck::FORM_COUNT] = {
     launch_step<32, TopoCassie32, FEAT>,
     launch_step<32, TopoCassie32, FEAT, MID_ROWS, 2, false, 1>,
     launch_step<32, TopoCassie32, FEAT, WIDE_ROWS, 2, false, 1>,
-    launch_step<32, TopoCassie32, FEAT, FAST_ROWS>,
-    launch_step<32, TopoCassie32, FEAT, FAST_ROWS, 2>,
-    launch_step<32, TopoCassie32, FEAT, FAST_ROWS, 2, false, 2, MID_ROWS>,
+    launch_step<32, TopoCassie32, FEAT, FAST_ROWS, 1, false, 1, 0, FEAT_LEAN>,
+    launch_step<32, TopoCassie32, FEAT, FAST_ROWS, 2, false, 2, 0, FEAT_LEAN>,
+    launch_step<32, TopoCassie32, FEAT, FAST_ROWS, 2, false, 2, MID_ROWS, FEAT_LEAN>,
     nullptr,
     launch_step<32, TopoCassie32, FEAT, MID_ROWS, 2, true>,
     launch_step<32, TopoCassie32, FEAT, WIDE_ROWS, 2, true, 1>,
+    launch_step<32, TopoCassie32, FEAT, FAST_ROWS, 1, false, 1, 0, FEAT_PROF>,
+    launch_step<32, TopoCassie32, FEAT, FAST_ROWS, 2, false, 2, 0, FEAT_PROF>,
 };
 static const ck::StepLauncher TRAY_FORMS[ck::FORM_COUNT] = {
     launch_step<40, TopoCassieTray38, ck::FEAT_WAVEPAIRS>,
     launch_step<40, TopoCassieTray38, ck::FEAT_WAVEPAIRS, MID_ROWS, 2>,
     nullptr,
-    launch_step<40, TopoCassieTray38, ck::FEAT_WAVEPAIRS, FAST_ROWS_TRAY>,
-    launch_step<40, TopoCassieTray38, ck::FEAT_WAVEPAIRS, FAST_ROWS_TRAY, 2>,
+    launch_step<40, TopoCassieTray38, ck::FEAT_WAVEPAIRS, FAST_ROWS_TRAY, 1, false, 1, 0, FEAT_LEAN>,
+    launch_step<40, TopoCassieTray38, ck::FEAT_WAVEPAIRS, FAST_ROWS_TRAY, 2, false, 2, 0, FEAT_READOUT>,
     nullptr,
     launch_step<40, TopoCassieTray38, ck::FEAT_WAVEPAIRS, MID_ROWS, 1, true>,
     launch_step<40, TopoCassieTray38, ck::FEAT_WAVEPAIRS, MID_ROWS, 2, true>,
     nullptr,
+    launch_step<40, TopoCassieTray38, ck::FEAT_WAVEPAIRS, FAST_ROWS_TRAY, 1, false, 1, 0, FEAT_PROF>,
+    launch_step<40, TopoCassieTray38, ck::FEAT_WAVEPAIRS, FAST_ROWS_TRAY, 2, false, 2, 0, FEAT_FULL>,
 };
 static const ck::StepLauncher CASSIE_ALL_FORMS[ck::FORM_COUNT] = {launch_step<32, TopoCassie32, ck::FEAT_ALL>};
 static const ck::StepLauncher TRAY_HFIELD_FORMS[ck::FORM_COUNT] = {launch_step<40, TopoCassieTray38, ck::FEAT_ALL>};
@@ -305,8 +310,9 @@
     const ck::StepFamily fam = ck::pick_family(hm, b->generic_kernel);
     const ck::StepLauncher *family = FAMILY_FORMS[fam];
     const bool has_inplace = family[ck::FORM_FAST_INPLACE] != nullptr;
+    const bool prof = io.prof != nullptr;
     auto forms_if = [&](bool inplace) {
-        return ck::launch_forms(fam, has_inplace, hm.maxefc, integrate, io.ext != nullptr, n, nsub, b->fast_rows, b->waves_per_env, b->waves_per_env_tray, inplace);
+        return ck::launch_forms(fam, has_inplace, hm.maxefc, integrate, io.ext != nullptr, n, nsub, b->fast_rows, b->waves_per_env, b->waves_per_env_tray, inplace, prof);
     };
     ck::StepForms forms = forms_if(false);
     const bool fast = ck::is_fast_form(forms.first);
@@ -322,9 +328,9 @@
         if (forms.wide) { hl.list2 = b->d_handover_list2; hl.count2 = b->d_handover_count2 + 2 * (size_t)env0; hl.seen2 = b->handover_seen2.dev() + env0; }
         const int seen = *(volatile int *)(b->handover_seen.host() + env0);
         grids = ck::pass_grids(n, seen, forms.wide ? b->handover_seen2.host()[env0] : 0, forms.wide);
-        if (forms.first == ck::FORM_FAST_2W && has_inplace) {
+        if ((forms.first == ck::FORM_FAST_2W || forms.first == ck::FORM_FAST_2W_PROF) && has_inplace) {
             const bool was = range->inplace;
-            range->inplace = ck::next_inplace(was, seen, b->inplace_mode, io.order != nullptr);
+            range->inplace = !prof && ck::next_inplace(was, seen, b->inplace_mode, io.order != nullptr);
             if (was != range->inplace) reset_range_words(b, env0, s);
             ++b->form_launches[range->inplace ? 1 : 0];
             forms = forms_if(range->inplace);
@@ -334,6 +340,10 @@
     for (int i = 0; i < plan.n; ++i) {
         const ck::StepPass &p = plan.pass[i];
         if (!family[p.form]) { (void)hip_ok(hipErrorInvalidDeviceFunction, "cassie_step_kernel launch (no instantiation of this form)"); return -1; }
+        if (ck::lean_form_refuses(p.form, p.io.ext != nullptr, p.io.integrate, p.io.prof != nullptr)) {
+            (void)hip_ok(hipErrorInvalidValue, "cassie_step_kernel launch (a lean fast form with the read-out block, a forward pass or the stage stamps)");
+            return -1;
+        }
         family[p.form](p.grid, s, p.io);
         if (!hip_ok(hipGetLastError(), "cassie_step_kernel launch")) return -1;
         if (i == 0 && ev_after) (void)hipEventRecord(ev_after, s);
diff --git a/cassie-mujoco-sim_amd/csrc/physics_kernel.h b/cassie-mujoco-sim_amd/csrc/physics_kernel.h
--- a/cassie-mujoco-sim_amd/csrc/physics_kernel.h
+++ b/cassie-mujoco-sim_amd/csrc/physics_kernel.h
@@ -102,8 +102,8 @@
     bool bailed = false, bailed_down = false;
     int sub = sub_start;
     for (; sub < nsub; ++sub) {
-        const bool lastsub = sub == nsub - 1 || !io.integrate;
-        const bool need_quat = lastsub || io.ext != nullptr || io.all_outputs_every_substep || (io.drive_mode && sub + 2 == nsub);
+        const bool lastsub = sub == nsub - 1 || !integrates<FEAT>(io);
+        const bool need_quat = lastsub || readout_ext<FEAT>(io) != nullptr || io.all_outputs_every_substep || (io.drive_mode && sub + 2 == nsub);
         {
             bool badv = false;
             if (lane < nq) { double v = S.qpos[lane]; badv |= !(v == v) || fabs(v) > 1e10; }
@@ -430,7 +430,7 @@
         CK_STAMP(24);
         if constexpr (NW == 2) {
             wv::publish(&S.cmd[1], sub + 1);
-        } else bias_forces_and_qfrc_smooth<NVP>(io, S, m, env, ids, kdamp, kstiff, kref, kgear, klo, khi, kq, ka);
+        } else bias_forces_and_qfrc_smooth<NVP, FEAT>(io, S, m, env, ids, kdamp, kstiff, kref, kgear, klo, khi, kq, ka);
         const int pf_eq = lane < 3 * m->neq ? lane / 3 : 0;
         int pf_eb1 = m->eq_body1[pf_eq], pf_eb2 = m->eq_body2[pf_eq], pf_er1 = m->eq_root[pf_eq][0], pf_er2 = m->eq_root[pf_eq][1];
 
@@ -442,7 +442,7 @@
         io.progress[env] = bailed ? sub : nsub;
         if (bailed && !bailed_down && io.handover_out_list) io.handover_out_list[io.env0 + wv::atomic_add(io.handover_out_count, 1)] = env;
     }
-    if (io.integrate && io.drive_mode) {
+    if (integrates<FEAT>(io) && io.drive_mode) {
         drive_state_store(io, S, env, lane);
         if (lane < nu) io.ctrl[(size_t)env * io.su + lane] = S.ctrl[lane];
         if (bailed) {
@@ -454,7 +454,7 @@
             }
         }
     }
-    if (io.integrate) {
+    if (integrates<FEAT>(io)) {
         if (lane < nq) io.qpos[(size_t)env * io.sq + lane] = S.qpos[lane];
         if (lane < nv) {
             io.qvel[(size_t)env * io.sqv + lane] = S.qvel[lane];
@@ -471,8 +471,9 @@
     return (warn & WARN_DIVERGED) ? -2 : (bailed ? (bailed_down ? sub | ENV_STEP_WENT_DOWN : sub) : nsub);
 }
 
-template <int NVP, class TOPO, int FEAT = FEAT_ALL, int MAXR = MID_ROWS, int NW = 1, bool WALK = false, int WPS = NW, int INROWS = 0>
+template <int NVP, class TOPO, int FEAT = FEAT_ALL, int MAXR = MID_ROWS, int NW = 1, bool WALK = false, int WPS = NW, int INROWS = 0, int SERVE = FEAT_FULL>
 WV_GLOBAL void __launch_bounds__(WV_WAVE * NW) WV_OCC WV_WAVES_PER_SIMD(WPS) cassie_step_kernel(PhysIO io) {
+    static_assert((FEAT & FEAT_FULL) == 0 && (SERVE & ~FEAT_FULL) == 0, "FEAT: the collision bits; SERVE: FEAT_READOUT / FEAT_PROF");
     WV_SHARED EnvShared<NVP, LPack<TOPO, NVP>::count, MAXR> S;
     const int slot = wv::env_id();
     if constexpr (WALK) {
@@ -481,7 +482,7 @@
         for (int idx = slot; idx < count; idx += wv::grid_size()) {
             const int env = io.handover_list[io.env0 + idx];
             const long long t0 = io.cost ? wv::clock() : 0, t0w = io.cost_wall ? wv::wall_clock() : 0;
-            env_step<NVP, TOPO, FEAT, MAXR, NW>(io, S, env, io.progress[env], io.nsub);
+            env_step<NVP, TOPO, FEAT | SERVE, MAXR, NW>(io, S, env, io.progress[env], io.nsub);
             if (io.cost && wv::lane() == 0 && (NW == 1 || wv::wave_id() == 0)) {
                 io.cost[env] += (unsigned)((wv::clock() - t0) >> 6);
                 if (io.cost_wall) io.cost_wall[env] += (unsigned)(wv::wall_clock() - t0w);
@@ -526,13 +527,13 @@
         const bool stay = io.inplace_stay_rows > 0;
         bool did = false;
         for (int s = sub_start;;) {
-            int at = env_step<NVP, TOPO, FEAT, MAXR, NW>(io, S, env, s, sub_end);
+            int at = env_step<NVP, TOPO, FEAT | SERVE, MAXR, NW>(io, S, env, s, sub_end);
             if (wv::lane() == 0 && wv::wave_id() == 0) S.cmd[5] = at;
             wv::drain_vmem(); wv::block_barrier();
             at = wv::opaque(S.cmd[5]);
             if (at < 0 || at >= sub_end) break;
             did = true;
-            int at2 = env_step<NVP, TOPO, FEAT, INROWS, NW>(io2, S2, env, at, stay ? sub_end : at + 1);
+            int at2 = env_step<NVP, TOPO, FEAT | SERVE, INROWS, NW>(io2, S2, env, at, stay ? sub_end : at + 1);
             if (wv::lane() == 0 && wv::wave_id() == 0) S.cmd[5] = at2;
             wv::drain_vmem(); wv::block_barrier();
             at2 = wv::opaque(S.cmd[5]);
@@ -544,11 +545,13 @@
             s = at2;
         }
         if (did && io.inplace_count && wv::lane() == 0 && wv::wave_id() == 0) wv::atomic_add(io.inplace_count, 1);
-    } else env_step<NVP, TOPO, FEAT, MAXR, NW>(io, S, env, sub_start, sub_end);
+    } else env_step<NVP, TOPO, FEAT | SERVE, MAXR, NW>(io, S, env, sub_start, sub_end);
     if (sub_end < io.nsub) wv::publish_global<NW>(io.chunk_flag + env, io.chunk_seq, chunk + 1);
+    if constexpr (feat_prof(SERVE)) {
     if (io.prof && wv::lane() == 0) io.prof[(size_t)env * NSTAMP + 40 + (NW == 2 ? wv::wave_id() : 0)] = wv::hw_id();
     if (io.prof && wv::lane() == 0 && (NW == 1 || wv::wave_id() == 0)) {
         io.prof[(size_t)env * NSTAMP + 42] = wv::clock(); io.prof[(size_t)env * NSTAMP + 43] = wv::wall_clock();
+    }
     }
     if (io.cost && wv::lane() == 0 && (NW == 1 || wv::wave_id() == 0)) {
         const unsigned c = (unsigned)((wv::clock() - t0) >> 6);
diff --git a/cassie-mujoco-sim_amd/csrc/pk_stages.h b/cassie-mujoco-sim_amd/csrc/pk_stages.h
--- a/cassie-mujoco-sim_amd/csrc/pk_stages.h
+++ b/cassie-mujoco-sim_amd/csrc/pk_stages.h
@@ -159,7 +159,12 @@
     }
 }
 
-enum { FEAT_HFIELD = 1, FEAT_WAVEPAIRS = 2, FEAT_ALL = 3 };
+enum { FEAT_HFIELD = 1, FEAT_WAVEPAIRS = 2, FEAT_READOUT = 4, FEAT_PROF = 8, FEAT_LEAN = 0, FEAT_FULL = FEAT_READOUT | FEAT_PROF, FEAT_ALL = FEAT_HFIELD | FEAT_WAVEPAIRS };
+
+constexpr bool feat_readout(int feat) { return (feat & FEAT_READOUT) != 0; }
+constexpr bool feat_prof(int feat) { return (feat & FEAT_PROF) != 0; }
+template <int FEAT> WV_DEVICE cm_ext_t *readout_ext(const PhysIO &io) { if constexpr (feat_readout(FEAT)) return io.ext; else return nullptr; }
+template <int FEAT> WV_DEVICE bool integrates(const PhysIO &io) { if constexpr (feat_readout(FEAT)) return io.integrate != 0; else return true; }
 
 struct LaneIds { int nbody, nv, broot, bend, kjnt, kbody, kjt, kda, kroot, kbend; unsigned long long kdesc; };
 
@@ -316,15 +321,15 @@
         }
     }
     }
-    if (io.ext && isdof) {
-        cm_ext_t *ex = io.ext + env;
+    if (readout_ext<FEAT>(io) && isdof) {
+        cm_ext_t *ex = readout_ext<FEAT>(io) + env;
 #pragma unroll
         for (int i = 0; i < NVP; ++i) if (i < nv && i >= k_) { const double v = (i == k_) ? col[i] + m->dof_armature[k_] : col[i]; ex->qM[i][k_] = v; ex->qM[k_][i] = v; }
     }
     CK_STAMP(3);
 }
 
-template <int NVP, bool ROLLED = false, class SH>
+template <int NVP, int FEAT, bool ROLLED = false, class SH>
 WV_DEVICE void bias_forces_and_qfrc_smooth(const PhysIO &io, SH &S, ModelPtr m, int env, const LaneIds &ids, const double kdamp, const double kstiff,
                                            const double kref, const double kgear, const double klo, const double khi, const int kq, const int ka) {
     const int nbody = ids.nbody, nv = ids.nv, kbody = ids.kbody, kbend = ids.kbend;
diff --git a/cassie-mujoco-sim_amd/csrc/pk_types.h b/cassie-mujoco-sim_amd/csrc/pk_types.h
--- a/cassie-mujoco-sim_amd/csrc/pk_types.h
+++ b/cassie-mujoco-sim_amd/csrc/pk_types.h
@@ -12,7 +12,7 @@
 constexpr int FAST_ROWS_TRAY = 47;
 constexpr int NSTAMP = 48;
 #define CK_TRI(k, i) ((k) * ((k) + 1) / 2 + (i))
-#define CK_STAMP(i) do { if (io.prof && lane == 0) io.prof[(size_t)env * NSTAMP + (i)] = wv::clock(); CK_FRESH(); } while (0)
+#define CK_STAMP(i) do { if constexpr (feat_prof(FEAT)) { if (io.prof && lane == 0) io.prof[(size_t)env * NSTAMP + (i)] = wv::clock(); } CK_FRESH(); } while (0)
 #define CK_FRESH() do { lane = wv::fresh_lane(); b = lane; k_ = lane; isbody = b < nbody; isdof = k_ < nv; } while (0)
 
 enum { WARN_CONTACT_FULL = 1, WARN_CONSTRAINT_FULL = 2, WARN_UNSUPPORTED_PAIR = 4, WARN_DIVERGED = 8,
diff --git a/cassie-mujoco-sim_amd/csrc/step_kernels.h b/cassie-mujoco-sim_amd/csrc/step_kernels.h
--- a/cassie-mujoco-sim_amd/csrc/step_kernels.h
+++ b/cassie-mujoco-sim_amd/csrc/step_kernels.h
@@ -4,9 +4,9 @@
 #include "step_launch.h"
 
 namespace ck {
-template <int NVP, class TOPO, int FEAT, int MAXR, int NW, bool WALK, int WPS, int INROWS>
+template <int NVP, class TOPO, int FEAT, int MAXR, int NW, bool WALK, int WPS, int INROWS, int SERVE>
 void launch_step(unsigned grid, hipStream_t s, const PhysIO &io) {
-    hipLaunchKernelGGL((cassie_step_kernel<NVP, TOPO, FEAT, MAXR, NW, WALK, WPS, INROWS>), dim3(grid), dim3(NW * WV_WAVE), 0, s, io);
+    hipLaunchKernelGGL((cassie_step_kernel<NVP, TOPO, FEAT, MAXR, NW, WALK, WPS, INROWS, SERVE>), dim3(grid), dim3(NW * WV_WAVE), 0, s, io);
 }
 }
 #endif
diff --git a/cassie-mujoco-sim_amd/csrc/step_launch.h b/cassie-mujoco-sim_amd/csrc/step_launch.h
--- a/cassie-mujoco-sim_amd/csrc/step_launch.h
+++ b/cassie-mujoco-sim_amd/csrc/step_launch.h
@@ -8,7 +8,7 @@
 namespace ck {
 using StepLauncher = void (*)(unsigned grid, hipStream_t s, const PhysIO &io);
 
-template <int NVP, class TOPO, int FEAT = FEAT_ALL, int MAXR = MID_ROWS, int NW = 1, bool WALK = false, int WPS = NW, int INROWS = 0>
+template <int NVP, class TOPO, int FEAT = FEAT_ALL, int MAXR = MID_ROWS, int NW = 1, bool WALK = false, int WPS = NW, int INROWS = 0, int SERVE = FEAT_FULL>
 void launch_step(unsigned grid, hipStream_t s, const PhysIO &io);
 }
 #endif
diff --git a/cassie-mujoco-sim_amd/csrc/step_plan.h b/cassie-mujoco-sim_amd/csrc/step_plan.h
--- a/cassie-mujoco-sim_amd/csrc/step_plan.h
+++ b/cassie-mujoco-sim_amd/csrc/step_plan.h
@@ -15,6 +15,8 @@
     FORM_MID_WALK,
     FORM_MID_WALK_2W,
     FORM_WIDE_WALK,
+    FORM_FAST_PROF,
+    FORM_FAST_2W_PROF,
     FORM_COUNT
 };
 
@@ -60,7 +62,9 @@
 struct StepPass { int form; unsigned grid; PhysIO io; };
 struct StepPlan { int n; StepPass pass[3]; };
 
-inline bool is_fast_form(int form) { return form == FORM_FAST || form == FORM_FAST_2W || form == FORM_FAST_INPLACE; }
+inline bool is_lean_form(int form) { return form == FORM_FAST || form == FORM_FAST_2W || form == FORM_FAST_INPLACE; }
+inline bool is_prof_form(int form) { return form == FORM_FAST_PROF || form == FORM_FAST_2W_PROF; }
+inline bool is_fast_form(int form) { return is_lean_form(form) || is_prof_form(form); }
 
 inline StepPlan plan_step(const PhysIO &base, const StepForms &f, const HandoverLists &hl, const StepGrids &g) {
     StepPlan p;
diff --git a/cassie-mujoco-sim_amd/csrc/step_policy.h b/cassie-mujoco-sim_amd/csrc/step_policy.h
--- a/cassie-mujoco-sim_amd/csrc/step_policy.h
+++ b/cassie-mujoco-sim_amd/csrc/step_policy.h
@@ -13,20 +13,29 @@
 constexpr int INPLACE_STAY_ROWS = FAST_ROWS - 4;
 
 inline StepForms launch_forms(int fam, bool has_inplace, int maxefc, int integrate, bool ext, int n, int nsub, bool fast_rows,
-                              int waves_per_env, int waves_per_env_tray, bool inplace) {
+                              int waves_per_env, int waves_per_env_tray, bool inplace, bool prof = false) {
     StepForms forms = {FORM_ALONE, FORM_ALONE, false, INPLACE_STAY_ROWS};
     if (fam == CASSIE || fam == CASSIE_HFIELD) {
         forms.wide = maxefc > CM_MAXEFC_NARROW;
         if (!fast_rows || !integrate || ext || (n <= SMALL_BATCH && nsub <= SMALL_BATCH_NSUB))
             forms.first = forms.wide ? FORM_WIDE : n > SMALL_BATCH ? FORM_ALONE : FORM_ALONE_2W;
-        else if (waves_per_env == 2) { forms.first = inplace && has_inplace ? FORM_FAST_INPLACE : FORM_FAST_2W; forms.mid = FORM_MID_WALK_2W; }
-        else forms.first = FORM_FAST;
+        else if (waves_per_env == 2) { forms.first = prof ? FORM_FAST_2W_PROF : inplace && has_inplace ? FORM_FAST_INPLACE : FORM_FAST_2W; forms.mid = FORM_MID_WALK_2W; }
+        else forms.first = prof ? FORM_FAST_PROF : FORM_FAST;
     } else if (fam == TRAY) {
         const bool plain = integrate && !ext, two = plain && waves_per_env_tray == 2;
-        if (plain && fast_rows) { forms.first = two ? FORM_FAST_2W : FORM_FAST; forms.mid = two ? FORM_MID_WALK_2W : FORM_MID_WALK; }
+        if (plain && fast_rows) {
+            forms.first = two ? (prof ? FORM_FAST_2W_PROF : FORM_FAST_2W) : (prof ? FORM_FAST_PROF : FORM_FAST);
+            forms.mid = two ? FORM_MID_WALK_2W : FORM_MID_WALK;
+        }
         else forms.first = two ? FORM_ALONE_2W : FORM_ALONE;
     }
     return forms;
+}
+
+inline bool lean_form_refuses(int form, bool ext, int integrate, bool prof) {
+    if (is_lean_form(form)) return ext || !integrate || prof;
+    if (is_prof_form(form)) return ext || !integrate;
+    return false;
 }
 
 
```

After: 27.88 million, median of 6. +1.2%, better.
